# althonos/pyhmmer

Measured on AMD Instinct MI355X. Metric: GCUPS (DP cells/s) + seqs/s for hmmsearch, Pfam-A vs proteome, 1/2/4/8 GPUs, higher is better.
Workload: dtype u8/i16 filters (MSV, Viterbi), f32 Forward/Backward

## Files before the change

include/p7x.h:

```cpp
#ifndef P7X_H
#define P7X_H

#include <stddef.h>
#include <stdint.h>

#ifdef __cplusplus
extern "C" {
#endif

#define P7X_ABI_VERSION 8

enum {
  P7X_OK = 0, P7X_EMEM = 5, P7X_EFORMAT = 7, P7X_EINVAL = 11, P7X_ERANGE = 16, P7X_ENORESULT = 19,
  P7X_ENODEVICE = 100, P7X_EDEVICE = 101
};

enum { P7X_RNA = 1, P7X_DNA = 2, P7X_AMINO = 3 };
enum { P7X_SEARCH_SEQS = 0, P7X_SCAN_MODELS = 1 };
enum { P7X_ZSETBY_NTARGETS = 0, P7X_ZSETBY_OPTION = 1, P7X_ZSETBY_FILEINFO = 2 };
enum { P7X_MMU = 0, P7X_MLAMBDA, P7X_VMU, P7X_VLAMBDA, P7X_FTAU, P7X_FLAMBDA };
enum { P7X_GA1 = 0, P7X_GA2, P7X_TC1, P7X_TC2, P7X_NC1, P7X_NC2 };
#define P7X_CUTOFF_UNSET (-99999.0f)
#define P7X_EVPARAM_UNSET (-99999.0f)
enum { P7X_IS_INCLUDED = 1, P7X_IS_REPORTED = 2, P7X_IS_NEW = 4, P7X_IS_DROPPED = 8, P7X_IS_DUPLICATE = 16 };
// ... 78 lines not shown
  int32_t do_max, do_biasfilter, do_null2;
  uint32_t seed;
  int32_t mode;
  int32_t host_threads;
  int32_t host_envelopes;
  int32_t host_regions;
  int32_t long_targets;
  int32_t strands;
  int32_t B1, B2, B3;
  int32_t block_length;
  int32_t window_length;
  int32_t evalue_window_length;
  int32_t lt_part, lt_nparts;
  float   oa_guard;
  float   f3_guard;
  uint64_t lt_resident_key;
  int32_t host_ensembles;
  float   ens_guard;
} p7x_pipeline_cfg;
enum { P7X_STRAND_BOTH = 0, P7X_STRAND_TOPONLY = 1, P7X_STRAND_BOTTOMONLY = 2 };
void p7x_pipeline_cfg_default(p7x_pipeline_cfg *cfg);

typedef struct p7x_counters {
  uint64_t nmodels, nseqs, nres, nnodes;
  uint64_t n_past_msv, n_past_bias, n_past_vit, n_past_fwd;
  uint64_t n_output, pos_past_msv, pos_past_bias, pos_past_vit, pos_past_fwd, pos_output;
} p7x_counters;

typedef struct p7x_domain {
  int64_t ienv, jenv, iali, jali, iorf, jorf;
  float envsc, domcorrection, dombias, oasc, bitscore;
  double lnP;
  int32_t is_reported, is_included;
  int32_t N, hmmfrom, hmmto, M;
  int64_t sqfrom, sqto, L;
  const char *model, *mline, *aseq, *ppline, *rfline, *mmline, *csline;
  const char *hmmname, *hmmacc, *hmmdesc, *sqname, *sqacc, *sqdesc;
} p7x_domain;

typedef struct p7x_hit {
  const char *name, *acc, *desc;
  int64_t seqidx;
  int32_t window_length;
  double sortkey;
  float score, pre_score, sum_score;
  double lnP, pre_lnP, sum_lnP;
  float nexpected;
  int32_t nregions, nclustered, noverlaps, nenvelopes, ndom;
  uint32_t flags;
  int32_t nreported, nincluded, best_domain;
} p7x_hit;

typedef struct p7x_tophits p7x_tophits;

int p7x_search_block(const p7x_pipeline_cfg *cfg, const p7x_oprofile *om, const float *bg_f,
                     const p7x_seqdb *db, const char *const *names, const char *const *accs,
                     const char *const *descs, p7x_tophits **out);

typedef struct p7x_pending p7x_pending;
int  p7x_search_block_begin(const p7x_pipeline_cfg *cfg, const p7x_oprofile *om, const float *bg_f,
                            const p7x_seqdb *db, p7x_pending **out);
int  p7x_search_block_finish(p7x_pending *pending, const char *const *names, const char *const *accs,
                             const char *const *descs, p7x_tophits **out);
void p7x_pending_destroy(p7x_pending *pending);
int  p7x_search_block_enqueue(const p7x_pipeline_cfg *cfg, const p7x_oprofile *om, const float *bg_f,
                              const p7x_seqdb *db, p7x_pending **out);
int  p7x_search_block_wait(p7x_pending *pending);
int  p7x_search_batch_enqueue(const p7x_pipeline_cfg *cfg, const p7x_oprofile *const *oms, size_t nq, const float *bg_f,
                              const p7x_seqdb *db, p7x_pending **out);
int  p7x_search_batch_finish(p7x_pending *pending, const char *const *names, const char *const *accs,
                             const char *const *descs, p7x_tophits **outs);
size_t p7x_pending_nqueries(const p7x_pending *pending);
int  p7x_debug_log_of_float(int device, const float *in, float *out, size_t n);
int  p7x_debug_memory_stats(int device, int64_t out[4]);
int  p7x_debug_choice(const float *p, int n, uint32_t x, int *via_thresholds, int *via_fchoose);
int  p7x_debug_order_spread(const p7x_oprofile *om, const uint8_t *dsq1, int32_t L, int32_t i, int32_t j, int multihit, double *out12);
int  p7x_debug_parser_rows(const p7x_oprofile *om, const uint8_t *dsq1, int32_t L, float *fx, float *bx);
int64_t p7x_debug_ssv_tables(const p7x_oprofile *om, int pair, int32_t *R, int32_t *pair_slack, uint32_t *tab4q, size_t cap_words);
int  p7x_debug_set_option(const char *name, int value);
int  p7x_debug_ensemble(const p7x_oprofile *om, const p7x_seqdb *db, int64_t target, int32_t i, int32_t j, uint32_t seed,
                        int use_device, int32_t *ndom, int32_t *dom, int32_t dom_cap, float *n2, int32_t *status);
int  p7x_search_batch_raw(const p7x_pipeline_cfg *cfg, const p7x_oprofile *const *oms, size_t nq, const float *bg_f,
                          const p7x_seqdb *db, int32_t *xJ, int32_t *xC, uint8_t *stage);

int p7x_search_longtargets(const p7x_pipeline_cfg *cfg, const p7x_oprofile *om, int device,
                           const uint8_t *dsq, const int64_t *offsets, const int64_t *lengths, size_t n,
                           const char *const *names, const char *const *accs, const char *const *descs, p7x_tophits **out);
int p7x_longtargets_release_resident(int device, uint64_t key);
int64_t p7x_ssv_longtarget_seeds(const p7x_pipeline_cfg *cfg, const p7x_oprofile *om, int device, const uint8_t *dsq, int64_t L,
                                 int complement, int64_t *seeds, size_t cap);
int p7x_longtarget_from_seeds(const p7x_pipeline_cfg *cfg, const p7x_oprofile *om,
                              const uint8_t *dsq, const int64_t *offsets, const int64_t *lengths, size_t n,
                              const char *const *names, const char *const *accs, const char *const *descs,
                              const int64_t *seed_target, const int64_t *seed_block, const int32_t *seed_strand,
                              const int64_t *seeds, size_t nseeds, p7x_tophits **out);

int p7x_forward_parser_exact(const p7x_oprofile *om, const uint8_t *dsq, int32_t L, float *sc);

int p7x_scan_collect(p7x_tophits *const *per_model, size_t nmodels, const p7x_pipeline_cfg *cfg, size_t nseqs,
                     const char *const *seq_names, const char *const *seq_accs, const char *const *seq_descs,
                     const int32_t *seq_lengths, p7x_tophits **out);
typedef struct p7x_scan_accum p7x_scan_accum;
int  p7x_scan_accum_create(const p7x_pipeline_cfg *cfg, size_t nseqs, const char *const *seq_names, const char *const *seq_accs,
                           const char *const *seq_descs, const int32_t *seq_lengths, p7x_scan_accum **out);
int  p7x_scan_accum_add(p7x_scan_accum *acc, p7x_tophits *const *per_model, size_t nmodels);
int  p7x_scan_accum_add_indexed(p7x_scan_accum *acc, p7x_tophits *const *per_model, const int64_t *model_index, size_t nmodels);
int  p7x_debug_tophits_set_stages(p7x_tophits *th, const uint8_t *stage, size_t n);
int  p7x_scan_accum_finish(p7x_scan_accum *acc, p7x_tophits **out);
void p7x_scan_accum_destroy(p7x_scan_accum *acc);

int p7x_postprocess_targets(const p7x_pipeline_cfg *cfg, const p7x_oprofile *om, const uint8_t *dsq,
                            const int64_t *offsets, const int32_t *lengths, size_t n, const int32_t *surv,
                            size_t nsurv, const float *fwdsc, const float *fwd_xmx, const float *bck_xmx,
                            const int64_t *xmx_off, const uint64_t *stage_counts, const char *const *names,
                            const char *const *accs, const char *const *descs, p7x_tophits **out);

void     p7x_tophits_destroy(p7x_tophits *th);
void     p7x_tophits_destroy_many(p7x_tophits **th, size_t n);
p7x_tophits *p7x_tophits_clone(const p7x_tophits *th);
int64_t  p7x_tophits_nhits(const p7x_tophits *th);
int      p7x_tophits_abc_type(const p7x_tophits *th);
int      p7x_tophits_get_counters(const p7x_tophits *th, p7x_counters *c);
int      p7x_tophits_get_cfg(const p7x_tophits *th, p7x_pipeline_cfg *cfg);
int      p7x_tophits_get_hit(const p7x_tophits *th, int64_t i, p7x_hit *hit);
int      p7x_tophits_get_domain(const p7x_tophits *th, int64_t i, int32_t d, p7x_domain *dom);
int      p7x_tophits_merge(p7x_tophits *dst, const p7x_tophits *src);
int      p7x_tophits_merge_longtargets(p7x_tophits **parts, size_t nparts, p7x_tophits **out);
int      p7x_tophits_merge_many(const void *const *blobs, const size_t *sizes, size_t nq, size_t nparts, int threads, p7x_tophits **outs);
int64_t  p7x_tophits_serialize(const p7x_tophits *th, void *buf, size_t cap);
p7x_tophits *p7x_tophits_deserialize(const void *buf, size_t n);
int      p7x_tophits_sort_by_key(p7x_tophits *th);
int      p7x_tophits_threshold(p7x_tophits *th);
int      p7x_tophits_sort_by_seqidx(p7x_tophits *th);
int      p7x_tophits_is_sorted(const p7x_tophits *th, int by_seqidx);
int      p7x_tophits_set_hit_flags(p7x_tophits *th, int64_t i, uint32_t flags);
int      p7x_tophits_set_hit_text(p7x_tophits *th, int64_t i, int which, const char *value);
int      p7x_tophits_get_timings(const p7x_tophits *th, double *ms, int n);
int      p7x_tophits_get_guard_counts(const p7x_tophits *th, int64_t *f3_dropped, int64_t *oa_redone, int64_t oa_why[8]);
int      p7x_tophits_get_ensemble_counts(const p7x_tophits *th, int64_t *sampled_on_device, int64_t *redone_by_host, int64_t *region_scans_redone);

typedef struct p7x_traces p7x_traces;
enum { P7X_TRACE_HAS_PP = 1, P7X_TRACE_DEVICE = 2 };
int     p7x_tracealign_compute(const p7x_oprofile *om, int device, const uint8_t *dsq, const int64_t *offsets,
                               const int32_t *lengths, size_t n, int host_threads, p7x_traces **out);
int64_t p7x_traces_count(const p7x_traces *tr);
int64_t p7x_traces_nflagged(const p7x_traces *tr);
int     p7x_traces_stats(const p7x_traces *tr, int64_t out4[4]);
int     p7x_traces_get(const p7x_traces *tr, int64_t idx, int32_t *N, int32_t *M, int32_t *L, float *sc2, int32_t *status, uint8_t *origin);
int     p7x_traces_copy(const p7x_traces *tr, int64_t idx, int8_t *st, int32_t *k, int32_t *i, float *pp);
void    p7x_traces_destroy(p7x_traces *tr);

enum { P7X_MSA_TRIM = 1, P7X_MSA_ALL_CONSENSUS_COLS = 2, P7X_MSA_DIGITIZE = 4 };
typedef struct p7x_msa p7x_msa;
int     p7x_msa_from_traces(int32_t M, size_t n, const int8_t *st, const int32_t *k, const int32_t *i, const float *pp,
                            const int64_t *toff, const uint8_t *origin, const uint8_t *dsq, const int64_t *offsets,
                            const int32_t *lengths, int32_t abc_type, const char *cs, int flags, const p7x_oprofile *om,
                            p7x_msa **out);
int64_t p7x_msa_alen(const p7x_msa *msa);
int64_t p7x_msa_get(const p7x_msa *msa, int64_t idx, int which, char *buf, size_t cap);
void    p7x_msa_destroy(p7x_msa *msa);
int64_t p7x_msa_write_stockholm(size_t n, int64_t alen, const char *const *names, const char *const *accs,
                                const char *const *descs, const char *const *aseqs, const char *const *pps,
                                const char *ss_cons, const char *pp_cons, const char *rf, char *buf, size_t cap);

int     p7x_alidisplay_backconvert(int32_t abc_type, const char *model, const char *aseq, const char *ppline, int32_t hmmfrom,
                                   int32_t hmmto, int64_t sqfrom, int64_t sqto, int64_t L, int whole, int32_t *N, int32_t *subL,
// ... 33 lines not shown
```

pyhmmer_amd/_lib.py:

```python
from __future__ import annotations

import ctypes as C
import os
import shutil
import subprocess
from pathlib import Path

_PKG = Path(__file__).resolve().parent
_ROOT = _PKG.parent
CSRC = _PKG / "csrc"
LIB_PATH = _PKG / "libp7x.so"

SOURCES = ["p7x_profile.cpp", "p7x_device.hip", "p7x_devmem.hip", "p7x_devimage.hip", "p7x_msv.hip", "p7x_vitfwd.hip", "p7x_vitpk.hip", "p7x_fwdpk.hip", "p7x_envelope.hip", "p7x_ensemble.hip", "p7x_ssvlong.hip", "p7x_longtarget.hip",
           "p7x_envscore.hip", "p7x_pipeline.hip", "p7x_domaindef.cpp", "p7x_longtarget_host.cpp", "p7x_tophits.cpp", "p7x_align.hip", "p7x_tracealign.cpp", "p7x_builder.cpp", "p7x_calibrate.hip"]


def _hipcc() -> str:
    for cand in (os.environ.get("HIPCC"), shutil.which("hipcc"), "/opt/rocm/bin/hipcc"):
        if cand and os.path.exists(cand):
            return cand
    raise RuntimeError("hipcc not found (need ROCm; set HIPCC=/path/to/hipcc)")


ISA_CHECKED = ("p7x_msv.hip", "p7x_envelope.hip")
# ... 121 lines not shown
        ("hmmname", C.c_char_p), ("hmmacc", C.c_char_p), ("hmmdesc", C.c_char_p),
        ("sqname", C.c_char_p), ("sqacc", C.c_char_p), ("sqdesc", C.c_char_p),
    ]


class HitRec(C.Structure):
    _fields_ = [
        ("name", C.c_char_p), ("acc", C.c_char_p), ("desc", C.c_char_p),
        ("seqidx", C.c_int64), ("window_length", C.c_int32), ("sortkey", C.c_double),
        ("score", C.c_float), ("pre_score", C.c_float), ("sum_score", C.c_float),
        ("lnP", C.c_double), ("pre_lnP", C.c_double), ("sum_lnP", C.c_double),
        ("nexpected", C.c_float),
        ("nregions", C.c_int32), ("nclustered", C.c_int32), ("noverlaps", C.c_int32),
        ("nenvelopes", C.c_int32), ("ndom", C.c_int32),
        ("flags", C.c_uint32), ("nreported", C.c_int32), ("nincluded", C.c_int32), ("best_domain", C.c_int32),
    ]


_VP = C.c_void_p
_SIGNATURES = {
    "p7x_abi_version": (C.c_int, []),
    "p7x_tophits_merge_longtargets": (C.c_int, [C.POINTER(_VP), C.c_size_t, C.POINTER(_VP)]),
    "p7x_tophits_merge_many": (C.c_int, [C.POINTER(C.c_char_p), C.POINTER(C.c_size_t), C.c_size_t, C.c_size_t, C.c_int, C.POINTER(_VP)]),
    "p7x_tophits_get_guard_counts": (C.c_int, [_VP, C.POINTER(C.c_int64), C.POINTER(C.c_int64), C.POINTER(C.c_int64)]),
    "p7x_tophits_get_ensemble_counts": (C.c_int, [_VP, C.POINTER(C.c_int64), C.POINTER(C.c_int64), C.POINTER(C.c_int64)]),
    "p7x_hmm_max_length": (C.c_int, [C.POINTER(HmmView), C.c_double, C.POINTER(C.c_int32)]),
    "p7x_expf_neg": (None, [_VP, _VP, C.c_size_t]),
    "p7x_oprofile_create": (C.c_int, [C.POINTER(HmmView), _VP, C.c_int32, C.POINTER(_VP)]),
    "p7x_oprofile_destroy": (None, [_VP]),
    "p7x_oprofile_get_info": (C.c_int, [_VP, C.POINTER(OprofileInfo)]),
    "p7x_oprofile_striped": (C.c_int64, [_VP, C.c_int, _VP, C.c_size_t]),
    "p7x_device_count": (C.c_int, []),
    "p7x_device_name": (C.c_int, [C.c_int, C.c_char_p, C.c_size_t]),
    "p7x_seqdb_create": (C.c_int, [C.c_int, C.c_int32, _VP, _VP, _VP, C.c_size_t, C.POINTER(_VP)]),
    "p7x_seqdb_destroy": (None, [_VP]),
    "p7x_seqdb_ntargets": (C.c_int64, [_VP]),
    "p7x_seqdb_nresidues": (C.c_int64, [_VP]),
    "p7x_msv_filter": (C.c_int, [_VP, C.c_int, _VP, C.c_int32, C.POINTER(C.c_float)]),
    "p7x_vit_filter": (C.c_int, [_VP, C.c_int, _VP, C.c_int32, C.POINTER(C.c_float)]),
    "p7x_fwd_parser": (C.c_int, [_VP, C.c_int, _VP, C.c_int32, C.POINTER(C.c_float)]),
    "p7x_bck_parser": (C.c_int, [_VP, C.c_int, _VP, C.c_int32, C.POINTER(C.c_float)]),
    "p7x_filters_batch": (C.c_int, [_VP, _VP, _VP, _VP, _VP, _VP]),
    "p7x_pipeline_cfg_default": (None, [C.POINTER(PipelineCfg)]),
    "p7x_search_block": (C.c_int, [C.POINTER(PipelineCfg), _VP, _VP, _VP, _VP, _VP, _VP, C.POINTER(_VP)]),
    "p7x_postprocess_targets": (C.c_int, [C.POINTER(PipelineCfg), _VP, _VP, _VP, _VP, C.c_size_t, _VP, C.c_size_t, _VP, _VP, _VP,
                                          _VP, _VP, _VP, _VP, _VP, C.POINTER(_VP)]),
    "p7x_tophits_destroy": (None, [_VP]),
    "p7x_tophits_destroy_many": (None, [_VP, C.c_size_t]),
    "p7x_tophits_clone": (_VP, [_VP]),
    "p7x_tophits_nhits": (C.c_int64, [_VP]),
    "p7x_tophits_abc_type": (C.c_int, [_VP]),
    "p7x_tophits_get_counters": (C.c_int, [_VP, C.POINTER(Counters)]),
    "p7x_tophits_get_cfg": (C.c_int, [_VP, C.POINTER(PipelineCfg)]),
    "p7x_tophits_get_hit": (C.c_int, [_VP, C.c_int64, C.POINTER(HitRec)]),
    "p7x_tophits_get_domain": (C.c_int, [_VP, C.c_int64, C.c_int32, C.POINTER(DomainRec)]),
    "p7x_tophits_merge": (C.c_int, [_VP, _VP]),
    "p7x_tophits_serialize": (C.c_int64, [_VP, _VP, C.c_size_t]),
    "p7x_tophits_deserialize": (_VP, [_VP, C.c_size_t]),
    "p7x_tophits_sort_by_key": (C.c_int, [_VP]),
    "p7x_tophits_threshold": (C.c_int, [_VP]),
    "p7x_tophits_sort_by_seqidx": (C.c_int, [_VP]),
    "p7x_tophits_is_sorted": (C.c_int, [_VP, C.c_int]),
    "p7x_tophits_set_hit_flags": (C.c_int, [_VP, C.c_int64, C.c_uint32]),
    "p7x_tophits_set_hit_text": (C.c_int, [_VP, C.c_int64, C.c_int, C.c_char_p]),
    "p7x_tophits_get_timings": (C.c_int, [_VP, C.POINTER(C.c_double), C.c_int]),
    "p7x_search_block_begin": (C.c_int, [C.POINTER(PipelineCfg), _VP, _VP, _VP, C.POINTER(_VP)]),
    "p7x_search_block_enqueue": (C.c_int, [C.POINTER(PipelineCfg), _VP, _VP, _VP, C.POINTER(_VP)]),
    "p7x_search_block_wait": (C.c_int, [_VP]),
    "p7x_search_block_finish": (C.c_int, [_VP, _VP, _VP, _VP, C.POINTER(_VP)]),
    "p7x_pending_destroy": (None, [_VP]),
    "p7x_search_batch_enqueue": (C.c_int, [C.POINTER(PipelineCfg), C.POINTER(_VP), C.c_size_t, _VP, _VP, C.POINTER(_VP)]),
    "p7x_search_batch_finish": (C.c_int, [_VP, _VP, _VP, _VP, C.POINTER(_VP)]),
    "p7x_pending_nqueries": (C.c_size_t, [_VP]),
    "p7x_debug_log_of_float": (C.c_int, [C.c_int, _VP, _VP, C.c_size_t]),
    "p7x_debug_memory_stats": (C.c_int, [C.c_int, C.POINTER(C.c_int64)]),
    "p7x_debug_choice": (C.c_int, [_VP, C.c_int, C.c_uint32, _VP, _VP]),
    "p7x_debug_order_spread": (C.c_int, [_VP, _VP, C.c_int32, C.c_int32, C.c_int32, C.c_int, _VP]),
    "p7x_debug_parser_rows": (C.c_int, [_VP, _VP, C.c_int32, _VP, _VP]),
    "p7x_debug_ssv_tables": (C.c_int64, [_VP, C.c_int, _VP, _VP, _VP, C.c_size_t]),
    "p7x_debug_set_option": (C.c_int, [C.c_char_p, C.c_int]),
    "p7x_longtargets_release_resident": (C.c_int, [C.c_int, C.c_uint64]),
    "p7x_debug_ensemble": (C.c_int, [_VP, _VP, C.c_int64, C.c_int32, C.c_int32, C.c_uint32, C.c_int, _VP, _VP, C.c_int32, _VP, _VP]),
    "p7x_search_batch_raw": (C.c_int, [C.POINTER(PipelineCfg), C.POINTER(_VP), C.c_size_t, _VP, _VP, _VP, _VP, _VP]),
    "p7x_search_longtargets": (C.c_int, [C.POINTER(PipelineCfg), _VP, C.c_int, _VP, _VP, _VP, C.c_size_t, _VP, _VP, _VP, C.POINTER(_VP)]),
    "p7x_ssv_longtarget_seeds": (C.c_int64, [C.POINTER(PipelineCfg), _VP, C.c_int, _VP, C.c_int64, C.c_int, _VP, C.c_size_t]),
    "p7x_forward_parser_exact": (C.c_int, [_VP, _VP, C.c_int32, C.POINTER(C.c_float)]),
    "p7x_longtarget_from_seeds": (C.c_int, [C.POINTER(PipelineCfg), _VP, _VP, _VP, _VP, C.c_size_t, _VP, _VP, _VP, _VP, _VP, _VP, _VP,
                                            C.c_size_t, C.POINTER(_VP)]),
    "p7x_oprofile_write_pressed": (C.c_int, [_VP, C.POINTER(C.c_int64), _VP, C.c_size_t, C.POINTER(C.c_size_t), _VP, C.c_size_t,
                                             C.POINTER(C.c_size_t)]),
    "p7x_oprofile_read_pressed": (C.c_int, [_VP, C.c_size_t, _VP, C.c_size_t, _VP, C.POINTER(_VP), C.POINTER(C.c_size_t),
                                            C.POINTER(C.c_size_t), C.POINTER(C.c_int64)]),
    "p7x_oprofile_get_string": (C.c_int, [_VP, C.c_int, C.c_char_p, C.c_size_t]),
    "p7x_scan_collect": (C.c_int, [C.POINTER(_VP), C.c_size_t, C.POINTER(PipelineCfg), C.c_size_t, _VP, _VP, _VP, _VP, C.POINTER(_VP)]),
    "p7x_scan_accum_create": (C.c_int, [C.POINTER(PipelineCfg), C.c_size_t, _VP, _VP, _VP, _VP, C.POINTER(_VP)]),
    "p7x_scan_accum_add": (C.c_int, [_VP, C.POINTER(_VP), C.c_size_t]),
    "p7x_scan_accum_add_indexed": (C.c_int, [_VP, C.POINTER(_VP), C.POINTER(C.c_int64), C.c_size_t]),
    "p7x_debug_tophits_set_stages": (C.c_int, [_VP, _VP, C.c_size_t]),
    "p7x_scan_accum_finish": (C.c_int, [_VP, C.POINTER(_VP)]),
    "p7x_scan_accum_destroy": (None, [_VP]),
    "p7x_fasta_parse": (C.c_int, [_VP, C.c_size_t, _VP, C.POINTER(C.c_size_t), C.POINTER(C.c_size_t), C.POINTER(C.c_size_t),
                                  _VP, _VP, _VP, _VP, _VP, _VP, C.POINTER(C.c_size_t)]),
    "p7x_tracealign_compute": (C.c_int, [_VP, C.c_int, _VP, _VP, _VP, C.c_size_t, C.c_int, C.POINTER(_VP)]),
    "p7x_traces_count": (C.c_int64, [_VP]),
    "p7x_traces_nflagged": (C.c_int64, [_VP]),
    "p7x_traces_stats": (C.c_int, [_VP, _VP]),
    "p7x_traces_get": (C.c_int, [_VP, C.c_int64, C.POINTER(C.c_int32), C.POINTER(C.c_int32), C.POINTER(C.c_int32), _VP,
                                 C.POINTER(C.c_int32), C.POINTER(C.c_uint8)]),
    "p7x_traces_copy": (C.c_int, [_VP, C.c_int64, _VP, _VP, _VP, _VP]),
    "p7x_traces_destroy": (None, [_VP]),
    "p7x_msa_from_traces": (C.c_int, [C.c_int32, C.c_size_t, _VP, _VP, _VP, _VP, _VP, _VP, _VP, _VP, _VP, C.c_int32, C.c_char_p,
                                      C.c_int, _VP, C.POINTER(_VP)]),
    "p7x_msa_alen": (C.c_int64, [_VP]),
    "p7x_msa_get": (C.c_int64, [_VP, C.c_int64, C.c_int, C.c_char_p, C.c_size_t]),
    "p7x_msa_destroy": (None, [_VP]),
    "p7x_msa_write_stockholm": (C.c_int64, [C.c_size_t, C.c_int64, C.POINTER(C.c_char_p), C.POINTER(C.c_char_p),
                                            C.POINTER(C.c_char_p), C.POINTER(C.c_char_p), C.POINTER(C.c_char_p), C.c_char_p,
                                            C.c_char_p, C.c_char_p, C.c_char_p, C.c_size_t]),
    "p7x_alidisplay_backconvert": (C.c_int, [C.c_int32, C.c_char_p, C.c_char_p, C.c_char_p, C.c_int32, C.c_int32, C.c_int64, C.c_int64,
                                             C.c_int64, C.c_int, C.POINTER(C.c_int32), C.POINTER(C.c_int32), _VP, _VP, _VP, _VP, _VP,
                                             C.c_size_t]),
    "p7x_tophits_to_msa": (C.c_int, [_VP, C.c_int32, C.c_int32, C.c_size_t, _VP, _VP, _VP, _VP, _VP, _VP, _VP, _VP, _VP,
                                     C.POINTER(C.c_char_p), C.POINTER(C.c_char_p), C.POINTER(C.c_char_p), C.c_int, C.POINTER(_VP)]),
    "p7x_debug_tophits_from_displays": (C.c_int, [C.c_char_p, C.c_int32, C.c_int32, C.c_size_t, C.POINTER(C.c_char_p),
                                                  C.POINTER(C.c_char_p), C.POINTER(C.c_char_p), C.POINTER(C.c_uint32),
                                                  C.POINTER(C.c_int32), C.POINTER(DomainRec), C.POINTER(_VP)]),
    "p7x_debug_tophits_from_trace": (C.c_int, [_VP, _VP, C.c_int32, C.c_int32, _VP, _VP, _VP, _VP, C.c_char_p, C.POINTER(_VP)]),
    "p7x_builder_single": (C.c_int, [C.c_int32, _VP, C.c_int32, _VP, C.c_char_p, C.c_double, C.c_double, _VP, _VP, _VP]),
    "p7x_calibration_stream": (C.c_int, [C.c_int32, _VP, C.c_uint32, C.c_int, _VP]),
    "p7x_calibration_redraw": (C.c_int, [C.c_int32, _VP, C.c_uint32, C.c_int, _VP, C.c_int, _VP]),
    "p7x_calibration_draw_of": (C.c_int32, [C.c_int32, _VP, C.c_int]),
    "p7x_calibration_scores": (C.c_int, [_VP, _VP, _VP, _VP, _VP]),
    "p7x_calibration_fit": (C.c_int, [_VP, _VP, C.c_double, _VP]),
    "p7x_oprofile_match_relent": (C.c_double, [_VP]),
    "p7x_calibrate_batch": (C.c_int, [C.POINTER(_VP), C.c_size_t, C.c_int, C.c_uint32, _VP, _VP]),
    "p7x_last_error": (C.c_char_p, []),
}

_lib = None


def lib() -> C.CDLL:
    global _lib
    if _lib is None:
        if not LIB_PATH.exists():
            raise ImportError(
                f"{LIB_PATH} is missing: the HIP extension has not been built. "
                "Run `python -c 'import __graft_entry__ as g; g.build()'` (needs hipcc); there is no CPU fallback.")
        l = C.CDLL(str(LIB_PATH))
        for name, (res, args) in _SIGNATURES.items():
            fn = getattr(l, name)
            fn.restype = res
            fn.argtypes = args
        if l.p7x_abi_version() != 8:
            raise ImportError("libp7x ABI version mismatch; rebuild")
        _lib = l
    return _lib


def declared_symbols():
    return sorted(_SIGNATURES)


def last_error() -> str:
    e = lib().p7x_last_error()
    return e.decode() if e else ""
# ... 6 lines not shown
```

pyhmmer_amd/csrc/p7x_device.hpp:

```cpp
#pragma once
#include "p7x_internal.hpp"
#include "p7x_devmem.hpp"
#include <hip/hip_runtime.h>
#include <map>
#include <memory>
#include <mutex>

namespace p7x {

constexpr int kMaxL      = 100000;
constexpr int kTabRows   = 32;
constexpr int kNegPad    = -512;

#define P7X_HIP(call)                                                                          \
  do { hipError_t e_ = (call); if (e_ != hipSuccess) {                                         \
    p7x::set_error(std::string(#call) + ": " + hipGetErrorString(e_)); return e_ == hipErrorOutOfMemory ? P7X_EMEM : P7X_EDEVICE; } } while (0)

struct LengthTables {
  uint8_t *tjb = nullptr;
  int16_t *xwmove = nullptr;
  float   *null1 = nullptr;
  double  *logtab = nullptr;
};

struct DeviceCtx {
  int device = -1;
  hipStream_t stream = nullptr;
  hipStream_t stream2 = nullptr;
  LengthTables lt;
  int num_cu = 256;
  std::mutex mu;
  std::mutex msv_mu;
  std::mutex lt_scan_mu;
  static constexpr int kLtStreams = 4;
  hipStream_t lt_stream[kLtStreams]{};
  int lt_next = 0;
  hipEvent_t msv_done[2] = { nullptr, nullptr };
  int msv_last = -1;
  std::mutex slab_mu;
  std::multimap<size_t, void *> slab_free;
  size_t slab_free_bytes = 0;
  size_t slab_obtained_bytes = 0;
  static constexpr int kWsSets = 4, kWsSide = 7;
  hipStream_t ws_main[kWsSets]{};
  hipStream_t ws_side[kWsSets][kWsSide]{};
  std::vector<hipStream_t> ws_spacers;
  int ws_set_users[kWsSets]{};
};
int get_ctx(int device, DeviceCtx **out);
int create_tail_stream(DeviceCtx *ctx, bool high_priority, hipStream_t *out);

struct DevProfile {
  int device = -1;
  int M = 0, Kp = 0;
  int msvR = 0, msvK = 0, msvS = 0;
  uint32_t *msv_tab = nullptr;
  int16_t *msvw_emis = nullptr;
  uint32_t *msvw_pk = nullptr;
  int msvwC = 0, msvw_rows = kTabRows;
  int vitC = 0, Mpad = 0;
  int16_t *vit_trans = nullptr;
  int16_t *vit_emis = nullptr;
  int vitpkT = 0, vitpkP = 0;
  uint32_t *vitpk_trans = nullptr, *vitpk_emis = nullptr;
  float *fwd_trans = nullptr;
  float *fwd_emis = nullptr;
  int fwdgT = 0, fwdgC = 0;
  float *fwdg_trans = nullptr, *fwdg_emis = nullptr;
  float *bias_eo = nullptr;
  std::shared_ptr<DeviceBuf> shared;
};

int get_dev_profile(const p7x_oprofile *om, DeviceCtx *ctx, DevProfile **out);
int get_dev_profiles(const p7x_oprofile *const *oms, int n, DeviceCtx *ctx, DevProfile **out, int nthreads);
void free_dev_profile(DevProfile *d);

struct EnvelopeScorer;
struct EnsembleRunner;
}
struct p7x_seqdb;
#include <memory>
namespace p7x {
struct LongTargetWindowRegions;
int device_regions_of_all(const p7x_oprofile *om, const p7x_seqdb *db, std::vector<LongTargetWindowRegions> &out);
std::unique_ptr<EnvelopeScorer> make_device_envelope_scorer(DeviceCtx *ctx, const p7x_seqdb *db, float oa_guard);
std::unique_ptr<EnvelopeScorer> make_device_align_scorer(DeviceCtx *ctx, const p7x_seqdb *db, float oa_guard);
size_t align_budget_bytes();
std::unique_ptr<EnsembleRunner> make_device_ensemble_runner(DeviceCtx *ctx, const p7x_seqdb *db, float guard);

}

struct p7x_seqdb {
  int device = -1;
  int abc_type = 0, Kp = 0;
  int64_t n = 0;
  int64_t nres = 0;
  int64_t nslots = 0;
  int64_t ngroups = 0;
  std::vector<int32_t> h_len;
  std::vector<int32_t> h_order;
  std::vector<int64_t> h_off;
  std::vector<uint8_t> h_dsq;
  int64_t vit_long_slots = 0;
  std::vector<int32_t> h_grp_len;
  std::vector<int64_t> h_grp_suffix;
  uint8_t *d_dsq = nullptr;
  int64_t *d_slot_off = nullptr;
  int32_t *d_slot_len = nullptr;
  uint4   *d_tiles = nullptr;
  int64_t *d_grp_off = nullptr;
  int32_t *d_grp_nblk = nullptr;
  int64_t tile_u4 = 0;
  p7x::DeviceBuf slab;
};
```

pyhmmer_amd/csrc/p7x_devimage.hip:

```cpp
#include "p7x_device.hpp"
#include "p7x_kernels.hpp"
#include "p7x_host.hpp"
#include <cstring>
#include <memory>

namespace p7x {

static void chunk_transpose_fill(int M, int C, std::vector<int> &pos_of_node)
{
  pos_of_node.assign(M + 1, -1);
  for (int k = 1; k <= M; ++k) { const int z = (k - 1) / C, c = (k - 1) % C; pos_of_node[k] = c * 64 + z; }
}

void free_dev_profile(DevProfile *d)
{
  delete d;
}

struct DevCache { std::mutex mu; std::vector<DevProfile *> per_device; };

struct ImageStage { int device = -1; PinnedBuf pinned; hipStream_t stream = nullptr; };

struct HostImage {
  std::vector<char> bytes;
  std::vector<std::pair<void **, size_t>> fix;
  template <typename T, typename F>
  void add(F **field, const std::vector<T> &v)
  {
    const size_t off = bytes.size(), n = v.size() * sizeof(T);
    bytes.resize(((off + n + 255) / 256) * 256);
    std::memcpy(bytes.data() + off, v.data(), n);
    fix.emplace_back(reinterpret_cast<void **>(field), off);
  }
};

static void build_host_image(const Profile &p, DevProfile *d, HostImage &img)
{
  d->msvR = msv_pick(p.M, &d->msvK);
  if (d->msvR > 0) {
    d->msvS = msv_stride(d->msvR, d->msvK);
    std::vector<uint32_t> tab;
    msv_build_tables(p, d->msvR, d->msvK, tab);
    img.add(&d->msv_tab, tab);
  }
  d->vitC = vit_pick_C(p.M);
  if (d->vitC > 0) {
    const int C = d->vitC, Mpad = 64 * C, nrows = p.Kp + 1;
    d->Mpad = Mpad;
    std::vector<int> pos;
    chunk_transpose_fill(p.M, C, pos);
    std::vector<int16_t> vt((size_t) Mpad * 8, -32768), ve((size_t) nrows * Mpad, -32768);
    std::vector<float> ft((size_t) Mpad * 8, 0.0f), fe((size_t) nrows * Mpad, 0.0f);
    for (int k = 1; k <= p.M; ++k) {
      for (int t = 0; t < NTRANS; ++t) {
        vt[(size_t) pos[k] * 8 + t] = p.tw[(size_t) t * (p.M + 1) + k];
        ft[(size_t) pos[k] * 8 + t] = p.tf[(size_t) t * (p.M + 1) + k];
      }
      for (int x = 0; x < p.Kp; ++x) {
        ve[(size_t) x * Mpad + pos[k]] = p.rw[(size_t) x * (p.M + 1) + k];
        fe[(size_t) x * Mpad + pos[k]] = p.rf_[(size_t) x * (p.M + 1) + k];
      }
    }
    {
      std::vector<int16_t> me((size_t) kTabRows * Mpad, (int16_t) kNegPad);
      for (int k = 1; k <= p.M; ++k)
        for (int x = 0; x < p.Kp; ++x) me[(size_t) x * Mpad + pos[k]] = (int16_t) ((int) p.bias_b - (int) p.rb[(size_t) x * (p.M + 1) + k]);
      img.add(&d->msvw_emis, me);
      d->msvwC = C; d->msvw_rows = kTabRows;
      int Cp = 0;
      if ((d->msvR <= 0 || d->msvK >= 8) && C % 4 == 0 && C <= 32) Cp = C;
      else if (d->msvR <= 0 && C > 32 && p.M <= 2560 && p.Kp + 1 <= 30) { Cp = p.M <= 2304 ? 36 : 40; d->msvwC = Cp; d->msvw_rows = p.Kp + 1; }
      if (Cp > 0) {
        const int P2 = Cp / 4, rows = d->msvw_rows;
        std::vector<uint32_t> pk((size_t) rows * P2 * 64 * 2);
        auto em = [&](int x, int k) -> uint32_t { return (uint32_t) (uint16_t) (int16_t) ((x < p.Kp && k <= p.M) ? (int) p.bias_b - (int) p.rb[(size_t) x * (p.M + 1) + k] : kNegPad); };
        for (int x = 0; x < rows; ++x)
          for (int j2 = 0; j2 < P2; ++j2)
            for (int z = 0; z < 64; ++z)
              for (int h = 0; h < 2; ++h) {
                const int k = z * Cp + 2 * (2 * j2 + h) + 1;
                pk[(((size_t) x * P2 + j2) * 64 + z) * 2 + h] = em(x, k) | (em(x, k + 1) << 16);
              }
        img.add(&d->msvw_pk, pk);
      }
    }
    img.add(&d->vit_trans, vt);
    img.add(&d->vit_emis, ve);
    img.add(&d->fwd_trans, ft);
    img.add(&d->fwd_emis, fe);
    int gT = 0, gC = 0;
    if (fwdg_pick(p.M, d->vitC, &gT, &gC)) {
      std::vector<float> gt, ge;
      fwdg_build_tables(p, gT, gC, gt, ge);
      d->fwdgT = gT; d->fwdgC = gC;
      img.add(&d->fwdg_trans, gt);
      img.add(&d->fwdg_emis, ge);
    }
  }
  {
    int T = 0, P = 0;
    if (vitpk_pick(p.M, &T, &P)) {
      std::vector<uint32_t> tt, te;
      vitpk_build_tables(p, T, P, tt, te);
      d->vitpkT = T; d->vitpkP = P;
      img.add(&d->vitpk_trans, tt);
      img.add(&d->vitpk_emis, te);
    }
  }
  {
    const Alphabet &abc = Alphabet::get(p.abc_type);
    std::vector<float> eo((size_t) kTabRows * 2, 1.0f);
    for (int x = 0; x < p.K; ++x) { eo[x * 2 + 0] = p.bgf[x] / p.bgf[x]; eo[x * 2 + 1] = p.compo[x] / p.bgf[x]; }
    for (int x = p.K + 1; x <= p.Kp - 3; ++x)
      for (int s = 0; s < 2; ++s) {
        float e = 0.0f, den = 0.0f;
        for (int y = 0; y < p.K; ++y) if (abc.degen[x][y]) { e += (s == 0 ? p.bgf[y] : p.compo[y]); den += p.bgf[y]; }
        eo[x * 2 + s] = den > 0.0f ? e / den : 0.0f;
      }
    img.add(&d->bias_eo, eo);
  }
}

int get_dev_profiles(const p7x_oprofile *const *oms, int n, DeviceCtx *ctx, DevProfile **out, int nthreads)
{
  std::vector<int> missing;
  for (int i = 0; i < n; ++i) {
// ... 74 lines not shown
```

pyhmmer_amd/csrc/p7x_internal.hpp:

```cpp
#pragma once
#include "../../include/p7x.h"
#include <cstdint>
#include <string>
#include <vector>

namespace p7x {

constexpr int MAXK  = 20;
constexpr int MAXKP = 29;
constexpr double kLog2  = 0.69314718055994529;
constexpr double kLog2R = 1.44269504088896341;

enum { XE = 0, XN = 1, XJ = 2, XC = 3 };
enum { MOVE = 0, LOOP = 1 };
enum { tBM = 0, tMM, tIM, tDM, tMD, tMI, tII, tDD, NTRANS };
enum { gMM = 0, gIM, gDM, gBM, gMD, gDD, gMI, gII };

struct Alphabet {
  int type, K, Kp;
  const char *sym;
  unsigned char degen[MAXKP][MAXK];
  static const Alphabet &get(int type);
};

struct Profile {
  int M = 0, K = 0, Kp = 0, abc_type = 0, L = 0, max_length = -1, mode = 0;
  float nj = 1.0f;
  double relent_mh = 0.0;
  std::string name, acc, desc, consensus, rf, mm, cs;
  bool has_acc = false, has_desc = false;
  float evparam[6], cutoff[6], compo[MAXK], bgf[MAXK];
  std::vector<float> tsc;
  std::vector<float> msc;
  float xsc[4][2];
  std::vector<uint8_t> rb;
  uint8_t tbm_b, tec_b, tjb_b, base_b, bias_b;
  float scale_b;
  std::vector<int16_t> rw;
  std::vector<int16_t> tw;
  int16_t xw[4][2];
  float scale_w; int16_t base_w, ddbound_w; float ncj_roundoff;
  std::vector<float> rf_;
  std::vector<float> tf;
  float xf[4][2];

  int Q16() const { int q = (M - 1) / 16 + 1; return q < 2 ? 2 : q; }
  int Q8()  const { int q = (M - 1) / 8  + 1; return q < 2 ? 2 : q; }
  int Q4()  const { int q = (M - 1) / 4  + 1; return q < 2 ? 2 : q; }
};

float  sse_expf(float x);
uint8_t unbiased_byteify(float scale_b, float sc);
int16_t wordify(float scale_w, float sc);
double gumbel_surv(double x, double mu, double lambda);
double exp_surv(double x, double mu, double lambda);
double exp_logsurv(double x, double mu, double lambda);
float  null1_score(int L);
double match_relent_sum(const float *mat, const float *bg_f, int M, int K);
void   flogsum_init();
float  flogsum(float a, float b);

void set_error(const std::string &msg);

enum { OPT_SMALL_BLOCK = 0, OPT_VIT_WAVE, OPT_MSV_EXACT, OPT_MSV_LONG_GROUPS, OPT_MSV_BLOCKS_PER_CU, OPT_ENV_WORKSPACE_GB, OPT_DEVICE_CLUSTERED,
       OPT_TRACE_FINISH, OPT_TRACE_LONGTARGET, OPT_TRACE_ENVELOPE, OPT_HOST_PROFILE, OPT_SSV_KERNEL, OPT_MSV_F16, OPT_ENS_LDS_KB, OPT_ENS_FAIL, OPT_MSV_TIERS, OPT_STAGE_MERGE, OPT_EARLY_PACK, OPT_HOST_ORDER, OPT_VIT_LONG_CUT, OPT_FWD_GROUPED, OPT_REGION_GUARD_PPM, OPT_MSV_K8, OPT_MSV_LANE_BLOCKS, OPT_HOST_ALIGN, OPT_ALIGN_WORKSPACE_GB, OPT_COUNT };
int debug_opt(int which);

}
struct p7x_oprofile;
namespace p7x {
void attach_dev_cache(p7x_oprofile *om);

}

struct p7x_oprofile { p7x::Profile p; void *dev_cache = nullptr; };
```

pyhmmer_amd/csrc/p7x_kernels.hpp:

```cpp
#pragma once
#include <type_traits>
#include "p7x_device.hpp"

namespace p7x {

struct ArgRef { const void *base; uint32_t stride; };
#if defined(__HIPCC__)
template <class A> __device__ __forceinline__ A load_args(const ArgRef r)
{
#if defined(__HIP_DEVICE_COMPILE__)
  typedef const __attribute__((address_space(4))) A *cptr;
  return *(cptr) (unsigned long long) (static_cast<const char *>(r.base) + (size_t) blockIdx.y * r.stride);
#else
  return *reinterpret_cast<const A *>(static_cast<const char *>(r.base) + (size_t) blockIdx.y * r.stride);
#endif
}
#endif
template <class A> struct ArgRun {
  const A *host = nullptr; const void *dev = nullptr; uint32_t stride = 0; int n = 0;
  const A &at(int i) const { return *reinterpret_cast<const A *>(reinterpret_cast<const char *>(host) + (size_t) i * stride); }
  ArgRef ref() const { return ArgRef{ dev, stride }; }
};
inline unsigned lane_grid(long want, long resident, int nlanes)
{
  (void) nlanes;
  if (want > resident) want = resident;
  return (unsigned) (want < 1 ? 1 : want);
}

inline unsigned lane_grid_pull(long want, long resident, int nlanes, bool old_rule)
{
  if (old_rule || nlanes < 32) return lane_grid(want, resident, nlanes);
  long b = (2 * resident + nlanes - 1) / nlanes;
  if (b > resident) b = resident;
  if (b > want) b = want;
  return (unsigned) (b < 1 ? 1 : b);
}

struct MsvArgs {
  const uint32_t *tab;
  const uint4 *tiles;
  const int64_t *grp_off;
  const int32_t *grp_nblk;
  const int32_t *slot_len;
  const uint8_t *tjb_tab;
  int ngroups;
  int group_first;
  int base, bias, tec, tbm;
  int *counter;
  int16_t *out_xJ;
  int *amb_count; int *amb_groups; int *counter2;
  const int *group_list; const int *group_count;
  int R;
};
int  msv_pick(int M, int *K);
int  msv_stride(int R, int K);
void msv_build_tables(const Profile &p, int R, int K, std::vector<uint32_t> &out);
int  msv_launch(int R, int K, const ArgRun<MsvArgs> &main, const ArgRun<MsvArgs> *amb, int num_cu, hipStream_t st);
constexpr int kMsvTiers = 6;
int  msv_tier(int R, int K);
int  msv_tier_launch(int tier, const ArgRun<MsvArgs> &main, int num_cu, hipStream_t st);
int  msv_exact_launch(int R, int K, const ArgRun<MsvArgs> &amb, int num_cu, hipStream_t st);

#define P7X_NODE_TIERS(X) X(1) X(2) X(3) X(4) X(5) X(6) X(8) X(10) X(12) X(16) X(20) X(24) X(32) X(48) X(64) X(96) X(128)
template <class F> int node_tier_dispatch(int C, const char *too_long, F &&f)
{
  switch (C) {
#define P7X_TIER_CASE(CC) case CC: return f(std::integral_constant<int, CC>());
    P7X_NODE_TIERS(P7X_TIER_CASE)
#undef P7X_TIER_CASE
    default: set_error(too_long); return P7X_EINVAL;
  }
}
struct WaveSeqArgs {
  int M, C;
  const void *trans;
  const void *emis;
  const uint8_t *dsq;
  const int64_t *slot_off;
  const int32_t *slot_len;
  const int32_t *list;
  int nlist;
  const int *nlist_ptr;
  const int *abort_flag;
  int nrows;
  int *counter;
  const int16_t *xwmove_tab; int base_w, xw_e, ddbound;
  int32_t *out_xC;
  const int *lt_thresh;
  int *lt_nrec; int *lt_rec; int lt_cap;
  float xf_e_move, xf_e_loop;
  float *out_sc;
  float *xmx;
  const int64_t *xmx_off;
  const float *fwd_xmx;
};
int vit_pick_C(int M);
int vit_launch(const ArgRun<WaveSeqArgs> &a, int num_cu, hipStream_t st);
int fwd_launch(const ArgRun<WaveSeqArgs> &a, int num_cu, hipStream_t st);
bool fwdg_pick(int M, int vitC, int *T, int *C);
int fwdg_launch(const ArgRun<WaveSeqArgs> &a, int num_cu, hipStream_t st);
void fwdg_build_tables(const Profile &p, int T, int C, std::vector<float> &trans, std::vector<float> &emis);
int bck_launch(const ArgRun<WaveSeqArgs> &a, int num_cu, hipStream_t st);

struct MsvWaveArgs {
  int C, nrows;
  const void *emis;
  const void *emis_pk;
  const uint8_t *dsq; const int64_t *slot_off; const int32_t *slot_len; const uint8_t *tjb_tab;
  int nslots, base, bias, tec, tbm;
  int16_t *out_xJ;
};
int msv_wave_launch(const ArgRun<MsvWaveArgs> &a, int num_cu, hipStream_t st);

struct VitPkArgs {
  const void *trans, *emis;
  const uint8_t *dsq; const int64_t *slot_off; const int32_t *slot_len;
  const int32_t *list; int nlist; const int *nlist_ptr;
  const int *nskip_ptr;
  int nrows;
  const int16_t *xwmove_tab; int base_w, xw_e, ddbound;
  int32_t *out_xC;
};
bool vitpk_pick(int M, int *T, int *P);
void vitpk_build_tables(const Profile &p, int T, int P, std::vector<uint32_t> &trans, std::vector<uint32_t> &emis);
int  vitpk_launch(int T, int P, const ArgRun<VitPkArgs> &a, int num_cu, hipStream_t st);

struct EnvArgs {
  int M, C, K, nrows;
  const void *trans;
  const void *emis;
  const uint8_t *dsq;
  float nj, xf_e_move, xf_e_loop;
  int nenv;
  const int64_t *env_sq;
  const int32_t *env_len;
  const int32_t *env_L;
  const int32_t *order;
  int *cursor;
  float *work; int64_t work_stride; int Lmax;
  int nblocks, slab_base;
  float *out_sc;
  const float *env_emis;
  long long env_emis_stride;
  float *out_orig;
  float oa_guard;
  int32_t *out_status;
  float *out_null2;
  const int64_t *tr_off;
  uint32_t *tr_a; int32_t *tr_i; float *tr_pp;
  int32_t *tr_n;
};
constexpr int env_waves(int C) { return C >= 8 ? 4 : 8; }
enum class EnvMode { Envelope, LongTarget, Align };
inline size_t env_work_floats(int C, int Lmax)
{
  const size_t rows = (size_t) Lmax + 1, Mpad = (size_t) 64 * C;
  size_t f = 2 * rows * Mpad + rows * (6 + 6 + 5 + 3 + 1);
  f += (rows * Mpad + 1) / 2;
  return (f + 63) & ~(size_t) 63;
}
int env_max_blocks(EnvMode mode, int C, int nrows, int num_cu, int *nblocks);
int env_launch(EnvMode mode, const ArgRun<EnvArgs> &a, hipStream_t st);
__host__ __device__ inline float align_pp_guard(int M) { return 1.0e-5f + 2.5e-9f * (float) M; }
__host__ __device__ inline float align_pp_band(int M) { return 0.5f - 10.0f * align_pp_guard(M); }
int align_max_blocks(int C, int nrows, int num_cu, int *nblocks);
int align_launch(const ArgRun<EnvArgs> &a, hipStream_t st);

struct ChoiceCell; struct ChoiceRow;
struct EnsRegion {
  int64_t sq;
  int64_t cell0;
  int64_t row0;
  int64_t dom0;
  int32_t Lr, L;
  int32_t job, dom_cap;
};
struct EnsJob {
  int M, C, K, Kp, nrows, Q;
  const void *trans, *emis;
  const float *rft;
  const uint8_t *degen;
  int reg_first, nreg;
};
struct EnsArgs {
  const EnsJob *jobs; const EnsRegion *regions; int nregions;
  const uint8_t *dsq;
  ChoiceCell *cells; float2 *md; ChoiceRow *rows;
  uint32_t seed_x;
  int nsamples;
  float *n2acc;
  int32_t *dom;
  int32_t *out_ndom; int32_t *out_status;
  int lds_bytes;
// ... 26 lines not shown
```

pyhmmer_amd/csrc/p7x_msv.hip:

```cpp
#include <cstdlib>
#include <iterator>
#include <map>
#include <mutex>
#include "p7x_device.hpp"
#include "p7x_kernels.hpp"

namespace p7x {

typedef short s2 __attribute__((ext_vector_type(2)));

__device__ __forceinline__ s2 as_s2(uint32_t u) { return __builtin_bit_cast(s2, u); }
__device__ __forceinline__ uint32_t as_u32(s2 v) { return __builtin_bit_cast(uint32_t, v); }
__device__ __forceinline__ s2 pk_max(s2 a, s2 b) { return __builtin_elementwise_max(a, b); }
__device__ __forceinline__ s2 pk_adds(s2 a, s2 b) { return __builtin_elementwise_add_sat(a, b); }
__device__ __forceinline__ s2 pk_subs(s2 a, s2 b) { return __builtin_elementwise_sub_sat(a, b); }
__device__ __forceinline__ s2 splat(int v) { s2 r; r.x = (short) v; r.y = (short) v; return r; }
__device__ __forceinline__ s2 swap_halves(s2 v) { return as_s2(__builtin_amdgcn_alignbit(as_u32(v), as_u32(v), 16)); }

typedef _Float16 h2 __attribute__((ext_vector_type(2)));
__device__ __forceinline__ h2 as_h2(s2 v) { return __builtin_bit_cast(h2, v); }
__device__ __forceinline__ s2 as_s2(h2 v) { return __builtin_bit_cast(s2, v); }
__device__ __forceinline__ s2 h_adds(s2 a, s2 b)
{
  const h2 z = { (_Float16) 0.0f, (_Float16) 0.0f }, o = { (_Float16) 1.0f, (_Float16) 1.0f };
  return as_s2(__builtin_elementwise_min(__builtin_elementwise_max(as_h2(a) + as_h2(b), z), o));
}
__device__ __forceinline__ s2 h_subs(s2 a, s2 b)
{
  const h2 z = { (_Float16) 0.0f, (_Float16) 0.0f }, o = { (_Float16) 1.0f, (_Float16) 1.0f };
  return as_s2(__builtin_elementwise_min(__builtin_elementwise_max(as_h2(a) - as_h2(b), z), o));
}
__device__ __forceinline__ s2 h_max(s2 a, s2 b) { return as_s2(__builtin_elementwise_maximum(as_h2(a), as_h2(b))); }
__device__ __forceinline__ s2 h_max3(s2 a, s2 b, s2 c)
{ return as_s2(__builtin_elementwise_maximum(__builtin_elementwise_maximum(as_h2(a), as_h2(b)), as_h2(c))); }
__device__ __forceinline__ s2 h_splat(int units)
{ const _Float16 x = (_Float16) ((float) units * (1.0f / 256.0f)); h2 r; r.x = x; r.y = x; return as_s2(r); }
__device__ __forceinline__ uint32_t h_of_i16_pair(uint32_t w)
{
  const int lo = max((int) (short) (w & 0xffffu), -512), hi = max((int) (short) (w >> 16), -512);
  return __builtin_bit_cast(uint32_t, __builtin_amdgcn_cvt_pkrtz((float) lo * (1.0f / 256.0f), (float) hi * (1.0f / 256.0f)));
}


constexpr int msv_stride_c(int R)
{
  int S = R + (R & 1);
  if (((S / 2) & 1) == 0) S += 2;
  return S;
}
constexpr int msv_lane_stride_c(int R, int K)
{
  if (K == 1) return msv_stride_c(R);
  int s = R + (R & 1);
  while (s % 64 != 2) s += 2;
  return s;
}
constexpr int msv_row_stride_c(int R, int K) { return K * msv_lane_stride_c(R, K); }
constexpr bool msv_uniform_c(int K) { return K >= 8; }
constexpr int msv_parities_c(int K) { return msv_uniform_c(K) ? 1 : 2; }
constexpr int msv_even_imm_c(int R, int K) { return K == 1 ? kTabRows * msv_row_stride_c(R, K) * 4 : 0; }
constexpr int msv_even_add_c(int R, int K) { return (K == 1 || msv_uniform_c(K)) ? 0 : kTabRows * msv_row_stride_c(R, K) * 4; }
constexpr int msv_block_c(int K) { return K == 1 ? 256 : 512; }
template <int K, bool H = false> __device__ __forceinline__ s2 target_max(s2 m)
{
  auto mx = [](s2 a, s2 b) { if constexpr (H) return h_max(a, b); else return pk_max(a, b); };
  if constexpr (K >= 2) m = mx(m, as_s2((uint32_t) __builtin_amdgcn_update_dpp(0, (int) as_u32(m), 0xB1, 0xf, 0xf, false)));
  if constexpr (K >= 4) m = mx(m, as_s2((uint32_t) __builtin_amdgcn_update_dpp(0, (int) as_u32(m), 0x4E, 0xf, 0xf, false)));
  if constexpr (K >= 8) m = mx(m, as_s2((uint32_t) __builtin_amdgcn_update_dpp(0, (int) as_u32(m), 0x141, 0xf, 0xf, false)));
  return m;
}
template <int K> __device__ __forceinline__ s2 carry_in(s2 last, s2 edge, int h)
{
  if constexpr (K == 1) return edge;
  const s2 up = as_s2((uint32_t) __builtin_amdgcn_update_dpp(0, (int) as_u32(last), 0x111, 0xf, 0xf, false));
  return h == 0 ? edge : up;
}

struct Chunk { uint2 e0, e1, e2, e3; };

template <int OFF>
__device__ __forceinline__ void lds_issue4(uint32_t addr, Chunk &c)
{
  asm volatile("ds_read_b64 %0, %4 offset:%5\n\t"
               "ds_read_b64 %1, %4 offset:%6\n\t"
               "ds_read_b64 %2, %4 offset:%7\n\t"
               "ds_read_b64 %3, %4 offset:%8"
               : "=&v"(c.e0), "=&v"(c.e1), "=&v"(c.e2), "=&v"(c.e3)
               : "v"(addr), "i"(OFF), "i"(OFF + 8), "i"(OFF + 16), "i"(OFF + 24));
}
template <int OFF>
__device__ __forceinline__ void lds_issue2(uint32_t addr, Chunk &c)
{
  asm volatile("ds_read_b64 %0, %2 offset:%3\n\t"
               "ds_read_b64 %1, %2 offset:%4"
               : "=&v"(c.e0), "=&v"(c.e1)
               : "v"(addr), "i"(OFF), "i"(OFF + 8));
}
template <int PENDING>
__device__ __forceinline__ void lds_wait4(Chunk &c)
{
  asm volatile("s_waitcnt lgkmcnt(%4)" : "+v"(c.e0), "+v"(c.e1), "+v"(c.e2), "+v"(c.e3) : "i"(PENDING));
}
template <int PENDING>
__device__ __forceinline__ void lds_wait2(Chunk &c)
{
  asm volatile("s_waitcnt lgkmcnt(%2)" : "+v"(c.e0), "+v"(c.e1) : "i"(PENDING));
}

template <int R, int TB, bool ODD, int T, int FAST = 0, bool U = false>
struct RowChunks {
  static_assert(!U || ODD, "the uniform row reads the register below: it is walked from the top register down");
  static_assert(R % 4 == 0, "a row is walked in chunks of 8 registers and a last one of 4: the register count must be a multiple of 4");
  static constexpr int NT = (R + 7) / 8;
  static constexpr int TBASE = TB;
  static constexpr int pairs(int t) { return (t == NT - 1 && (R % 8) != 0) ? 2 : 4; }

  template <int TT>
  static __device__ __forceinline__ void issue(uint32_t addr, Chunk &c)
  {
    if constexpr (pairs(TT) == 4) lds_issue4<TBASE + TT * 32>(addr, c); else lds_issue2<TBASE + TT * 32>(addr, c);
  }

  template <int JJ>
// ... 45 lines not shown
      }
      accA = pk_max(accA, v[2 * JJ]);
      accB = pk_max(accB, v[2 * JJ + 1]);
      asm volatile("" : "+v"(accA), "+v"(accB));
    } else if constexpr (ODD) {
      const s2 t1 = pk_max(v[2 * JJ], xB);
      v[2 * JJ + 1] = t1 + as_s2(e.y);
      accA = pk_max(accA, v[2 * JJ + 1]);
      s2 t0 = pk_max(carry, xB);
      if constexpr (JJ > 0) t0 = pk_max(v[2 * JJ - 1], xB);
      v[2 * JJ] = t0 + as_s2(e.x);
      accB = pk_max(accB, v[2 * JJ]);
    } else {
      v[2 * JJ] = pk_max(v[2 * JJ], xB) + as_s2(e.x);
      accA = pk_max(accA, v[2 * JJ]);
      v[2 * JJ + 1] = pk_max(v[2 * JJ + 1], xB) + as_s2(e.y);
      accB = pk_max(accB, v[2 * JJ + 1]);
    }
  }

  static __device__ __forceinline__ void run(s2 (&v)[R], uint32_t addr, Chunk &cur, Chunk &nxt, const s2 xB, const s2 carry, s2 &accA, s2 &accB)
  {
    constexpr bool last = ODD ? (T == 0) : (T == NT - 1);
    constexpr int TN = ODD ? T - 1 : T + 1;
    constexpr int np = pairs(T);
    if constexpr (!last) {
      issue<TN>(addr, nxt);
      if constexpr (np == 4) lds_wait4<pairs(TN)>(cur); else lds_wait2<pairs(TN)>(cur);
    } else {
      if constexpr (np == 4) lds_wait4<0>(cur); else lds_wait2<0>(cur);
    }
    if constexpr (ODD) {
      if constexpr (np == 4) {
        pair<4 * T + 3>(v, cur.e3, xB, carry, accA, accB);
        pair<4 * T + 2>(v, cur.e2, xB, carry, accA, accB);
      }
      pair<4 * T + 1>(v, cur.e1, xB, carry, accA, accB);
      pair<4 * T + 0>(v, cur.e0, xB, carry, accA, accB);
    } else {
      pair<4 * T + 0>(v, cur.e0, xB, carry, accA, accB);
      pair<4 * T + 1>(v, cur.e1, xB, carry, accA, accB);
      if constexpr (np == 4) {
        pair<4 * T + 2>(v, cur.e2, xB, carry, accA, accB);
        pair<4 * T + 3>(v, cur.e3, xB, carry, accA, accB);
      }
    }
    if constexpr (!last) RowChunks<R, TB, ODD, TN, FAST, U>::run(v, addr, nxt, cur, xB, carry, accA, accB);
  }
};

template <int R, int K, bool ODD>
__device__ __forceinline__ void msv_row(s2 (&v)[R], uint32_t addr, int h, s2 &xB, s2 &xJ, s2 &xEmax,
                                        const s2 basev, const s2 tecv, const s2 tjbmv, const s2 zerov)
{
  constexpr int NT = (R + 7) / 8;
  constexpr bool U = msv_uniform_c(K), DOWN = ODD || U;
  constexpr int T0 = DOWN ? NT - 1 : 0;
  constexpr int TB = DOWN ? 0 : msv_even_imm_c(R, K);
  const s2 carry = DOWN ? carry_in<K>(v[R - 1], xB, h) : xB;
  Chunk ca, cb;
  RowChunks<R, TB, DOWN, T0, 0, U>::template issue<T0>(addr, ca);
  s2 accA = splat(kNegPad), accB = accA;
  RowChunks<R, TB, DOWN, T0, 0, U>::run(v, addr, ca, cb, xB, carry, accA, accB);
  s2 m = pk_max(accA, accB);
  m = pk_max(m, swap_halves(m));
  m = target_max<K>(m);
  xEmax = pk_max(xEmax, m);
  m = m - tecv;
  xJ = pk_max(xJ, m);
  xB = pk_max(pk_max(basev, xJ) - tjbmv, zerov);
}

template <int K> struct MsvItem {
  int g, t, h;
  __device__ __forceinline__ MsvItem(int group, int part, int lane) : g(group), t(part * (64 / K) + lane / K), h(lane % K) {}
};

template <int R, int K>
__global__ void __launch_bounds__(msv_block_c(K)) msv_kernel(const ArgRef ref)
{
  extern __shared__ __attribute__((aligned(16))) uint32_t lds[];
  constexpr int S = msv_row_stride_c(R, K), Rs = msv_lane_stride_c(R, K), BLK = msv_block_c(K);
  const MsvArgs a = load_args<MsvArgs>(ref);
  const int nitems = (a.group_list ? *a.group_count : a.ngroups - a.group_first) * K;
  if (nitems <= 0 || *a.counter >= nitems) return;
  {
    constexpr int n4 = (msv_parities_c(K) * kTabRows * S) / 4;
    const uint4 *src = reinterpret_cast<const uint4 *>(a.tab);
    uint4 *dst = reinterpret_cast<uint4 *>(lds);
    for (int i = threadIdx.x; i < n4; i += BLK) dst[i] = src[i];
  }
  __syncthreads();

  const int lane = threadIdx.x & 63;
  const s2 basev = splat(a.base), tecv = splat(a.tec), zerov = splat(0);

  for (;;) {
    int item = 0;
    if (lane == 0) item = atomicAdd(a.counter, 1);
    item = __builtin_amdgcn_readfirstlane(item);
    if (item >= nitems) break;
    const int gi = item / K;
    const MsvItem<K> it(a.group_list ? __builtin_amdgcn_readfirstlane(a.group_list[gi]) : gi + a.group_first, item % K, lane);

    const int slot = it.g * 64 + it.t;
    const int L = a.slot_len[slot];
    const int nblk = a.grp_nblk[it.g];
    const uint4 *tp = a.tiles + a.grp_off[it.g] + it.t;
    const s2 tjbmv = splat((int) a.tjb_tab[L] + a.tbm);
    const uint32_t lane_col = (uint32_t) it.h * (uint32_t) (Rs * 4);

    s2 v[R];
#pragma unroll
    for (int j = 0; j < R; ++j) v[j] = zerov;
    s2 xJ = zerov, xEmax = zerov;
    s2 xB = pk_max(basev - tjbmv, zerov);

    uint4 cur = tp[0];
    for (int b = 0; b < nblk; ++b) {
      const uint4 nxt = (b + 1 < nblk) ? tp[(size_t) (b + 1) * 64] : cur;
      uint32_t w0 = cur.x, w1 = cur.y, w2 = cur.z, w3 = cur.w;
#pragma unroll 1
      for (int c = 0; c < 8; ++c) {
        const uint32_t x0 = w0 & 0xffu, x1 = (w0 >> 8) & 0xffu;
        w0 = __builtin_amdgcn_alignbit(w1, w0, 16); w1 = __builtin_amdgcn_alignbit(w2, w1, 16);
        w2 = __builtin_amdgcn_alignbit(w3, w2, 16); w3 >>= 16;
        msv_row<R, K, true >(v, x0 * (uint32_t) (S * 4) + lane_col, it.h, xB, xJ, xEmax, basev, tecv, tjbmv, zerov);
        msv_row<R, K, false>(v, x1 * (uint32_t) (S * 4) + lane_col + (uint32_t) msv_even_add_c(R, K), it.h, xB, xJ, xEmax, basev, tecv, tjbmv, zerov);
      }
      cur = nxt;
    }
    if (L > 0 && it.h == 0) {
      const int xe = xEmax.x;
      a.out_xJ[slot] = (xe >= 255 - a.bias) ? (int16_t) -1 : (int16_t) xJ.x;
    }
  }
}

template <int R, int K, bool H>
__device__ __forceinline__ void msv_fast_body(const MsvArgs &a, uint32_t *lds)
{
  constexpr int S = msv_row_stride_c(R, K), Rs = msv_lane_stride_c(R, K), BLK = msv_block_c(K);
  constexpr int MODE = H ? 2 : 1;
  const int nitems = (a.ngroups - a.group_first) * K;
  if (*a.counter >= nitems) return;
  {
    constexpr int n4 = (msv_parities_c(K) * kTabRows * S) / 4;
    const uint4 *src = reinterpret_cast<const uint4 *>(a.tab);
    uint4 *dst = reinterpret_cast<uint4 *>(lds);
    for (int i = threadIdx.x; i < n4; i += BLK) {
      uint4 w = src[i];
      if constexpr (H) { w.x = h_of_i16_pair(w.x); w.y = h_of_i16_pair(w.y); w.z = h_of_i16_pair(w.z); w.w = h_of_i16_pair(w.w); }
      dst[i] = w;
    }
  }
  __syncthreads();

  const int lane = threadIdx.x & 63;
  const s2 floorv = H ? as_s2(0u) : splat(-32768);
  constexpr int NT = (R + 7) / 8;
  auto mx = [](s2 x, s2 y) { if constexpr (H) return h_max(x, y); else return pk_max(x, y); };

  for (;;) {
    int item = 0;
    if (lane == 0) item = atomicAdd(a.counter, 1);
    item = __builtin_amdgcn_readfirstlane(item);
    if (item >= nitems) break;
    const MsvItem<K> it(item / K + a.group_first, item % K, lane);

    const int slot = it.g * 64 + it.t;
    const int L = a.slot_len[slot];
    const int nblk = a.grp_nblk[it.g];
    const uint2 *tp = reinterpret_cast<const uint2 *>(a.tiles + a.grp_off[it.g] + it.t);
    const int tjbm = (int) a.tjb_tab[L] + a.tbm;
    const uint32_t lane_col = (uint32_t) it.h * (uint32_t) (Rs * 4);

    s2 v[R];
#pragma unroll
    for (int j = 0; j < R; ++j) v[j] = floorv;
    int xJ = 0, xEmax = 0;
    int xB = max(a.base - tjbm, 0);
    const int F0 = xB - a.tec;
    const s2 Tv = H ? h_splat(tjbm + a.tec) : splat(tjbm + a.tec - 32768);
    s2 accA = floorv, accB = floorv;
    auto fold = [&](const s2 m2) -> int {
      int rel;
      if constexpr (H) { const h2 m = as_h2(m2); rel = (int) (256.0f * fmaxf((float) m.x, (float) m.y)); }
      else rel = max((int) m2.x, (int) m2.y) + 32768;
      const int xE = rel + xB;
      xEmax = max(xEmax, xE);
      xJ = max(xJ, xE - a.tec);
      return max(max(a.base, xJ) - tjbm, 0);
    };

    uint2 cur = tp[0];
    for (int hb = 0; hb < 2 * nblk; ++hb) {
      const uint2 nxt = (hb + 1 < 2 * nblk) ? tp[(size_t) ((hb + 1) >> 1) * 128 + ((hb + 1) & 1)] : cur;
      uint32_t w0 = cur.x, w1 = cur.y;
#pragma unroll 1
      for (int c = 0; c < 4; ++c) {
        const uint32_t x0 = w0 & 0xffu, x1 = (w0 >> 8) & 0xffu;
        w0 = __builtin_amdgcn_alignbit(w1, w0, 16); w1 >>= 16;
#pragma unroll
        for (int half = 0; half < 2; ++half) {
          Chunk ca, cb;
          if constexpr (msv_uniform_c(K)) {
            const uint32_t addr = (half == 0 ? x0 : x1) * (uint32_t) (S * 4) + lane_col;
            const s2 carry = carry_in<K>(v[R - 1], floorv, it.h);
            RowChunks<R, 0, true, NT - 1, MODE, true>::template issue<NT - 1>(addr, ca);
            RowChunks<R, 0, true, NT - 1, MODE, true>::run(v, addr, ca, cb, floorv, carry, accA, accB);
          } else if (half == 0) {
            const uint32_t addr = x0 * (uint32_t) (S * 4) + lane_col;
            const s2 carry = carry_in<K>(v[R - 1], floorv, it.h);
            RowChunks<R, 0, true, NT - 1, MODE>::template issue<NT - 1>(addr, ca);
            RowChunks<R, 0, true, NT - 1, MODE>::run(v, addr, ca, cb, floorv, carry, accA, accB);
          } else {
            const uint32_t addr = x1 * (uint32_t) (S * 4) + lane_col + (uint32_t) msv_even_add_c(R, K);
            RowChunks<R, msv_even_imm_c(R, K), false, 0, MODE>::template issue<0>(addr, ca);
            RowChunks<R, msv_even_imm_c(R, K), false, 0, MODE>::run(v, addr, ca, cb, floorv, floorv, accA, accB);
          }
          const s2 m2 = target_max<K, H>(mx(accA, accB));
          if (__builtin_expect(__any(as_u32(mx(m2, Tv)) != as_u32(Tv)), 0)) {
            asm volatile("; re-bias: the begin score moved" ::: "memory");
            const int xBn = fold(m2);
            const s2 dv = H ? h_splat(xBn - xB) : splat(xBn - xB);
#pragma unroll
            for (int j = 0; j < R; ++j) v[j] = H ? h_subs(v[j], dv) : pk_subs(v[j], dv);
            xB = xBn;
            accA = floorv; accB = floorv;
          }
        }
      }
      cur = nxt;
    }
    fold(target_max<K, H>(mx(accA, accB)));
    const bool ambiguous = (L > 0) && (xJ == F0) && !(xEmax >= 255 - a.bias);
    if (L > 0 && it.h == 0) a.out_xJ[slot] = (xEmax >= 255 - a.bias) ? (int16_t) -1 : (int16_t) xJ;
    if (__any(ambiguous) && lane == 0) { const int idx = atomicAdd(a.amb_count, 1); a.amb_groups[idx] = it.g; }
  }
}

constexpr int msv_min_blocks_c(int R, int K) { return K > 1 ? 2 : (R <= 92 ? 4 : (R <= 136 ? 3 : 2)); }

template <int R, int K, bool H>
__global__ void __launch_bounds__(msv_block_c(K), msv_min_blocks_c(R, K)) msv_fast_kernel(const ArgRef ref)
{
  extern __shared__ __attribute__((aligned(16))) uint32_t lds[];
  const MsvArgs a = load_args<MsvArgs>(ref);
  msv_fast_body<R, K, H>(a, lds);
}

#define P7X_TILES_TIER0(X) X(8, 1) X(12, 1) X(16, 1) X(20, 1) X(24, 1) X(28, 1) X(32, 1) X(36, 1) X(40, 1) X(44, 1) X(48, 1) X(52, 1) \
                           X(56, 1) X(60, 1) X(64, 1) X(68, 1) X(72, 1) X(76, 1) X(80, 1) X(84, 1) X(88, 1) X(92, 1)
#define P7X_TILES_TIER1(X) X(96, 1) X(100, 1) X(104, 1) X(108, 1) X(112, 1) X(116, 1) X(120, 1) X(124, 1) X(128, 1) X(132, 1) X(136, 1)
#define P7X_TILES_TIER2(X) X(140, 1) X(144, 1) X(148, 1) X(152, 1) X(156, 1) X(160, 1) X(176, 1) X(192, 1) X(208, 1) X(224, 1)
#define P7X_TILES_TIER3(X) X(120, 2) X(128, 2) X(136, 2) X(144, 2) X(152, 2) X(160, 2) X(168, 2) X(176, 2) X(184, 2) X(192, 2) X(200, 2) \
                           X(208, 2) X(216, 2) X(224, 2)
#define P7X_TILES_TIER4(X) X(120, 4) X(128, 4)
#define P7X_TILES_TIER5(X) X(64, 8) X(72, 8) X(80, 8) X(88, 8) X(96, 8) X(104, 8) X(112, 8) X(120, 8) X(128, 8)
constexpr int msv_tier_block_c(int T) { return T <= 2 ? 256 : 512; }
constexpr int msv_tier_min_blocks_c(int T) { return T == 0 ? 4 : (T == 1 ? 3 : 2); }

template <int TIER>
__global__ void __launch_bounds__(msv_tier_block_c(TIER), msv_tier_min_blocks_c(TIER)) msv_tier_kernel(const ArgRef ref)
{
  extern __shared__ __attribute__((aligned(16))) uint32_t lds[];
  const MsvArgs a = load_args<MsvArgs>(ref);
  const int R = __builtin_amdgcn_readfirstlane(a.R);
#define P7X_TILE(r, k) case r: msv_fast_body<r, k, true>(a, lds); break;
  if constexpr (TIER == 0) { switch (R) { P7X_TILES_TIER0(P7X_TILE) default: break; } }
  else if constexpr (TIER == 1) { switch (R) { P7X_TILES_TIER1(P7X_TILE) default: break; } }
  else if constexpr (TIER == 2) { switch (R) { P7X_TILES_TIER2(P7X_TILE) default: break; } }
  else if constexpr (TIER == 3) { switch (R) { P7X_TILES_TIER3(P7X_TILE) default: break; } }
  else if constexpr (TIER == 4) { switch (R) { P7X_TILES_TIER4(P7X_TILE) default: break; } }
  else { switch (R) { P7X_TILES_TIER5(P7X_TILE) default: break; } }
#undef P7X_TILE
}


#define P7X_R_ONLY(r, k) r,
static const int kRList[] = { P7X_TILES_TIER0(P7X_R_ONLY) P7X_TILES_TIER1(P7X_R_ONLY) P7X_TILES_TIER2(P7X_R_ONLY) };
static const int kRList2[] = { P7X_TILES_TIER3(P7X_R_ONLY) };
static const int kRList4[] = { P7X_TILES_TIER4(P7X_R_ONLY) };
static const int kRList8[] = { P7X_TILES_TIER5(P7X_R_ONLY) };
#undef P7X_R_ONLY
static bool msv_tile_exists(int R, int K)
{
  auto in = [R](const int *b, const int *e) { for (; b != e; ++b) if (*b == R) return true; return false; };
  switch (K) {
    case 1: return in(std::begin(kRList), std::end(kRList));
    case 2: return in(std::begin(kRList2), std::end(kRList2));
    case 4: return in(std::begin(kRList4), std::end(kRList4));
    case 8: return in(std::begin(kRList8), std::end(kRList8));
    default: return false;
  }
}

int msv_pick(int M, int *K)
{
  const int need = (M + 1) / 2 + 1;
  *K = 1;
  for (int r : kRList) if (r >= need) return r;
  *K = 2;
  for (int r : kRList2) if (2 * r >= need) return r;
  *K = 4;
  for (int r : kRList4) if (4 * r >= need) return r;
  *K = 8;
  if (debug_opt(OPT_MSV_K8) != 0)
    for (int r : kRList8) if (8 * r >= (M + 1) / 2) return r;
  *K = 0;
  return -1;
}

static int row_stride(int R, int K)
{
  int rs = R + (R & 1);
  if (K == 1) { if (((rs / 2) & 1) == 0) rs += 2; return rs; }
  while (rs % 64 != 2) rs += 2;
  return K * rs;
}
int msv_stride(int R, int K) { return row_stride(R, K); }
// ... 170 lines not shown
```

pyhmmer_amd/csrc/p7x_pipeline.hip:

```cpp
#include "p7x_wave.hpp"
#include "p7x_host.hpp"
#include <atomic>
#include <chrono>
#include <cmath>
#include <cstdlib>
#include <cstring>
#include <memory>
#include <string>

namespace p7x {

struct StageBufs {
  int16_t *xJ;
  float *usc, *filtersc, *vfsc, *fwdsc;
  int32_t *xC;
  float *fwd_by_item;
  int32_t *list_bias, *list_vit, *list_fwd, *list_fin;
  uint8_t *stage;
  int *counters;
};

struct StageParams {
  double F1, F2, F3;
  double F3_near;
  float mmu, mlambda, vmu, vlambda, ftau, flambda;
  float msv_reject_below;
  int do_bias;
  int base_b, tjb_unused; float scale_b;
  int base_w; float scale_w;
  int M;
};

__device__ __forceinline__ double d_gumbel_surv(double x, double mu, double lambda)
{
  const double y = lambda * (x - mu), ey = -exp(-y);
  return (fabs(ey) < 5e-9) ? -ey : 1 - exp(ey);
}
__device__ __forceinline__ double d_exp_surv(double x, double mu, double lambda) { return x < mu ? 1.0 : exp(-lambda * (x - mu)); }

__device__ __forceinline__ void wave_append(int *counter, int32_t *list, bool take, int32_t value)
{
  const unsigned long long mask = __ballot(take);
  if (mask == 0) return;
  const int lane = (int) (threadIdx.x & 63);
  const int leader = __ffsll((long long) mask) - 1;
  int base = 0;
  if (lane == leader) base = atomicAdd(counter, __popcll(mask));
  base = __shfl(base, leader);
  if (take) list[base + __popcll(mask & ((1ull << lane) - 1ull))] = value;
}
__device__ __forceinline__ void wave_count(int *counter, bool take)
{
  const unsigned long long mask = __ballot(take);
  if (mask != 0 && (int) (threadIdx.x & 63) == __ffsll((long long) mask) - 1) atomicAdd(counter, __popcll(mask));
}

struct DecideArgs {
  StageBufs b; StageParams p;
  const int32_t *slot_len; const uint8_t *tjb_tab; const float *null1_tab; const int16_t *xwmove_tab; const double *logtab;
  const uint8_t *dsq; const int64_t *slot_off; const float *eo;
  int64_t nslots;
};

__global__ void decide_msv_kernel(const ArgRef ref)
{
  const DecideArgs a = load_args<DecideArgs>(ref);
  const StageBufs &b = a.b; const StageParams &p = a.p;
  const int64_t s = (int64_t) blockIdx.x * blockDim.x + threadIdx.x;
  bool take = false;
  if (s < a.nslots) {
    const int L = a.slot_len[s];
    const int xJ = b.xJ[s];
    float usc;
    if (xJ < 0) usc = __builtin_inff();
    else {
      usc = ((float) (xJ - (int) a.tjb_tab[L]) - (float) p.base_b);
      usc /= p.scale_b;
      usc -= 3.0f;
    }
    b.usc[s] = usc;
    const float seq_score = (float) ((double) (usc - a.null1_tab[L]) / kLog2);
    if (!(seq_score < p.msv_reject_below)) {
      const double P = d_gumbel_surv((double) seq_score, (double) p.mmu, (double) p.mlambda);
      take = !(P > p.F1);
    }
    b.stage[s] = take ? 1 : 0;
  }
  wave_append(&b.counters[1], b.list_bias, take, (int32_t) s);
}

__device__ __forceinline__ float log_of_float(float x, const double *tab)
{
  const uint32_t u = __float_as_uint(x);
  if (u - 0x00800000u >= 0x7f000000u) return (float) log((double) x);
  const int e = (int) (u >> 23) - 127;
  const uint32_t mant = u & 0x7fffffu;
  const int i = (int) (mant >> 16);
  const double m = (double) __uint_as_float(mant | 0x3f800000u);
  const double r = fma(m, tab[2 * i], -1.0);
  const double q = r * fma(r, fma(r, fma(r, fma(r, 0.2, -0.25), 1.0 / 3.0), -0.5), 1.0);
  const double y = fma((double) e, 0.693147180559945309417232121458, tab[2 * i + 1] + q);
  const float f = (float) y;
  const uint32_t fb = __float_as_uint(f) & 0x7f800000u;
  if (fb > (25u << 23)) {
    const double half_ulp = (double) __uint_as_float(fb - (24u << 23));
    if (fabs(fabs(y - (double) f) - half_ulp) < 4e-14 * fabs(y) + 1e-17) return (float) log((double) x);
  }
  return f;
}

__global__ void log_of_float_kernel(const float *in, float *out, size_t n, const double *tab)
{
  __shared__ double s_logtab[256];
  for (int z = (int) threadIdx.x; z < 256; z += (int) blockDim.x) s_logtab[z] = tab[z];
  __syncthreads();
  for (size_t i = (size_t) blockIdx.x * blockDim.x + threadIdx.x; i < n; i += (size_t) gridDim.x * blockDim.x) out[i] = log_of_float(in[i], s_logtab);
}

__global__ void bias_kernel(const ArgRef ref)
{
  const DecideArgs a = load_args<DecideArgs>(ref);
  const StageBufs &b = a.b; const StageParams &p = a.p;
  const uint8_t *dsq = a.dsq; const float *eo = a.eo;
  __shared__ double s_logtab[256];
  __shared__ float s_eo[kTabRows * 2];
  for (int z = (int) threadIdx.x; z < 256; z += (int) blockDim.x) s_logtab[z] = a.logtab[z];
  for (int z = (int) threadIdx.x; z < kTabRows * 2; z += (int) blockDim.x) s_eo[z] = eo[z];
  __syncthreads();
  const int n = b.counters[1];
  for (int it0 = blockIdx.x * blockDim.x; it0 < n; it0 += gridDim.x * blockDim.x) {
    const int it = it0 + (int) threadIdx.x;
    bool to_vit = false, to_fwd = false;
    int s = 0;
    if (it < n) {
    s = b.list_bias[it];
    const int L = a.slot_len[s];
    const float nullsc = a.null1_tab[L];
    float filtersc = nullsc;
    const float usc = b.usc[s];
    double P;
    bool pass = true;
    if (p.do_bias) {
      const uint8_t *sq = dsq + a.slot_off[s];
      const float p1 = (float) L / (float) (L + 1);
      const float L1 = (float) ((double) (float) p.M / 8.0);
      const float t00 = p1, t01 = 1.0f - p1, t10 = 1.0f / (L1 + 1.0f), t11 = L1 / (L1 + 1.0f);
      const float pi0 = (float) 0.999, pi1 = (float) 0.001;
      int x = sq[0];
      float dp0 = s_eo[x * 2] * pi0, dp1 = s_eo[x * 2 + 1] * pi1;
      float mx = 0.0f; mx = dp0 > mx ? dp0 : mx; mx = dp1 > mx ? dp1 : mx;
      dp0 /= mx; dp1 /= mx;
      float logsc = 0.0f;
      logsc += log_of_float(mx, s_logtab);
      int xcur[16];
#pragma unroll
      for (int j = 0; j < 16; ++j) xcur[j] = (1 + j < L) ? (int) sq[1 + j] : 0;
      for (int i0 = 1; i0 < L; i0 += 16) {
        const int nstep = min(16, L - i0);
        int xnext[16];
#pragma unroll
        for (int j = 0; j < 16; ++j) xnext[j] = (i0 + 16 + j < L) ? (int) sq[i0 + 16 + j] : 0;
        float e0[16], e1[16];
#pragma unroll
        for (int j = 0; j < 16; ++j) { e0[j] = s_eo[xcur[j] * 2]; e1[j] = s_eo[xcur[j] * 2 + 1]; }
        float mxs[16];
#pragma unroll
        for (int j = 0; j < 16; ++j) {
          mxs[j] = 1.0f;
          if (j < nstep) {
            float n0 = 0.0f; n0 += dp0 * t00; n0 += dp1 * t10; n0 *= e0[j];
            float n1 = 0.0f; n1 += dp0 * t01; n1 += dp1 * t11; n1 *= e1[j];
// ... 375 lines not shown
  return P7X_OK;
}

static int get_workspace(DeviceCtx *ctx, int64_t nslots, int nlanes, Lease<Workspace> &out)
{
  out = LeasePool<Workspace>::instance().lease(ctx->device, [&](const Workspace &w, const Workspace *b) {
    return w.cap_slots >= nslots && w.nlanes >= nlanes && (!b || w.cap_slots * w.nlanes < b->cap_slots * b->nlanes); });
  if (out->cap_slots == 0) {
    const int st = build_workspace(out.get(), ctx, nslots, nlanes);
    if (st != P7X_OK) { out.discard(); return st; }
  }
  out->take_stream_set();
  return P7X_OK;
}

static StageParams make_params(const Profile &p, const p7x_pipeline_cfg &cfg)
{
  StageParams s{};
  s.F1 = cfg.do_max ? 1.0 : cfg.F1; s.F2 = cfg.do_max ? 1.0 : cfg.F2; s.F3 = cfg.do_max ? 1.0 : cfg.F3;
  s.F3_near = 2.0;
  if (!cfg.do_max && !cfg.long_targets && cfg.f3_guard > 0.0f) { s.F3 = cfg.F3 * (1.0 + (double) cfg.f3_guard); s.F3_near = cfg.F3 * (1.0 - (double) cfg.f3_guard); }
  s.mmu = p.evparam[P7X_MMU]; s.mlambda = p.evparam[P7X_MLAMBDA]; s.vmu = p.evparam[P7X_VMU];
  s.vlambda = p.evparam[P7X_VLAMBDA]; s.ftau = p.evparam[P7X_FTAU]; s.flambda = p.evparam[P7X_FLAMBDA];
  s.do_bias = cfg.do_max ? 0 : cfg.do_biasfilter;
  s.msv_reject_below = -INFINITY;
  if (s.F1 > 0.0 && s.F1 < 1.0 && s.mlambda > 0.0f) {
    const double x1 = (double) s.mmu - std::log(-std::log1p(-s.F1)) / (double) s.mlambda;
    if (std::isfinite(x1)) s.msv_reject_below = (float) (x1 - 1e-3) - 1e-3f;
  }
  s.base_b = p.base_b; s.scale_b = p.scale_b; s.base_w = p.base_w; s.scale_w = p.scale_w; s.M = p.M;
  return s;
}

struct ListEstimates { int bias, vit, fwd, fin; };
static ListEstimates estimate_lists(const p7x_pipeline_cfg &cfg, int64_t nslots)
{
  auto est = [&](double f, double slack, int floor_) {
    const double v = cfg.do_max ? (double) nslots : std::min<double>((double) nslots, (double) nslots * f * slack + floor_);
    return (int) std::min<double>(v, (double) INT_MAX);
  };
  ListEstimates e;
  e.bias = est(cfg.F1, 2.0, 1024); e.vit = e.bias;
  e.fwd = est(cfg.F2, 8.0, 512);
  e.fin = est(cfg.F3, 50.0, 1024);
  return e;
}

static WaveSeqArgs ws_args(const Profile &p, const DevProfile *dp, const p7x_seqdb *db, DeviceCtx *ctx)
{
  WaveSeqArgs a{};
  a.M = p.M; a.C = dp->vitC; a.nrows = p.Kp + 1;
  a.dsq = db->d_dsq; a.slot_off = db->d_slot_off; a.slot_len = db->d_slot_len;
  a.xwmove_tab = ctx->lt.xwmove; a.base_w = p.base_w; a.xw_e = p.xw[XE][MOVE]; a.ddbound = p.ddbound_w;
  a.xf_e_move = p.xf[XE][MOVE]; a.xf_e_loop = p.xf[XE][LOOP];
  return a;
}

static bool msv_exact_only() { return debug_opt(OPT_MSV_EXACT) > 0; }
static bool vit_wave_only() { return debug_opt(OPT_VIT_WAVE) > 0; }
static bool device_clustered(int host_threads)
{
  const int forced = debug_opt(OPT_DEVICE_CLUSTERED);
  if (forced >= 0) return forced != 0;
  const int threads = host_threads > 0 ? std::min(host_threads, tophits_usable_cpus()) : tophits_usable_cpus();
  return threads < 12;
}

static bool small_block(const p7x_seqdb *db, const DeviceCtx *ctx, int nlanes)
{
  return debug_opt(OPT_SMALL_BLOCK) != 0 && db->ngroups * (int64_t) nlanes <= (int64_t) ctx->num_cu * 4;
}

static int long_groups(const p7x_seqdb *db, const DeviceCtx *ctx, int nlanes)
{
  if (debug_opt(OPT_MSV_LONG_GROUPS) == 0 || db->ngroups < 2) return 0;
  const int64_t resident = (int64_t) ctx->num_cu * 4 * 3;
  const int64_t G = db->ngroups;
  int64_t g = 0;
  while (g < G / 2 && (int64_t) db->h_grp_len[(size_t) g] * resident > (int64_t) nlanes * db->h_grp_suffix[(size_t) g]) ++g;
  return (int) g;
}

static void fill_msv_args(LaneArgs &la, const Profile &p, const DevProfile *dp, const p7x_seqdb *db, DeviceCtx *ctx, const StageBufs &b,
                          int nlong = 0)
{
  MsvWaveArgs w{};
  w.C = dp->msvwC; w.nrows = dp->msvw_rows; w.emis = dp->msvw_emis; w.emis_pk = dp->msvw_pk; w.dsq = db->d_dsq; w.slot_off = db->d_slot_off; w.slot_len = db->d_slot_len;
  w.tjb_tab = ctx->lt.tjb; w.nslots = (int) db->nslots; w.base = p.base_b; w.bias = p.bias_b; w.tec = p.tec_b; w.tbm = p.tbm_b;
  w.out_xJ = b.xJ;
  if (nlong > 0) w.nslots = (int) std::min<int64_t>((int64_t) nlong * 64, db->nslots);
  la.msvw = w;
  MsvArgs a{};
  a.group_first = nlong;
  a.tab = dp->msv_tab; a.tiles = db->d_tiles; a.grp_off = db->d_grp_off; a.grp_nblk = db->d_grp_nblk;
  a.slot_len = db->d_slot_len; a.tjb_tab = ctx->lt.tjb; a.ngroups = (int) db->ngroups;
  a.base = p.base_b; a.bias = p.bias_b; a.tec = p.tec_b; a.tbm = p.tbm_b;
  a.counter = &b.counters[0]; a.out_xJ = b.xJ;
  a.amb_count = &b.counters[10]; a.counter2 = &b.counters[11];
  a.amb_groups = msv_exact_only() ? nullptr : b.list_fin;
  a.R = dp->msvR;
  la.msv = a;
  MsvArgs x = a;
  x.group_list = a.amb_groups; x.group_count = a.amb_count; x.counter = a.counter2; x.amb_groups = nullptr;
  la.msv_amb = x;
}

static void fill_vit_args(LaneArgs &la, const Profile &p, const DevProfile *dp, const p7x_seqdb *db, DeviceCtx *ctx,
                          const int32_t *list, int nlist, const int *nlist_ptr, int32_t *out_xC,
                          const int *nlong_ptr = nullptr, int nlong_bound = 0)
{
  WaveSeqArgs w = ws_args(p, dp, db, ctx);
  w.trans = dp->vit_trans; w.emis = dp->vit_emis; w.list = list; w.nlist = nlist; w.nlist_ptr = nlist_ptr; w.out_xC = out_xC;
  if (nlong_ptr) { w.nlist_ptr = nlong_ptr; w.nlist = nlong_bound; }
  la.vit = w;
  VitPkArgs a{};
  a.trans = dp->vitpk_trans; a.emis = dp->vitpk_emis; a.dsq = db->d_dsq; a.slot_off = db->d_slot_off; a.slot_len = db->d_slot_len;
  a.list = list; a.nlist = nlist; a.nlist_ptr = nlist_ptr; a.nskip_ptr = nlong_ptr; a.nrows = p.Kp + 1;
  a.xwmove_tab = ctx->lt.xwmove; a.base_w = p.base_w; a.xw_e = p.xw[XE][MOVE]; a.ddbound = p.ddbound_w;
  a.out_xC = out_xC;
  la.vitpk = a;
}

template <class A> static ArgRun<A> lane_run(const Workspace *ws, A LaneArgs::*member, int first, int n)
{
  ArgRun<A> r;
  r.host = &(ws->h_args.as<LaneArgs>()[first].*member);
  r.dev = reinterpret_cast<const char *>(ws->d_args.as<LaneArgs>() + first) + (reinterpret_cast<const char *>(r.host) - reinterpret_cast<const char *>(ws->h_args.as<LaneArgs>() + first));
  r.stride = (uint32_t) sizeof(LaneArgs); r.n = n;
  return r;
}

struct LaneModel { const p7x_oprofile *om = nullptr; DevProfile *dp = nullptr; };

static int upload_args(Workspace *ws, int first, int n, hipStream_t s)
{
  P7X_HIP(hipMemcpyAsync(ws->d_args.as<LaneArgs>() + first, ws->h_args.as<LaneArgs>() + first, (size_t) n * sizeof(LaneArgs), hipMemcpyHostToDevice, s));
  return P7X_OK;
}

struct LaneClass { int first = 0, n = 0; long msv_key = 0, vit_key = 0; int C = 0; int nlong = 0; int64_t vit_long = 0; };

static long msv_key_of(const DevProfile *dp, bool small)
{
  return (dp->msvR <= 0 || small) ? -(long) dp->msvwC : (long) (dp->msvK * 1000 + dp->msvR);
}
static long vit_key_of(const DevProfile *dp, bool small)
{
  return (dp->vitpkT > 0 && !vit_wave_only() && !small) ? (long) (dp->vitpkT * 256 + dp->vitpkP) : -(long) dp->vitC;
}

static int lane_classes(const std::vector<LaneModel> &lm, const p7x_seqdb *db, const DeviceCtx *ctx, std::vector<LaneClass> &out)
{
  const int nl = (int) lm.size();
  const bool small = small_block(db, ctx, nl);
  const int nlong = small ? 0 : long_groups(db, ctx, nl);
  out.clear();
  for (int l = 0; l < nl; ++l) {
    const DevProfile *dp = lm[l].dp;
    if ((dp->msvR <= 0 || small) && !dp->msvw_emis) { set_error("model too long for the MSV kernels (M > 8192)"); return P7X_EINVAL; }
    LaneClass c; c.first = l; c.n = 1; c.msv_key = msv_key_of(dp, small); c.vit_key = vit_key_of(dp, small); c.C = dp->vitC;
    c.nlong = (c.msv_key >= 0 && dp->msvw_emis) ? nlong : 0;
    c.vit_long = c.vit_key >= 0 ? db->vit_long_slots : 0;
    if (!out.empty() && out.back().msv_key == c.msv_key && out.back().vit_key == c.vit_key && out.back().C == c.C) out.back().n++;
    else out.push_back(c);
  }
  return P7X_OK;
}

static int class_msv(const LaneClass &c, const std::vector<LaneModel> &lm, DeviceCtx *ctx, Workspace *ws, hipStream_t stream)
{
  if (c.msv_key < 0) return msv_wave_launch(lane_run(ws, &LaneArgs::msvw, c.first, c.n), ctx->num_cu, stream);
  if (c.nlong > 0) {
    const int st = msv_wave_launch(lane_run(ws, &LaneArgs::msvw, c.first, c.n), ctx->num_cu, stream);
    if (st != P7X_OK) return st;
  }
  const ArgRun<MsvArgs> amb = lane_run(ws, &LaneArgs::msv_amb, c.first, c.n);
  return msv_launch(lm[c.first].dp->msvR, lm[c.first].dp->msvK, lane_run(ws, &LaneArgs::msv, c.first, c.n), msv_exact_only() ? nullptr : &amb, ctx->num_cu, stream);
}

static int class_msv_rest(const LaneClass &c, const std::vector<LaneModel> &lm, DeviceCtx *ctx, Workspace *ws, hipStream_t stream)
{
  if (c.nlong > 0) {
    const int st = msv_wave_launch(lane_run(ws, &LaneArgs::msvw, c.first, c.n), ctx->num_cu, stream);
    if (st != P7X_OK) return st;
  }
  return msv_exact_launch(lm[c.first].dp->msvR, lm[c.first].dp->msvK, lane_run(ws, &LaneArgs::msv_amb, c.first, c.n), ctx->num_cu, stream);
}
static bool msv_tiers_enabled() { return !msv_exact_only() && debug_opt(OPT_MSV_F16) != 0 && debug_opt(OPT_MSV_TIERS) != 0; }

static int class_viterbi(const LaneClass &c, const std::vector<LaneModel> &lm, DeviceCtx *ctx, Workspace *ws, hipStream_t s)
{
  if (c.vit_key < 0) return vit_launch(lane_run(ws, &LaneArgs::vit, c.first, c.n), ctx->num_cu, s);
  if (c.vit_long > 0) {
    const int st = vit_launch(lane_run(ws, &LaneArgs::vit, c.first, c.n), ctx->num_cu, s);
    if (st != P7X_OK) return st;
  }
  return vitpk_launch(lm[c.first].dp->vitpkT, lm[c.first].dp->vitpkP, lane_run(ws, &LaneArgs::vitpk, c.first, c.n), ctx->num_cu, s);
}

static int class_wave(const LaneClass &c, Workspace *ws, WaveSeqArgs LaneArgs::*member, bool backward, DeviceCtx *ctx, hipStream_t s)
{
  return backward ? bck_launch(lane_run(ws, member, c.first, c.n), ctx->num_cu, s) : fwd_launch(lane_run(ws, member, c.first, c.n), ctx->num_cu, s);
}

struct CascadeOut {
  std::vector<int32_t> fin_slots;
  std::vector<float> fwdsc;
  std::vector<float> fwd_xmx, bck_xmx;
  std::vector<int64_t> xmx_off;
  std::vector<int32_t> reg_n, regs;
  std::vector<int32_t> reg_start;
  std::vector<float> nexpected;
  std::vector<char> near;
  bool have_xmx = false;
  std::vector<uint8_t> stage;
  int counts[16]{};
  double ms[12]{};
};

struct CascadeRun {
  p7x_pipeline_cfg cfg{};
  std::vector<const p7x_oprofile *> oms;
  std::vector<int> lane_of;
  std::vector<LaneModel> lm;
  std::vector<int> query_of;
  const p7x_seqdb *db = nullptr;
  DeviceCtx *ctx = nullptr;
  Lease<Workspace> ws;
  int est_bias = 0, est_vit = 0, est_fwd = 0, est_fin = 0;
  bool queued = false, collected = false;
  ~CascadeRun() { sync_and_return(ws); }
};

struct PackArgs {
  const int32_t *list_fin; const float *fwd_by_item; int64_t slot_pitch;
  const int64_t *xmx_off; const int32_t *reg_out; int64_t cap;
  const int *counters;
  const int32_t *lane_base;
  int32_t *fin; float *fwd; int64_t *off; int32_t *regn; float *nexp; int32_t *reg_start; int32_t *regs; int32_t regs_cap;
  int *cursor;
  int64_t tcap;
};
__global__ void pack_survivors_kernel(const PackArgs a)
{
  const int l = (int) blockIdx.y;
  const int nfin = a.counters[(size_t) l * kLaneCounters + 4];
  if (a.counters[(size_t) l * kLaneCounters + 12] != 0) return;
  const int32_t *reg_l = a.reg_out + (size_t) l * (size_t) a.cap * (kRegionCap * 3 + 2);
  for (int i = (int) (blockIdx.x * blockDim.x + threadIdx.x); i < nfin; i += (int) (gridDim.x * blockDim.x)) {
    const int64_t t = (int64_t) a.lane_base[l] + i;
    if (t >= a.tcap) return;
    a.fin[t] = a.list_fin[(size_t) l * a.slot_pitch + i];
    a.fwd[t] = a.fwd_by_item[(size_t) l * a.slot_pitch + i];
    a.off[t] = a.xmx_off[(size_t) l * a.cap + i];
    const int n = reg_l[(size_t) a.cap * kRegionCap * 3 + i];
    a.regn[t] = n;
    a.nexp[t] = reinterpret_cast<const float *>(reg_l)[(size_t) a.cap * (kRegionCap * 3 + 1) + i];
    int start = -1;
    if (n > 0) {
      const int r0 = atomicAdd(a.cursor, n);
      if (r0 + n <= a.regs_cap) {
        start = r0;
        const int32_t *src = reg_l + (size_t) i * kRegionCap * 3;
        for (int z = 0; z < n * 3; ++z) a.regs[(size_t) r0 * 3 + z] = src[z];
      }
    }
    a.reg_start[t] = start;
  }
}

__global__ void __launch_bounds__(1024) lane_base_kernel(const int *counters, int nq, int32_t *lane_base, int *cursor)
{
  __shared__ int part[1024];
  const int t = (int) threadIdx.x, per = (nq + 1023) / 1024;
  auto count_of = [&](int l) { return counters[(size_t) l * kLaneCounters + 12] != 0 ? 0 : counters[(size_t) l * kLaneCounters + 4]; };
  int sum = 0;
  for (int i = 0; i < per; ++i) { const int l = t * per + i; if (l < nq) sum += count_of(l); }
  part[t] = sum;
  __syncthreads();
  if (t == 0) {
    int run = 0;
    for (int i = 0; i < 1024; ++i) { const int v = part[i]; part[i] = run; run += v; }
    *cursor = 0;
  }
  __syncthreads();
  int run = part[t];
  for (int i = 0; i < per; ++i) { const int l = t * per + i; if (l < nq) { lane_base[l] = run; run += count_of(l); } }
}

struct PackLayout { size_t o_base, o_cursor, o_off, o_fin, o_fwd, o_regn, o_nexp, o_start, o_regs, o_stage, bytes; int64_t regs_cap; };
static PackLayout pack_layout(int nq, int64_t T, bool scan_mode, int64_t nslots)
{
  PackLayout p{};
  p.regs_cap = std::max<int64_t>(8 * T, 4096);
  p.o_base = 0; p.o_cursor = (size_t) nq * 4; p.o_off = (p.o_cursor + 4 + 7) & ~(size_t) 7;
  p.o_fin = p.o_off + (size_t) T * 8; p.o_fwd = p.o_fin + (size_t) T * 4; p.o_regn = p.o_fwd + (size_t) T * 4; p.o_nexp = p.o_regn + (size_t) T * 4;
  p.o_start = p.o_nexp + (size_t) T * 4; p.o_regs = p.o_start + (size_t) T * 4; p.o_stage = p.o_regs + (size_t) p.regs_cap * 12;
  p.bytes = p.o_stage + (scan_mode ? (size_t) nq * (size_t) nslots : 0);
  return p;
}

static int64_t longest_rows(const p7x_seqdb *db, int64_t count)
{
  int64_t rows = 0;
  count = std::min<int64_t>(count, db->nslots);
  for (int64_t sl = 0; sl < count; ++sl) rows += (int64_t) db->h_len[db->h_order[sl]] + 1;
  return rows;
}

static int fill_survivor_args(CascadeRun &r, int first, int n, bool retry, int nfin)
{
  const p7x_seqdb *db = r.db; Workspace *ws = r.ws.get(); DeviceCtx *ctx = r.ctx;
  int64_t want_cap = std::min<int64_t>(db->nslots, std::max<int64_t>(4096, db->nslots / 64));
// ... 14 lines not shown
    const size_t items = lanes * (size_t) want;
    if ((st = off.reserve(ctx, items * 8)) != P7X_OK || (st = reg.reserve(ctx, items * (kRegionCap * 3 + 2) * 4)) != P7X_OK ||
        (st = bck.reserve(ctx, items * 4)) != P7X_OK) return st;
    have = want;
    return (int) P7X_OK;
  };
  if (!retry) st = grow_survivors(ws->xmx_off, ws->reg_out, ws->bck_sc, ws->fin_cap, (size_t) ws->nlanes, want_cap);
  else st = grow_survivors(ws->rt_xmx_off, ws->rt_reg_out, ws->rt_bck_sc, ws->rt_cap, 1, want_cap);
  if (st != P7X_OK) return st;
  const int64_t cap = retry ? ws->rt_cap : ws->fin_cap;
  for (int l = first; l < first + n; ++l) {
    const Profile &p = r.lm[l].om->p; const DevProfile *dp = r.lm[l].dp;
    LaneArgs &la = ws->h_args.as<LaneArgs>()[l];
    const StageBufs b = ws->lane_bufs(l);
    int64_t *xmx_off = retry ? ws->rt_xmx_off.as<int64_t>() : ws->xmx_off.as<int64_t>() + (size_t) l * cap;
    int32_t *reg_out = retry ? ws->rt_reg_out.as<int32_t>() : ws->reg_out.as<int32_t>() + (size_t) l * cap * (kRegionCap * 3 + 2);
    float *bck_sc = retry ? ws->rt_bck_sc.as<float>() : ws->bck_sc.as<float>() + (size_t) l * cap;
    LayoutArgs lay{};
    lay.nfin_ptr = &b.counters[4]; lay.list_fin = b.list_fin; lay.slot_len = db->d_slot_len; lay.xmx_off = xmx_off;
    lay.cap_items = (int) std::min<int64_t>(cap, INT_MAX); lay.cap_floats = (long long) ws->xmx_cap; lay.cursor = ws->cursor();
    lay.flags = &b.counters[12];
    la.lay = lay;
    WaveSeqArgs a = ws_args(p, dp, db, ctx);
    a.trans = dp->fwd_trans; a.emis = dp->fwd_emis; a.list = b.list_fin; a.nlist_ptr = &b.counters[4];
    a.nlist = (int) std::min<int64_t>(cap, retry ? std::max(nfin, 1) : std::max(r.est_fin, 1));
    a.out_sc = b.fwd_by_item; a.xmx = ws->xmx_f.as<float>(); a.xmx_off = xmx_off;
    a.abort_flag = &b.counters[12];
    la.rows = a;
    a.out_sc = bck_sc; a.xmx = ws->xmx_b.as<float>(); a.fwd_xmx = ws->xmx_f.as<float>();
    la.bck = a;
    RegionArgs ra{};
    ra.nitems_ptr = &b.counters[4]; ra.abort_flag = &b.counters[12];
    ra.list = b.list_fin; ra.slot_len = db->d_slot_len; ra.fx = ws->xmx_f.as<float>(); ra.bx = ws->xmx_b.as<float>();
    ra.xmx_off = xmx_off; ra.scratch = ws->xmx_s.as<float>();
    ra.out_regs = reg_out; ra.out_n = reg_out + (size_t) cap * kRegionCap * 3;
    ra.out_nexpected = reinterpret_cast<float *>(ra.out_n + cap);
    ra.guard = (r.cfg.oa_guard > 0.0f && !r.cfg.long_targets && debug_opt(OPT_HOST_ORDER) <= 0) ? 2.0e-5f : 0.0f;
    if (debug_opt(OPT_REGION_GUARD_PPM) >= 0 && !r.cfg.long_targets) ra.guard = 1.0e-6f * (float) debug_opt(OPT_REGION_GUARD_PPM);
    la.reg = ra;
  }
  return P7X_OK;
}

static int launch_survivor_passes(CascadeRun &r, const LaneClass &c, hipStream_t s, bool retry, bool record_events)
{
  Workspace *ws = r.ws.get(); DeviceCtx *ctx = r.ctx;
  const int64_t cap = retry ? ws->rt_cap : ws->fin_cap;
  int st = P7X_OK;
  hipLaunchKernelGGL(layout_rows_kernel, dim3(1, (unsigned) c.n), dim3(256), 0, s, lane_run(ws, &LaneArgs::lay, c.first, c.n).ref());
  P7X_HIP(hipGetLastError());
  if ((st = class_wave(c, ws, &LaneArgs::rows, false, ctx, s)) != P7X_OK) return st;
  if (record_events) P7X_HIP(hipEventRecord(ws->ev[5], s));
  if ((st = class_wave(c, ws, &LaneArgs::bck, true, ctx, s)) != P7X_OK) return st;
  {
    const int64_t items = std::min<int64_t>(cap, retry ? cap : std::max(r.est_fin, 1));
    const unsigned gx = lane_grid((items + 3) / 4, ctx->num_cu * 4, c.n);
    hipLaunchKernelGGL(regions_kernel, dim3(gx, (unsigned) c.n), dim3(256), 0, s, lane_run(ws, &LaneArgs::reg, c.first, c.n).ref());
    P7X_HIP(hipGetLastError());
  }
  if (record_events) P7X_HIP(hipEventRecord(ws->ev[6], s));
  return P7X_OK;
}

static bool fwd_grouped(const p7x_seqdb *db) { return debug_opt(OPT_FWD_GROUPED) > 0 && db->ngroups > 256 && debug_opt(OPT_STAGE_MERGE) <= 0; }

static int class_cascade(CascadeRun &r, const LaneClass &c, hipStream_t s, bool record_events, bool chain_msv, bool msv_by_tier = false)
{
  const p7x_seqdb *db = r.db; Workspace *ws = r.ws.get(); DeviceCtx *ctx = r.ctx;
  int st = P7X_OK;
  if (chain_msv) {
    std::lock_guard<std::mutex> lk(ctx->msv_mu);
    if (ctx->msv_last >= 0) P7X_HIP(hipStreamWaitEvent(s, ctx->msv_done[ctx->msv_last], 0));
    if (record_events) P7X_HIP(hipEventRecord(ws->ev[0], s));
    if ((st = class_msv(c, r.lm, ctx, ws, s)) != P7X_OK) return st;
    if (record_events) P7X_HIP(hipEventRecord(ws->ev[7], s));
    ctx->msv_last = (ctx->msv_last + 1) & 1;
    P7X_HIP(hipEventRecord(ctx->msv_done[ctx->msv_last], s));
  } else {
    if (record_events) P7X_HIP(hipEventRecord(ws->ev[0], s));
    if ((st = msv_by_tier ? class_msv_rest(c, r.lm, ctx, ws, s) : class_msv(c, r.lm, ctx, ws, s)) != P7X_OK) return st;
    if (record_events) P7X_HIP(hipEventRecord(ws->ev[7], s));
  }
  const ArgRef dec = lane_run(ws, &LaneArgs::dec, c.first, c.n).ref();
  hipLaunchKernelGGL(decide_msv_kernel, dim3((unsigned) ((db->nslots + 255) / 256), (unsigned) c.n), dim3(256), 0, s, dec);
  if (record_events) P7X_HIP(hipEventRecord(ws->ev[1], s));
  hipLaunchKernelGGL(bias_kernel, dim3(lane_grid((r.est_bias + 63) / 64, ctx->num_cu * 4, c.n), (unsigned) c.n), dim3(64), 0, s, dec);
  {
    const unsigned nchunks = (unsigned) ((db->nslots + kCompactChunk - 1) / kCompactChunk);
    const ArgRef cmp = lane_run(ws, &LaneArgs::cmp, c.first, c.n).ref();
    hipLaunchKernelGGL(vit_compact_count_kernel, dim3(nchunks, (unsigned) c.n), dim3(256), 0, s, cmp);
    hipLaunchKernelGGL(vit_compact_write_kernel, dim3(nchunks, (unsigned) c.n), dim3(256), 0, s, cmp);
  }
  if (record_events) P7X_HIP(hipEventRecord(ws->ev[2], s));
  if ((st = class_viterbi(c, r.lm, ctx, ws, s)) != P7X_OK) return st;
  hipLaunchKernelGGL(decide_vit_kernel, dim3(lane_grid((r.est_vit + 255) / 256, ctx->num_cu, c.n), (unsigned) c.n), dim3(256), 0, s, dec);
  if (record_events) P7X_HIP(hipEventRecord(ws->ev[3], s));
  if (fwd_grouped(db) && r.lm[c.first].dp->fwdgT > 0) {
    if ((st = fwdg_launch(lane_run(ws, &LaneArgs::fwd, c.first, c.n), ctx->num_cu, s)) != P7X_OK) return st;
  } else if ((st = class_wave(c, ws, &LaneArgs::fwd, false, ctx, s)) != P7X_OK) return st;
  hipLaunchKernelGGL(decide_fwd_kernel, dim3(lane_grid((r.est_fwd + 255) / 256, ctx->num_cu, c.n), (unsigned) c.n), dim3(256), 0, s, dec);
  P7X_HIP(hipGetLastError());
  if (record_events) P7X_HIP(hipEventRecord(ws->ev[4], s));
  return launch_survivor_passes(r, c, s, false, record_events);
}

struct CascadeRun;
struct PackLayout;
static int queue_pack(CascadeRun &r, const PackLayout &lay, int64_t T, const int32_t *lane_base, int max_nfin);

static int staged_cascade(CascadeRun &r, const std::vector<LaneClass> &classes, hipStream_t s, int nside, const std::vector<int> &run_of)
{
  const p7x_seqdb *db = r.db; Workspace *ws = r.ws.get(); DeviceCtx *ctx = r.ctx;
  const int nq = (int) r.lm.size();
  constexpr int kStreams = Workspace::kSide + 1;
  int st = P7X_OK;
  auto stream_of = [&](size_t n) -> hipStream_t {
    int turn = (int) (n % (size_t) kStreams);
    if ((n / (size_t) kStreams) & 1) turn = kStreams - 1 - turn;
    turn = std::min(turn, nside);
    return turn == 0 ? s : ws->side[turn - 1];
  };
  auto fork = [&]() -> int {
    P7X_HIP(hipEventRecord(ws->ev_fork, s));
    for (int k = 0; k < nside; ++k) P7X_HIP(hipStreamWaitEvent(ws->side[k], ws->ev_fork, 0));
    return P7X_OK;
  };
  auto join = [&]() -> int {
    for (int k = 0; k < nside; ++k) {
      P7X_HIP(hipEventRecord(ws->ev_join[k], ws->side[k]));
      P7X_HIP(hipStreamWaitEvent(s, ws->ev_join[k], 0));
    }
    return P7X_OK;
  };
  auto runs_by = [&](auto same) {
    std::vector<LaneClass> out;
    for (const LaneClass &c : classes) {
      if (!out.empty() && same(out.back(), c)) out.back().n += c.n;
      else out.push_back(c);
    }
    std::reverse(out.begin(), out.end());
    return out;
  };
  P7X_HIP(hipEventRecord(ws->ev[0], s));
  for (size_t n = 0; n < classes.size(); ++n) {
    const size_t c = classes.size() - 1 - n;
    hipStream_t cs = stream_of(n);
    if (run_of[c] >= 0) P7X_HIP(hipStreamWaitEvent(cs, ws->ev_tier[run_of[c]], 0));
    if ((st = run_of[c] >= 0 ? class_msv_rest(classes[c], r.lm, ctx, ws, cs) : class_msv(classes[c], r.lm, ctx, ws, cs)) != P7X_OK) return st;
  }
  if ((st = join()) != P7X_OK) return st;
  P7X_HIP(hipEventRecord(ws->ev[7], s));
  const ArgRef dec = lane_run(ws, &LaneArgs::dec, 0, nq).ref();
  hipLaunchKernelGGL(decide_msv_kernel, dim3((unsigned) ((db->nslots + 255) / 256), (unsigned) nq), dim3(256), 0, s, dec);
  P7X_HIP(hipEventRecord(ws->ev[1], s));
  hipLaunchKernelGGL(bias_kernel, dim3(lane_grid((r.est_bias + 63) / 64, ctx->num_cu * 4, nq), (unsigned) nq), dim3(64), 0, s, dec);
  {
    const unsigned nchunks = (unsigned) ((db->nslots + kCompactChunk - 1) / kCompactChunk);
    const ArgRef cmp = lane_run(ws, &LaneArgs::cmp, 0, nq).ref();
    hipLaunchKernelGGL(vit_compact_count_kernel, dim3(nchunks, (unsigned) nq), dim3(256), 0, s, cmp);
    hipLaunchKernelGGL(vit_compact_write_kernel, dim3(nchunks, (unsigned) nq), dim3(256), 0, s, cmp);
  }
  P7X_HIP(hipGetLastError());
  P7X_HIP(hipEventRecord(ws->ev[2], s));
  if ((st = fork()) != P7X_OK) return st;
  {
    const std::vector<LaneClass> runs = runs_by([](const LaneClass &a, const LaneClass &b) { return a.vit_key == b.vit_key && a.C == b.C && a.vit_long == b.vit_long; });
    for (size_t n = 0; n < runs.size(); ++n)
      if ((st = class_viterbi(runs[n], r.lm, ctx, ws, stream_of(n))) != P7X_OK) return st;
  }
  if ((st = join()) != P7X_OK) return st;
  hipLaunchKernelGGL(decide_vit_kernel, dim3(lane_grid((r.est_vit + 255) / 256, ctx->num_cu, nq), (unsigned) nq), dim3(256), 0, s, dec);
  P7X_HIP(hipEventRecord(ws->ev[3], s));
  const std::vector<LaneClass> by_C = runs_by([](const LaneClass &a, const LaneClass &b) { return a.C == b.C; });
  if ((st = fork()) != P7X_OK) return st;
  for (size_t n = 0; n < by_C.size(); ++n)
    if ((st = class_wave(by_C[n], ws, &LaneArgs::fwd, false, ctx, stream_of(n))) != P7X_OK) return st;
  if ((st = join()) != P7X_OK) return st;
  hipLaunchKernelGGL(decide_fwd_kernel, dim3(lane_grid((r.est_fwd + 255) / 256, ctx->num_cu, nq), (unsigned) nq), dim3(256), 0, s, dec);
  P7X_HIP(hipEventRecord(ws->ev[4], s));
  hipLaunchKernelGGL(layout_rows_kernel, dim3(1, (unsigned) nq), dim3(256), 0, s, lane_run(ws, &LaneArgs::lay, 0, nq).ref());
  P7X_HIP(hipGetLastError());
  P7X_HIP(hipEventRecord(ws->ev[5], s));
  if ((st = fork()) != P7X_OK) return st;
  for (size_t n = 0; n < by_C.size(); ++n) {
    hipStream_t cs = stream_of(n);
    if ((st = class_wave(by_C[n], ws, &LaneArgs::rows, false, ctx, cs)) != P7X_OK) return st;
    if ((st = class_wave(by_C[n], ws, &LaneArgs::bck, true, ctx, cs)) != P7X_OK) return st;
  }
  if ((st = join()) != P7X_OK) return st;
  {
    const int64_t items = std::min<int64_t>(ws->fin_cap, std::max(r.est_fin, 1));
    const unsigned gx = lane_grid((items + 3) / 4, ctx->num_cu * 4, nq);
    hipLaunchKernelGGL(regions_kernel, dim3(gx, (unsigned) nq), dim3(256), 0, s, lane_run(ws, &LaneArgs::reg, 0, nq).ref());
    P7X_HIP(hipGetLastError());
  }
  P7X_HIP(hipEventRecord(ws->ev[6], s));
  return P7X_OK;
}

static int cascade_enqueue(CascadeRun &r)
{
  const p7x_pipeline_cfg &cfg = r.cfg; const p7x_seqdb *db = r.db;
  int st = get_ctx(db->device, &r.ctx);
  if (st != P7X_OK) return st;
  DeviceCtx *ctx = r.ctx;
  const int nq = (int) r.oms.size();
  r.query_of.resize(nq);
  for (int i = 0; i < nq; ++i) r.query_of[i] = i;
  std::stable_sort(r.query_of.begin(), r.query_of.end(), [&](int a, int b) { return r.oms[a]->p.M < r.oms[b]->p.M; });
  r.lane_of.resize(nq); r.lm.resize(nq);
  for (int l = 0; l < nq; ++l) { r.lane_of[r.query_of[l]] = l; r.lm[l].om = r.oms[r.query_of[l]]; }
  const bool debug = debug_opt(OPT_TRACE_FINISH) > 0;
  auto tlast = std::chrono::steady_clock::now();
  std::string dbg;
  auto tick = [&](const char *what) {
    if (!debug) return;
    const auto now = std::chrono::steady_clock::now();
    char buf[64]; std::snprintf(buf, sizeof buf, " %s %.2f", what, std::chrono::duration<double, std::milli>(now - tlast).count());
    dbg += buf; tlast = now;
  };
  {
    std::vector<const p7x_oprofile *> lane_oms((size_t) nq);
    std::vector<DevProfile *> dps((size_t) nq, nullptr);
    for (int l = 0; l < nq; ++l) lane_oms[(size_t) l] = r.lm[l].om;
    if ((st = get_dev_profiles(lane_oms.data(), nq, ctx, dps.data(), cfg.host_threads)) != P7X_OK) return st;
    for (int l = 0; l < nq; ++l) r.lm[l].dp = dps[(size_t) l];
  }
  tick("images");
  if (db->nslots == 0 || nq == 0) return P7X_OK;
  for (int l = 0; l < nq; ++l)
    if (r.lm[l].dp->vitC <= 0) { set_error("model too long for the device kernels: M > 8192 nodes (the reference has no limit, plan7.pyx:6156-6262; the lane-chunk layout of the wave-per-target kernels ends at 128 nodes per lane -- no Pfam-A model comes near it)"); return P7X_EINVAL; }
  std::vector<LaneClass> classes;
  if ((st = lane_classes(r.lm, db, ctx, classes)) != P7X_OK) return st;
  if ((st = get_workspace(ctx, db->nslots, nq, r.ws)) != P7X_OK) return st;
  tick("classes+workspace");
  Workspace *ws = r.ws.get();
  hipStream_t s = ws->stream;
  r.queued = true;
  const ListEstimates est = estimate_lists(cfg, db->nslots);
  r.est_bias = est.bias; r.est_vit = est.vit; r.est_fwd = est.fwd; r.est_fin = est.fin;
  std::vector<int> nlong_of((size_t) nq, 0);
  std::vector<int64_t> vit_long_of((size_t) nq, 0);
  for (const LaneClass &c : classes) for (int l = c.first; l < c.first + c.n; ++l) { nlong_of[(size_t) l] = c.nlong; vit_long_of[(size_t) l] = c.vit_long; }
  for (int l = 0; l < nq; ++l) {
    const Profile &p = r.lm[l].om->p; const DevProfile *dp = r.lm[l].dp;
    LaneArgs &la = ws->h_args.as<LaneArgs>()[l];
    const StageBufs b = ws->lane_bufs(l);
    DecideArgs d{};
    d.b = b; d.p = make_params(p, cfg);
    d.slot_len = db->d_slot_len; d.tjb_tab = ctx->lt.tjb; d.null1_tab = ctx->lt.null1; d.xwmove_tab = ctx->lt.xwmove; d.logtab = ctx->lt.logtab;
    d.dsq = db->d_dsq; d.slot_off = db->d_slot_off; d.eo = dp->bias_eo; d.nslots = db->nslots;
    la.dec = d;
    fill_msv_args(la, p, dp, db, ctx, b, nlong_of[(size_t) l]);
    const int64_t vit_long = vit_long_of[(size_t) l];
    fill_vit_args(la, p, dp, db, ctx, b.list_vit, est.vit, &b.counters[2], b.xC,
                  vit_long > 0 ? &b.counters[13] : nullptr, (int) std::min<int64_t>(vit_long, (int64_t) est.vit));
    CompactArgs ca{};
    ca.stage = b.stage; ca.list = b.list_vit; ca.chunk_cnt = ws->chunk_cnt.as<int>() + (size_t) l * (size_t) ws->chunks_per_lane; ca.counters = b.counters;
    ca.nslots = db->nslots; ca.long_slots = vit_long;
    la.cmp = ca;
    WaveSeqArgs a = ws_args(p, dp, db, ctx);
    a.trans = dp->fwd_trans; a.emis = dp->fwd_emis; a.list = b.list_fwd; a.nlist = est.fwd; a.nlist_ptr = &b.counters[3];
    a.out_sc = b.fwd_by_item;
    if (fwd_grouped(db) && dp->fwdgT > 0) { a.trans = dp->fwdg_trans; a.emis = dp->fwdg_emis; a.C = dp->fwdgT * 256 + dp->fwdgC; a.counter = &b.counters[5]; }
    la.fwd = a;
  }
  tick("args");
  if ((st = fill_survivor_args(r, 0, nq, false, 0)) != P7X_OK) return st;
  tick("survivor_args");
  if ((st = upload_args(ws, 0, nq, s)) != P7X_OK) return st;
  tick("upload");
  P7X_HIP(hipMemsetAsync(ws->counters.as<int>(), 0, ws->counters_bytes(), s));
  ws->ntier_runs = 0;
  if (classes.size() == 1) {
    const bool fills_device = (db->nslots / 64) * (int64_t) nq >= (int64_t) ctx->num_cu * 8;
    if ((st = class_cascade(r, classes[0], s, true, fills_device)) != P7X_OK) return st;
  } else {
    P7X_HIP(hipEventRecord(ws->ev_fork, s));
    const int nside = std::min<int>((int) classes.size() - 1, Workspace::kSide);
    for (int k = 0; k < nside; ++k) P7X_HIP(hipStreamWaitEvent(ws->side[k], ws->ev_fork, 0));
    constexpr int kStreamsAll = Workspace::kSide + 1;
    std::vector<int> run_of(classes.size(), -1);
    if (msv_tiers_enabled()) {
      int nruns = 0, last_tier = -1;
      for (size_t c = 0; c < classes.size(); ++c) {
        const LaneClass &k = classes[c];
        if (k.msv_key < 0) { last_tier = -1; continue; }
        const int tier = msv_tier(r.lm[k.first].dp->msvR, r.lm[k.first].dp->msvK);
        if (tier != last_tier) { if (nruns == Workspace::kTierRuns) break; ++nruns; last_tier = tier; }
        run_of[c] = nruns - 1;
      }
      for (int run = nruns - 1; run >= 0; --run) {
        size_t a = 0; while (run_of[a] != run) ++a;
        size_t b = a; while (b + 1 < classes.size() && run_of[b + 1] == run) ++b;
        const int first = classes[a].first, n = classes[b].first + classes[b].n - first;
        const int turn = (kStreamsAll - 1 - run) % kStreamsAll;
        hipStream_t ts = turn == 0 ? s : ws->side[std::min(turn, nside) - 1];
        const LaneClass &k = classes[a];
        P7X_HIP(hipEventRecord(ws->ev_tier0[run], ts));
        if ((st = msv_tier_launch(msv_tier(r.lm[k.first].dp->msvR, r.lm[k.first].dp->msvK), lane_run(ws, &LaneArgs::msv, first, n), ctx->num_cu, ts)) != P7X_OK) return st;
        P7X_HIP(hipEventRecord(ws->ev_tier[run], ts));
        ws->tier_lanes[run] = n; ws->tier_nodes[run] = 0;
        for (int l = first; l < first + n; ++l) ws->tier_nodes[run] += r.lm[l].om->p.M;
      }
      ws->ntier_runs = nruns;
    }
    const int sm = debug_opt(OPT_STAGE_MERGE);
    const bool staged = sm >= 0 ? sm != 0 : db->ngroups <= 256;
    if (staged) {
      if ((st = staged_cascade(r, classes, s, nside, run_of)) != P7X_OK) return st;
    } else
    for (size_t n = 0; n < classes.size(); ++n) {
      const size_t c = classes.size() - 1 - n;
      constexpr int kStreams = Workspace::kSide + 1;
      int turn = (int) (n % (size_t) kStreams);
      if ((n / (size_t) kStreams) & 1) turn = kStreams - 1 - turn;
      hipStream_t cs = turn == 0 ? s : ws->side[turn - 1];
      if (run_of[c] >= 0) P7X_HIP(hipStreamWaitEvent(cs, ws->ev_tier[run_of[c]], 0));
      if ((st = class_cascade(r, classes[c], cs, n == 0, false, run_of[c] >= 0)) != P7X_OK) return st;
    }
    for (int k = 0; k < nside; ++k) {
      P7X_HIP(hipEventRecord(ws->ev_join[k], ws->side[k]));
      P7X_HIP(hipStreamWaitEvent(s, ws->ev_join[k], 0));
    }
  }
  ws->early_T_cap = 0;
  if (debug_opt(OPT_EARLY_PACK) > 0 || (debug_opt(OPT_EARLY_PACK) < 0 && db->ngroups <= 256)) {
    int64_t room = 1024;
    while (room < 16384 && room < 2 * ws->last_T) room *= 2;
    const int64_t kEarlyPack = debug_opt(OPT_EARLY_PACK) > 0 ? debug_opt(OPT_EARLY_PACK) : room;
    const PackLayout lay = pack_layout(nq, kEarlyPack, cfg.mode == P7X_SCAN_MODELS, db->nslots);
    if ((st = queue_pack(r, lay, kEarlyPack, nullptr, 2048)) != P7X_OK) return st;
    ws->early_T_cap = kEarlyPack;
  }
  P7X_HIP(hipMemcpyAsync(ws->h_counts.as<int>(), ws->counters.as<int>(), ws->counters_bytes(), hipMemcpyDeviceToHost, s));
  P7X_HIP(hipEventRecord(ws->ev_sync, s));
// ... 318 lines not shown
    for (int64_t sl = 0; sl < ns; ++sl) bias_filtersc[db->h_order[sl]] = h[sl];
  }
  return P7X_OK;
}

static int run_cascade(const p7x_pipeline_cfg &cfg, const p7x_oprofile *om, const p7x_seqdb *db, CascadeOut &out)
{
  CascadeRun r;
  r.cfg = cfg; r.oms.assign(1, om); r.db = db;
  int st = cascade_enqueue(r);
  if (st != P7X_OK) return st;
  std::vector<CascadeOut> outs;
  if ((st = cascade_collect(r, outs)) != P7X_OK) return st;
  out = std::move(outs[0]);
  return P7X_OK;
}

static int one_seq(const p7x_oprofile *om, int device, const uint8_t *dsq, int32_t L, int which, float *sc)
{
  if (!om || !dsq || !sc || L < 1) { set_error("bad arguments"); return P7X_EINVAL; }
  const int64_t off = 0; const int32_t len = L;
  p7x_seqdb *db = nullptr;
  int st = p7x_seqdb_create(device, om->p.abc_type, dsq, &off, &len, 1, &db);
  if (st != P7X_OK) return st;
  int32_t xJ = 0, xC = 0; float f = 0;
  const Profile &p = om->p;
  DeviceCtx *ctx = nullptr;
  get_ctx(device, &ctx);
  if (which == 0) {
    st = p7x_filters_batch(om, db, &xJ, nullptr, nullptr, nullptr);
    if (st == P7X_OK) {
      if (xJ < 0) { *sc = INFINITY; st = P7X_ERANGE; }
      else {
        const uint8_t tjb = unbiased_byteify(p.scale_b, logf(3.0f / (float) (L + 3)));
        float v = ((float) (xJ - tjb) - (float) p.base_b); v /= p.scale_b; v -= 3.0; *sc = v;
      }
    }
  } else if (which == 1) {
    st = p7x_filters_batch(om, db, nullptr, &xC, nullptr, nullptr);
    if (st == P7X_OK) {
      if (xC >= 32767) { *sc = INFINITY; st = P7X_ERANGE; }
      else if (xC > -32768) {
        const float pmove = 3.0f / ((float) L + 3.0f);
        float v = (float) xC + (float) wordify(p.scale_w, logf(pmove)) - (float) p.base_w; v /= p.scale_w; v -= 3.0; *sc = v;
      } else *sc = -INFINITY;
    }
  } else if (which == 2) {
    st = p7x_filters_batch(om, db, nullptr, nullptr, &f, nullptr);
    *sc = f;
    if (st == P7X_OK && (std::isnan(f) || std::isinf(f))) st = P7X_ERANGE;
  } else {
    p7x_pipeline_cfg cfg; p7x_pipeline_cfg_default(&cfg);
    cfg.do_max = 1;
    cfg.host_regions = 1;
    CascadeOut out;
    st = run_cascade(cfg, om, db, out);
    if (st == P7X_OK) {
      if (out.fin_slots.size() != 1) { set_error("backward: sequence did not reach the Backward stage"); st = P7X_EINVAL; }
      else {
        double tot = 0.0;
        for (int i = 1; i <= L; ++i) { const float s = out.bck_xmx[(size_t) i * 6 + 5]; if (s > 1.0f) tot += std::log((double) s); }
        *sc = (float) (tot + std::log((double) out.bck_xmx[1]));
      }
    }
  }
  p7x_seqdb_destroy(db);
  return st;
}

int p7x_msv_filter(const p7x_oprofile *om, int device, const uint8_t *dsq, int32_t L, float *sc) { return one_seq(om, device, dsq, L, 0, sc); }
int p7x_vit_filter(const p7x_oprofile *om, int device, const uint8_t *dsq, int32_t L, float *sc) { return one_seq(om, device, dsq, L, 1, sc); }
int p7x_fwd_parser(const p7x_oprofile *om, int device, const uint8_t *dsq, int32_t L, float *sc) { return one_seq(om, device, dsq, L, 2, sc); }
int p7x_bck_parser(const p7x_oprofile *om, int device, const uint8_t *dsq, int32_t L, float *sc) { return one_seq(om, device, dsq, L, 3, sc); }

struct p7x_pending {
  p7x_pipeline_cfg cfg{};
  const p7x_seqdb *db = nullptr;
  CascadeRun run;
  std::vector<CascadeOut> co;
  bool waited = false;
  std::chrono::steady_clock::time_point t0;
};

int p7x_search_batch_enqueue(const p7x_pipeline_cfg *cfg, const p7x_oprofile *const *oms, size_t nq, const float *bg_f,
                             const p7x_seqdb *db, p7x_pending **out)
{
  if (!cfg || !oms || !db || !out || nq == 0 || nq > 4096) { set_error("p7x_search_batch_enqueue: bad arguments"); return P7X_EINVAL; }
  *out = nullptr;
  auto pd = std::make_unique<p7x_pending>();
  pd->t0 = std::chrono::steady_clock::now();
  for (size_t q = 0; q < nq; ++q) {
    if (!oms[q]) { set_error("p7x_search_batch_enqueue: null profile"); return P7X_EINVAL; }
    const Profile &p = oms[q]->p;
    if (p.abc_type != db->abc_type) { set_error("profile and target block have different alphabets"); return P7X_EINVAL; }
    if (bg_f) for (int x = 0; x < p.K; ++x) if (bg_f[x] != p.bgf[x]) {
      set_error("the pipeline's background differs from the one the optimized profile was configured with"); return P7X_EINVAL; }
    if (cfg->use_bit_cutoffs) {
      const int i = cfg->use_bit_cutoffs == P7X_BITCUT_GA ? P7X_GA1 : (cfg->use_bit_cutoffs == P7X_BITCUT_TC ? P7X_TC1 : P7X_NC1);
      if (p.cutoff[i] == P7X_CUTOFF_UNSET || p.cutoff[i + 1] == P7X_CUTOFF_UNSET) { set_error("model is missing the requested bit score cutoffs"); return P7X_EINVAL; }
    }
  }
  pd->cfg = *cfg; pd->db = db;
  pd->run.cfg = *cfg; pd->run.oms.assign(oms, oms + nq); pd->run.db = db;
  const int st = cascade_enqueue(pd->run);
  if (st != P7X_OK) return st;
  *out = pd.release();
  return P7X_OK;
}

int p7x_debug_log_of_float(int device, const float *in, float *out, size_t n)
{
  if (!in || !out) { set_error("p7x_debug_log_of_float: bad arguments"); return P7X_EINVAL; }
  if (n == 0) return P7X_OK;
  DeviceCtx *ctx = nullptr;
  int st = get_ctx(device, &ctx);
  if (st != P7X_OK) return st;
  DeviceBuf b_in, b_out;
  if ((st = b_in.reserve(ctx, n * 4)) != P7X_OK || (st = b_out.reserve(ctx, n * 4)) != P7X_OK) return st;
  float *d_in = b_in.as<float>(), *d_out = b_out.as<float>();
  P7X_HIP(hipMemcpy(d_in, in, n * 4, hipMemcpyHostToDevice));
  hipLaunchKernelGGL(log_of_float_kernel, dim3(1024), dim3(256), 0, ctx->stream, d_in, d_out, n, ctx->lt.logtab);
  P7X_HIP(hipGetLastError());
  P7X_HIP(hipStreamSynchronize(ctx->stream));
  P7X_HIP(hipMemcpy(out, d_out, n * 4, hipMemcpyDeviceToHost));
  return P7X_OK;
}

int p7x_search_batch_raw(const p7x_pipeline_cfg *cfg, const p7x_oprofile *const *oms, size_t nq, const float *bg_f,
                         const p7x_seqdb *db, int32_t *xJ, int32_t *xC, uint8_t *stage)
{
  p7x_pending *pd = nullptr;
  int st = p7x_search_batch_enqueue(cfg, oms, nq, bg_f, db, &pd);
  if (st != P7X_OK) return st;
  std::unique_ptr<p7x_pending> owner(pd);
  CascadeRun &r = pd->run;
  const int64_t n = db->n, ns = db->nslots;
  if (xJ) std::fill(xJ, xJ + nq * (size_t) n, 0);
  if (xC) std::fill(xC, xC + nq * (size_t) n, INT32_MIN);
  if (stage) std::fill(stage, stage + nq * (size_t) n, (uint8_t) 0);
  if (!r.queued || ns == 0) return P7X_OK;
  Workspace *ws = r.ws.get();
  P7X_HIP(hipStreamSynchronize(ws->stream));
  std::vector<int16_t> hj((size_t) ns); std::vector<int32_t> hl((size_t) ns), hc((size_t) ns); std::vector<uint8_t> hs((size_t) ns);
  for (size_t q = 0; q < nq; ++q) {
    const int l = r.lane_of[q];
    const StageBufs b = ws->lane_bufs(l);
    int counters[kLaneCounters];
    P7X_HIP(hipMemcpy(counters, b.counters, sizeof(counters), hipMemcpyDeviceToHost));
    if (xJ) {
      P7X_HIP(hipMemcpy(hj.data(), b.xJ, (size_t) ns * 2, hipMemcpyDeviceToHost));
      for (int64_t sl = 0; sl < ns; ++sl) xJ[q * (size_t) n + (size_t) db->h_order[sl]] = hj[(size_t) sl];
    }
    if (xC) {
      const int nv = counters[2];
      P7X_HIP(hipMemcpy(hl.data(), b.list_vit, (size_t) nv * 4, hipMemcpyDeviceToHost));
      P7X_HIP(hipMemcpy(hc.data(), b.xC, (size_t) nv * 4, hipMemcpyDeviceToHost));
      for (int it = 0; it < nv; ++it) xC[q * (size_t) n + (size_t) db->h_order[hl[(size_t) it]]] = hc[(size_t) it];
    }
    if (stage) {
      P7X_HIP(hipMemcpy(hs.data(), b.stage, (size_t) ns, hipMemcpyDeviceToHost));
      for (int64_t sl = 0; sl < ns; ++sl) stage[q * (size_t) n + (size_t) db->h_order[sl]] = hs[(size_t) sl];
    }
  }
  return p7x_search_block_wait(pd);
}

int p7x_search_block_enqueue(const p7x_pipeline_cfg *cfg, const p7x_oprofile *om, const float *bg_f, const p7x_seqdb *db,
                             p7x_pending **out)
{
  if (!cfg || !om || !db || !out) { set_error("p7x_search_block_enqueue: bad arguments"); return P7X_EINVAL; }
  return p7x_search_batch_enqueue(cfg, &om, 1, bg_f, db, out);
}

int p7x_search_block_wait(p7x_pending *pd)
{
  if (!pd) { set_error("p7x_search_block_wait: bad arguments"); return P7X_EINVAL; }
  if (pd->waited) return P7X_OK;
  const int st = cascade_collect(pd->run, pd->co);
  if (st != P7X_OK) return st;
  pd->waited = true;
  const double wall = std::chrono::duration<double, std::milli>(std::chrono::steady_clock::now() - pd->t0).count();
  for (auto &c : pd->co) c.ms[6] = wall;
  return P7X_OK;
}

size_t p7x_pending_nqueries(const p7x_pending *pd) { return pd ? pd->run.oms.size() : 0; }

int p7x_search_block_begin(const p7x_pipeline_cfg *cfg, const p7x_oprofile *om, const float *bg_f, const p7x_seqdb *db,
                           p7x_pending **out)
{
  if (!out) { set_error("p7x_search_block_begin: bad arguments"); return P7X_EINVAL; }
  p7x_pending *pd = nullptr;
  int st = p7x_search_block_enqueue(cfg, om, bg_f, db, &pd);
  if (st != P7X_OK) return st;
  if ((st = p7x_search_block_wait(pd)) != P7X_OK) { delete pd; *out = nullptr; return st; }
  *out = pd;
  return P7X_OK;
}

int p7x_search_batch_finish(p7x_pending *pd, const char *const *names, const char *const *accs, const char *const *descs,
                            p7x_tophits **outs)
{
  if (!pd || !outs) { set_error("p7x_search_batch_finish: bad arguments"); return P7X_EINVAL; }
  std::unique_ptr<p7x_pending> owner(pd);
  const size_t nq = pd->run.oms.size();
  for (size_t q = 0; q < nq; ++q) outs[q] = nullptr;
  if (!pd->waited) { const int wst = p7x_search_block_wait(pd); if (wst != P7X_OK) return wst; }
  const p7x_seqdb *db = pd->db;
  HostTargets tg;
  tg.n = db->n; tg.nres = db->nres; tg.len = db->h_len.data(); tg.off = db->h_off.data(); tg.dsq = db->h_dsq.data();
  const auto t1 = std::chrono::steady_clock::now();
  std::vector<std::vector<int32_t>> targets(nq);
  std::vector<DeviceRegions> dr(nq);
  std::vector<FinishItem> items(nq);
  bool any_device = false;
  for (size_t q = 0; q < nq; ++q) {
    const p7x_oprofile *om = pd->run.oms[q]; CascadeOut &co = pd->co[q];
    targets[q].resize(co.fin_slots.size());
    for (size_t i = 0; i < targets[q].size(); ++i) targets[q][i] = db->h_order[co.fin_slots[i]];
    FinishItem &it = items[q];
    it.om = om; it.targets = &targets[q]; it.fwdsc = co.fwdsc.data();
    it.near = &co.near;
    it.fwd_xmx = co.fwd_xmx.data(); it.bck_xmx = co.bck_xmx.data(); it.xmx_off = co.xmx_off.data();
    it.counts[0] = (uint64_t) co.counts[1]; it.counts[1] = (uint64_t) co.counts[8]; it.counts[2] = (uint64_t) co.counts[3]; it.counts[3] = (uint64_t) co.counts[4];
    it.ms = co.ms; it.nms = 12;
    if (!co.have_xmx && !targets[q].empty()) { dr[q].n = co.reg_n.data(); dr[q].regs = co.regs.data(); dr[q].nexpected = co.nexpected.data(); dr[q].cap = kRegionCap;
      dr[q].start = co.reg_start.empty() ? nullptr : co.reg_start.data(); it.regions = &dr[q]; }
    it.device_envelopes = !pd->cfg.host_envelopes && !targets[q].empty();
    any_device = any_device || it.device_envelopes;
  }
  int st = P7X_OK;
  std::unique_ptr<EnvelopeScorer> scorer, scorer2;
  std::unique_ptr<EnsembleRunner> ensembles;
  if (any_device) {
    DeviceCtx *ctx = nullptr;
    if ((st = get_ctx(db->device, &ctx)) != P7X_OK) return st;
    scorer = make_device_envelope_scorer(ctx, db, pd->cfg.oa_guard);
    if (!pd->cfg.host_ensembles) {
      ensembles = make_device_ensemble_runner(ctx, db, pd->cfg.ens_guard);
      scorer2 = make_device_envelope_scorer(ctx, db, pd->cfg.oa_guard);
    } else if (device_clustered(pd->cfg.host_threads)) scorer2 = make_device_envelope_scorer(ctx, db, pd->cfg.oa_guard);
  }
  const auto t2 = std::chrono::steady_clock::now();
  if ((st = host_finish_batch(pd->cfg, items, tg, names, accs, descs, outs, scorer.get(), scorer2.get(), ensembles.get())) != P7X_OK) return st;
  const auto t3 = std::chrono::steady_clock::now();
  const double stage2 = std::chrono::duration<double, std::milli>(t3 - t1).count();
  for (size_t q = 0; q < nq; ++q) {
// ... 64 lines not shown
```

pyhmmer_amd/csrc/p7x_profile.cpp:

```cpp
#include "p7x_internal.hpp"
#include <atomic>
#include <algorithm>
#include <cmath>
#include <cstdio>
#include <cstring>
#include <memory>
#include <mutex>

namespace p7x {
std::atomic<int> g_debug_opt[OPT_COUNT];
static const bool g_debug_opt_ready = [] { for (auto &o : g_debug_opt) o.store(-1); return true; }();
int debug_opt(int which) { return (which >= 0 && which < OPT_COUNT) ? g_debug_opt[which].load(std::memory_order_relaxed) : -1; }


static thread_local std::string g_err;
void set_error(const std::string &msg) { g_err = msg; }

static Alphabet make_alphabet(int type)
{
  Alphabet a{};
  a.type = type;
  std::memset(a.degen, 0, sizeof(a.degen));
  if (type == P7X_AMINO) {
    a.K = 20; a.Kp = 29; a.sym = "ACDEFGHIKLMNPQRSTVWY-BJZOUX*~";
// ... 147 lines not shown
  p.scale_b = 3.0 / kLog2;
  p.base_b = 190;
  p.bias_b = unbiased_byteify(p.scale_b, -1.0 * mx);
  p.rb.assign((size_t) p.Kp * (M + 1), 255);
  for (int x = 0; x < p.Kp; ++x)
    for (int k = 1; k <= M; ++k)
      p.rb[(size_t) x * (M + 1) + k] = biased_byteify(p.scale_b, p.bias_b, p.msc[(size_t) x * (M + 1) + k]);
  p.tbm_b = unbiased_byteify(p.scale_b, logf(2.0f / ((float) M * (float) (M + 1))));
  p.tec_b = unbiased_byteify(p.scale_b, logf(0.5f));
  p.tjb_b = unbiased_byteify(p.scale_b, logf(3.0f / (float) (p.L + 3)));
}

static void convert_viterbi(Profile &p)
{
  const int M = p.M;
  p.scale_w = 500.0 / kLog2;
  p.base_w = 12000;
  p.rw.assign((size_t) p.Kp * (M + 1), -32768);
  for (int x = 0; x < p.Kp; ++x)
    for (int k = 1; k <= M; ++k) p.rw[(size_t) x * (M + 1) + k] = wordify(p.scale_w, p.msc[(size_t) x * (M + 1) + k]);
  p.tw.assign((size_t) NTRANS * (M + 1), -32768);
  auto W = [&](int t, int k) -> int16_t & { return p.tw[(size_t) t * (M + 1) + k]; };
  auto cap = [](int16_t v, int16_t maxval) { return v <= maxval ? v : maxval; };
  for (int k = 1; k <= M; ++k) {
    W(tBM, k) = cap(wordify(p.scale_w, p.tsc[(size_t) (k - 1) * 8 + gBM]), 0);
    W(tMM, k) = cap(wordify(p.scale_w, p.tsc[(size_t) (k - 1) * 8 + gMM]), 0);
    W(tIM, k) = cap(wordify(p.scale_w, p.tsc[(size_t) (k - 1) * 8 + gIM]), 0);
    W(tDM, k) = cap(wordify(p.scale_w, p.tsc[(size_t) (k - 1) * 8 + gDM]), 0);
    if (k < M) {
      W(tMD, k) = cap(wordify(p.scale_w, p.tsc[(size_t) k * 8 + gMD]), 0);
      W(tMI, k) = cap(wordify(p.scale_w, p.tsc[(size_t) k * 8 + gMI]), 0);
      W(tII, k) = cap(wordify(p.scale_w, p.tsc[(size_t) k * 8 + gII]), -1);
      W(tDD, k) = wordify(p.scale_w, p.tsc[(size_t) k * 8 + gDD]);
    }
  }
  p.xw[XE][LOOP] = wordify(p.scale_w, p.xsc[XE][LOOP]);
  p.xw[XE][MOVE] = wordify(p.scale_w, p.xsc[XE][MOVE]);
  for (int s : {XN, XC, XJ}) { p.xw[s][MOVE] = wordify(p.scale_w, p.xsc[s][MOVE]); p.xw[s][LOOP] = 0; }
  p.ncj_roundoff = 0.0f;
  int bound = -32768;
  for (int k = 2; k < M - 1; ++k) {
    int dd = (int) wordify(p.scale_w, p.tsc[(size_t) k * 8 + gDD]);
    dd += (int) wordify(p.scale_w, p.tsc[(size_t) (k + 1) * 8 + gDM]);
    dd -= (int) wordify(p.scale_w, p.tsc[(size_t) (k + 1) * 8 + gBM]);
    if (dd > bound) bound = dd;
  }
  p.ddbound_w = (int16_t) bound;
}

static void convert_forward(Profile &p)
{
  const int M = p.M;
  p.rf_.assign((size_t) p.Kp * (M + 1), 0.0f);
  for (int x = 0; x < p.Kp; ++x)
    for (int k = 1; k <= M; ++k) p.rf_[(size_t) x * (M + 1) + k] = sse_expf(p.msc[(size_t) x * (M + 1) + k]);
  p.tf.assign((size_t) NTRANS * (M + 1), 0.0f);
  auto F = [&](int t, int k) -> float & { return p.tf[(size_t) t * (M + 1) + k]; };
  for (int k = 1; k <= M; ++k) {
    F(tBM, k) = sse_expf(p.tsc[(size_t) (k - 1) * 8 + gBM]);
    F(tMM, k) = sse_expf(p.tsc[(size_t) (k - 1) * 8 + gMM]);
    F(tIM, k) = sse_expf(p.tsc[(size_t) (k - 1) * 8 + gIM]);
    F(tDM, k) = sse_expf(p.tsc[(size_t) (k - 1) * 8 + gDM]);
    if (k < M) {
      F(tMD, k) = sse_expf(p.tsc[(size_t) k * 8 + gMD]);
      F(tMI, k) = sse_expf(p.tsc[(size_t) k * 8 + gMI]);
      F(tII, k) = sse_expf(p.tsc[(size_t) k * 8 + gII]);
      F(tDD, k) = sse_expf(p.tsc[(size_t) k * 8 + gDD]);
    }
  }
  for (int s = 0; s < 4; ++s) for (int m = 0; m < 2; ++m) p.xf[s][m] = expf(p.xsc[s][m]);
}

}

using namespace p7x;

extern "C" {

int p7x_abi_version(void) { return P7X_ABI_VERSION; }

int p7x_debug_set_option(const char *name, int value)
{
  static const char *const names[p7x::OPT_COUNT] = { "small_block", "vit_wave", "msv_exact", "msv_long_groups", "msv_blocks_per_cu", "env_workspace_gb",
                                                     "device_clustered", "trace_finish", "trace_longtarget", "trace_envelope", "host_profile", "ssv_kernel", "msv_f16", "ens_lds_kb", "ens_fail", "msv_tiers", "stage_merge", "early_pack", "host_order", "vit_long_cut", "fwd_grouped", "region_guard_ppm", "msv_k8", "msv_lane_blocks", "host_align", "align_workspace_gb" };
  if (!name) { p7x::set_error("p7x_debug_set_option: no name"); return P7X_EINVAL; }
  for (int i = 0; i < p7x::OPT_COUNT; ++i)
    if (std::strcmp(name, names[i]) == 0) { p7x::g_debug_opt[i].store(value); return P7X_OK; }
  p7x::set_error(std::string("p7x_debug_set_option: unknown option ") + name);
  return P7X_EINVAL;
}

const char *p7x_last_error(void) { return g_err.c_str(); }

void p7x_expf_neg(const double *in, float *out, size_t n)
{
  for (size_t i = 0; i < n; ++i) out[i] = std::isinf(in[i]) ? 0.0f : expf((float) (-1.0 * in[i]));
}

int p7x_hmm_max_length(const p7x_hmm_view *h, double beta, int32_t *out)
{
  if (!h || !out || h->M < 1 || !h->t || !(beta > 0.0)) { set_error("p7x_hmm_max_length: bad arguments"); return P7X_EINVAL; }
  const int M = h->M;
  if (M == 1) { *out = 1; return P7X_OK; }
  const float *t = h->t;
  auto T = [&](int k, int x) -> double { return (double) t[(size_t) k * 7 + x]; };
  std::vector<double> Mm(2 * (size_t) (M + 1), 0.0), I(2 * (size_t) (M + 1), 0.0), D(2 * (size_t) (M + 1), 0.0);
  auto at = [&](std::vector<double> &v, int k, int c) -> double & { return v[(size_t) c * (M + 1) + k]; };
  at(Mm, 1, 0) = 1.0;
  for (int k = 2; k <= M; ++k) at(D, k, 0) = T(k - 1, 2) * at(Mm, k - 1, 0) + T(k - 1, 6) * at(D, k - 1, 0);
  const int length_bound = 200000;
  for (int L = 2; L <= length_bound; ++L) {
    const int c = (L - 1) & 1, pc = L & 1;
    at(Mm, 1, c) = 0.0; at(D, 1, c) = 0.0;
    at(I, 1, c) = T(1, 1) * at(Mm, 1, pc) + T(1, 4) * at(I, 1, pc);
    double alive = at(I, 1, c);
    for (int k = 2; k <= M; ++k) {
      const double m = T(k - 1, 0) * at(Mm, k - 1, pc) + T(k - 1, 3) * at(I, k - 1, pc) + T(k - 1, 5) * at(D, k - 1, pc);
      const double i = k < M ? T(k, 1) * at(Mm, k, pc) + T(k, 4) * at(I, k, pc) : 0.0;
      at(Mm, k, c) = m; at(I, k, c) = i;
      at(D, k, c) = T(k - 1, 2) * at(Mm, k - 1, c) + T(k - 1, 6) * at(D, k - 1, c);
      alive += m + i;
    }
    if (alive < beta) { *out = L; return P7X_OK; }
  }
  set_error("p7x_hmm_max_length: no bound below 200000 residues");
  return P7X_ERANGE;
}

int p7x_oprofile_create(const p7x_hmm_view *h, const float *bg_f, int32_t L, p7x_oprofile **out)
{
  if (!h || !bg_f || !out || h->M < 1 || !h->t || !h->mat || !h->name) { set_error("p7x_oprofile_create: bad arguments"); return P7X_EINVAL; }
  if (h->abc_type != P7X_AMINO && h->abc_type != P7X_DNA && h->abc_type != P7X_RNA) { set_error("unknown alphabet"); return P7X_EINVAL; }
  flogsum_init();
  auto *om = new p7x_oprofile();
  Profile &p = om->p;
  const Alphabet &abc = Alphabet::get(h->abc_type);
  p.M = h->M; p.K = abc.K; p.Kp = abc.Kp; p.abc_type = h->abc_type; p.L = L; p.max_length = h->max_length;
  p.mode = 1;
  p.name = h->name;
  if (h->acc)  { p.acc = h->acc;   p.has_acc = true; }
  if (h->desc) { p.desc = h->desc; p.has_desc = true; }
  if (h->consensus) p.consensus = h->consensus;
  if (h->rf) p.rf = h->rf;
  if (h->mm) p.mm = h->mm;
  if (h->cs) p.cs = h->cs;
  std::memcpy(p.evparam, h->evparam, sizeof(p.evparam));
  std::memcpy(p.cutoff, h->cutoff, sizeof(p.cutoff));
  std::memset(p.compo, 0, sizeof(p.compo));
  if (h->compo) std::memcpy(p.compo, h->compo, sizeof(float) * p.K);
  std::memset(p.bgf, 0, sizeof(p.bgf));
  std::memcpy(p.bgf, bg_f, sizeof(float) * p.K);
  p.relent_mh = match_relent_sum(h->mat, bg_f, p.M, p.K);
  configure_generic(p, *h);
  convert_msv(p);
  convert_viterbi(p);
  convert_forward(p);
  attach_dev_cache(om);
  *out = om;
  return P7X_OK;
}

int p7x_oprofile_get_info(const p7x_oprofile *om, p7x_oprofile_info *o)
{
  if (!om || !o) return P7X_EINVAL;
  const Profile &p = om->p;
  std::memset(o, 0, sizeof(*o));
  o->M = p.M; o->K = p.K; o->Kp = p.Kp; o->abc_type = p.abc_type; o->L = p.L; o->max_length = p.max_length; o->mode = p.mode;
// ... 330 lines not shown
```

pyhmmer_amd/csrc/p7x_vitfwd.hip:

```cpp
#include "p7x_wave.hpp"

namespace p7x {

template <int C>
__global__ void __launch_bounds__(kWsBlock) vit_kernel(const ArgRef ref)
{
  extern __shared__ __attribute__((aligned(16))) unsigned char smem[];
  constexpr int Mpad = 64 * C;
  const WaveSeqArgs a = load_args<WaveSeqArgs>(ref);
  const int nlist = (a.abort_flag && *a.abort_flag) ? 0 : (a.nlist_ptr ? *a.nlist_ptr : a.nlist);
  if ((int) (blockIdx.x * (kWsBlock / 64)) >= nlist) return;
  constexpr bool EG = C > 32;
  uint4 *tr = reinterpret_cast<uint4 *>(smem);
  const short *em = EG ? reinterpret_cast<const short *>(a.emis) : reinterpret_cast<const short *>(smem + (size_t) Mpad * 16);
  {
    const uint4 *gt = reinterpret_cast<const uint4 *>(a.trans);
    for (int i = threadIdx.x; i < Mpad; i += kWsBlock) tr[i] = gt[i];
    if constexpr (!EG) {
      const uint4 *ge = reinterpret_cast<const uint4 *>(a.emis);
      uint4 *le = reinterpret_cast<uint4 *>(smem + (size_t) Mpad * 16);
      for (int i = threadIdx.x; i < a.nrows * Mpad / 8; i += kWsBlock) le[i] = ge[i];
    }
  }
  __syncthreads();
// ... 107 lines not shown
    const int tjbm = rfl((int) a.tjb_tab[L]) + a.tbm;
    int mm[C];
#pragma unroll unroll_c(C)
    for (int c = 0; c < C; ++c) mm[c] = 0;
    int xJ = 0, xEmax = 0;
    int xB = max(a.base - tjbm, 0);
    constexpr int kBlk = C <= 8 ? 16 : 1;
    for (int i0 = 0; i0 < L; i0 += 64) {
      const int nrow = min(64, L - i0);
      const uint32_t resid = (lane < nrow) ? sq[i0 + lane] : 0;
      for (int r0 = 0; r0 < nrow; r0 += kBlk) {
        if (kBlk == 1) {
          const int x = __builtin_amdgcn_readlane((int) resid, r0);
          const short *er = em + x * Mpad + lane;
          int mp = dpp_shr1(mm[C - 1], 0);
          int rowmax = kNegPad;
#pragma unroll unroll_c(C)
          for (int c = 0; c < C; ++c) {
            const int sv = max(mp, xB) + (int) er[c * 64];
            mp = mm[c];
            mm[c] = sv;
            rowmax = max(rowmax, sv);
          }
          const int xE = wave_max_i32(rowmax);
          xEmax = max(xEmax, xE);
          xJ = max(xJ, xE - a.tec);
          xB = max(max(a.base, xJ) - tjbm, 0);
          continue;
        }
        const int nb = min(kBlk, nrow - r0);
        int saved[C];
#pragma unroll unroll_c(C)
        for (int c = 0; c < C; ++c) saved[c] = mm[c];
        int blkmax = kNegPad;
        auto row_held = [&](int r) {
          const int x = __builtin_amdgcn_readlane((int) resid, r);
          const short *er = em + x * Mpad + lane;
          int mp = dpp_shr1(mm[C - 1], 0);
#pragma unroll unroll_c(C)
          for (int c = 0; c < C; ++c) {
            const int sv = max(mp, xB) + (int) er[c * 64];
            mp = mm[c];
            mm[c] = sv;
            blkmax = max(blkmax, sv);
          }
        };
        if (C <= 4 && nb == kBlk) {
#pragma unroll
          for (int rr = 0; rr < kBlk; ++rr) row_held(r0 + rr);
        } else if (C <= 12) {
#pragma unroll 4
          for (int rr = 0; rr < nb; ++rr) row_held(r0 + rr);
        } else {
#pragma unroll 2
          for (int rr = 0; rr < nb; ++rr) row_held(r0 + rr);
        }
        const int xEb = wave_max_i32(blkmax);
        if (xEb - a.tec <= max(a.base, xJ)) {
          xEmax = max(xEmax, xEb);
          xJ = max(xJ, xEb - a.tec);
          continue;
        }
#pragma unroll unroll_c(C)
        for (int c = 0; c < C; ++c) mm[c] = saved[c];
        for (int r = r0; r < r0 + nb; ++r) {
          const int x = __builtin_amdgcn_readlane((int) resid, r);
          const short *er = em + x * Mpad + lane;
          int mp = dpp_shr1(mm[C - 1], 0);
          int rowmax = kNegPad;
#pragma unroll unroll_c(C)
          for (int c = 0; c < C; ++c) {
            const int sv = max(mp, xB) + (int) er[c * 64];
            mp = mm[c];
            mm[c] = sv;
            rowmax = max(rowmax, sv);
          }
          const int xE = wave_max_i32(rowmax);
          xEmax = max(xEmax, xE);
          xJ = max(xJ, xE - a.tec);
          xB = max(max(a.base, xJ) - tjbm, 0);
        }
      }
    }
    if (lane == 0 && L > 0) a.out_xJ[slot] = (xEmax >= 255 - a.bias) ? (int16_t) -1 : (int16_t) xJ;
  }
}

typedef short s2v __attribute__((ext_vector_type(2)));
__device__ __forceinline__ s2v u2s(uint32_t u) { return __builtin_bit_cast(s2v, u); }
__device__ __forceinline__ uint32_t s2u(s2v v) { return __builtin_bit_cast(uint32_t, v); }
constexpr int kPkWaves = 16;
template <int C>
__global__ void __launch_bounds__(kPkWaves * 64) msv_wavepk_kernel(const ArgRef ref)
{
  extern __shared__ __attribute__((aligned(16))) unsigned char smem[];
  static_assert(C % 4 == 0, "pairs of pairs");
  constexpr int P = C / 2, P2 = C / 4;
  constexpr uint32_t kFloor = 0x80008000u;
  const MsvWaveArgs a = load_args<MsvWaveArgs>(ref);
  const int nlist = a.nslots;
  if ((int) (blockIdx.x * kPkWaves) >= nlist) return;
  {
    const uint4 *g = reinterpret_cast<const uint4 *>(a.emis_pk);
    uint4 *l = reinterpret_cast<uint4 *>(smem);
    for (int i = threadIdx.x; i < a.nrows * P * 64 / 4; i += kPkWaves * 64) l[i] = g[i];
  }
  __syncthreads();
  const int lane = threadIdx.x & 63;
  const uint2 *tab = reinterpret_cast<const uint2 *>(smem) + lane;
  const int wave0 = rfl((int) (blockIdx.x * kPkWaves + (threadIdx.x >> 6)));
  const int nwaves = (int) (gridDim.x * kPkWaves);
  for (int it = wave0; it < nlist; it += nwaves) {
    const int slot = it;
    const int L = rfl(a.slot_len[slot]);
    const unsigned long long off = (unsigned long long) a.slot_off[slot];
    const unsigned lo = (unsigned) rfl((int) (unsigned) off), hi = (unsigned) rfl((int) (unsigned) (off >> 32));
    const uint8_t *sq = a.dsq + (((unsigned long long) hi << 32) | lo);
    const int tjbm = rfl((int) a.tjb_tab[L]) + a.tbm;
    uint32_t mm[P];
#pragma unroll
    for (int j = 0; j < P; ++j) mm[j] = kFloor;
    int xJ = 0, xEmax = 0;
    int xB = max(a.base - tjbm, 0);
    auto row = [&](const uint2 (&ee)[P2], const s2v xBs, s2v &acc) {
      uint32_t left = (uint32_t) dpp_shr1((int) mm[P - 1], (int) kFloor);
#pragma unroll
      for (int j2 = 0; j2 < P2; ++j2) {
#pragma unroll
        for (int h = 0; h < 2; ++h) {
          const int j = 2 * j2 + h;
          const uint32_t cur = mm[j];
          const uint32_t mp = __builtin_amdgcn_alignbit(cur, left, 16);
          const s2v sv = __builtin_elementwise_add_sat(__builtin_elementwise_max(u2s(mp), xBs), u2s(h == 0 ? ee[j2].x : ee[j2].y));
          mm[j] = s2u(sv);
          acc = __builtin_elementwise_max(acc, sv);
          left = cur;
        }
      }
    };
    constexpr int kBlk = 8;
    for (int i0 = 0; i0 < L; i0 += 64) {
      const int nrow = min(64, L - i0);
      const uint32_t resid = (lane < nrow) ? sq[i0 + lane] : 0;
      auto load_e = [&](uint2 (&dst)[P2], int r) {
        const int x = __builtin_amdgcn_readlane((int) resid, r);
#pragma unroll
        for (int j2 = 0; j2 < P2; ++j2) dst[j2] = tab[(x * P2 + j2) * 64];
      };
      for (int r0 = 0; r0 < nrow; r0 += kBlk) {
        const int nb = min(kBlk, nrow - r0);
        const s2v xBs = u2s((uint32_t) ((xB - 32768) & 0xffff) * 0x00010001u);
        if (nb == kBlk) {
          uint32_t saved[P];
#pragma unroll
          for (int j = 0; j < P; ++j) saved[j] = mm[j];
          s2v acc = u2s(kFloor);
          uint2 ea[P2], eb[P2];
          load_e(ea, r0);
#pragma unroll
          for (int rr = 0; rr < kBlk; rr += 2) {
            load_e(eb, r0 + rr + 1);
            row(ea, xBs, acc);
            if (rr + 2 < kBlk) load_e(ea, r0 + rr + 2);
            row(eb, xBs, acc);
          }
          const int xEb = wave_max_i32(max((int) acc.x, (int) acc.y)) + 32768;
          if (xEb - a.tec <= max(a.base, xJ)) {
            xEmax = max(xEmax, xEb);
            xJ = max(xJ, xEb - a.tec);
            continue;
          }
#pragma unroll
          for (int j = 0; j < P; ++j) mm[j] = saved[j];
        }
        for (int r = r0; r < r0 + nb; ++r) {
          uint2 e1[P2];
          load_e(e1, r);
          s2v rowmax = u2s(kFloor);
          row(e1, u2s((uint32_t) ((xB - 32768) & 0xffff) * 0x00010001u), rowmax);
          const int xE = wave_max_i32(max((int) rowmax.x, (int) rowmax.y)) + 32768;
          xEmax = max(xEmax, xE);
          xJ = max(xJ, xE - a.tec);
          xB = max(max(a.base, xJ) - tjbm, 0);
        }
      }
    }
    if (lane == 0 && L > 0) a.out_xJ[slot] = (xEmax >= 255 - a.bias) ? (int16_t) -1 : (int16_t) xJ;
  }
}

template <int C, bool EG = false>
__global__ void __launch_bounds__(kWsBlock) fwd_kernel(const ArgRef ref)
{
  extern __shared__ __attribute__((aligned(16))) unsigned char smem[];
  constexpr int Mpad = 64 * C;
  const WaveSeqArgs a = load_args<WaveSeqArgs>(ref);
  const int nlist = (a.abort_flag && *a.abort_flag) ? 0 : (a.nlist_ptr ? *a.nlist_ptr : a.nlist);
  if ((int) (blockIdx.x * (kWsBlock / 64)) >= nlist) return;
  constexpr bool TG = C > 64;
  const float4 *tr = TG ? reinterpret_cast<const float4 *>(a.trans) : reinterpret_cast<const float4 *>(smem);
  const float *em = EG ? reinterpret_cast<const float *>(a.emis) : reinterpret_cast<const float *>(smem + (size_t) Mpad * 32);
  {
    if constexpr (!TG) {
      const float4 *gt = reinterpret_cast<const float4 *>(a.trans);
      float4 *lt = reinterpret_cast<float4 *>(smem);
      for (int i = threadIdx.x; i < 2 * Mpad; i += kWsBlock) lt[i] = gt[i];
    }
    if constexpr (!EG) {
      const float4 *ge = reinterpret_cast<const float4 *>(a.emis);
      float4 *le = reinterpret_cast<float4 *>(smem + (size_t) Mpad * 32);
      for (int i = threadIdx.x; i < a.nrows * Mpad / 4; i += kWsBlock) le[i] = ge[i];
    }
  }
  __syncthreads();
  const int lane = threadIdx.x & 63;

  P7X_WAVE_ITEMS(it) {
    const Item item = load_item(a, it);
    const int L = item.L;
    const uint8_t *sq = item.sq;
    float *xo = a.xmx ? a.xmx + a.xmx_off[it] : nullptr;
    const float pmove = (2.0f + 1.0f) / ((float) L + 2.0f + 1.0f), ploop = 1.0f - pmove;

    float mm[C], im[C], dm[C];
#pragma unroll unroll_c(C)
    for (int c = 0; c < C; ++c) mm[c] = im[c] = dm[c] = 0.0f;
    float ddprod = 1.0f;
#pragma unroll unroll_c(C)
    for (int c = 0; c < C; ++c) ddprod *= tr[2 * (c * 64 + lane) + 1].w;

    float xN = 1.0f, xB = pmove, xJ = 0.0f, xC = 0.0f, xE = 0.0f, totscale = 0.0f;
    if (xo && lane == 0) { xo[0] = 0.0f; xo[1] = 1.0f; xo[2] = 0.0f; xo[3] = xB; xo[4] = 0.0f; xo[5] = 1.0f; }
    for (int i0 = 0; i0 < L; i0 += 64) {
     const int nrow = min(64, L - i0);
     const uint32_t resid = (lane < nrow) ? sq[i0 + lane] : 0;
     for (int r = 0; r < nrow; ++r) {
      const int i = i0 + r;
      const int x = __builtin_amdgcn_readlane((int) resid, r);
      const float *er = em + x * Mpad + lane;
      float mp = dpp_shr1f(mm[C - 1], 0.0f), ip = dpp_shr1f(im[C - 1], 0.0f), dp = dpp_shr1f(dm[C - 1], 0.0f);
      float esum = 0.0f, dcarry = 0.0f;
      float tdd[C], tmd[C];
#pragma unroll unroll_c(C)
      for (int c = 0; c < C; ++c) {
        const F8 t = load_f8(tr, c * 64 + lane);
        float sv = xB * t.bm;
        sv = sv + mp * t.mm;
        sv = sv + ip * t.im;
        sv = sv + dp * t.dm;
        sv = sv * er[c * 64];
        esum = esum + sv;
        mp = mm[c]; ip = im[c]; dp = dm[c];
        im[c] = mp * t.mi + ip * t.ii;
        mm[c] = sv;
        tdd[c] = t.dd; tmd[c] = t.md;
      }
      float A = 0.0f;
#pragma unroll unroll_c(C)
      for (int c = 0; c < C; ++c) { dm[c] = A; A = mm[c] * tmd[c] + A * tdd[c]; }
      float sa = A, sp = ddprod;
      affine_scan_up(sa, sp);
      dcarry = dpp_shr1f(sa, 0.0f);
      {
        float w = dcarry;
#pragma unroll unroll_c(C)
        for (int c = 0; c < C; ++c) { dm[c] = dm[c] + w; esum = esum + dm[c]; w = w * tdd[c]; }
      }
      xE = wave_sum_f32(esum);
      xN = xN * ploop;
      xC = (xC * ploop) + (xE * a.xf_e_move);
// ... 303 lines not shown
```

Before: 23880.

## Fuse MSV pass decision into MSV kernels via precomputed per-length thresholds

```diff
diff --git a/include/p7x.h b/include/p7x.h
--- a/include/p7x.h
+++ b/include/p7x.h
@@ -184,6 +184,12 @@
                         int use_device, int32_t *ndom, int32_t *dom, int32_t dom_cap, float *n2, int32_t *status);
 int  p7x_search_batch_raw(const p7x_pipeline_cfg *cfg, const p7x_oprofile *const *oms, size_t nq, const float *bg_f,
                           const p7x_seqdb *db, int32_t *xJ, int32_t *xC, uint8_t *stage);
+int  p7x_debug_msv_decide(const p7x_pipeline_cfg *cfg, const p7x_oprofile *const *oms, size_t nq, const float *bg_f, const p7x_seqdb *db,
+                          int exact_all, int32_t *xJ, uint8_t *stage, int32_t *counters, int32_t *list_bias, float *usc);
+int  p7x_debug_msv_thresholds(const p7x_pipeline_cfg *cfg, const p7x_oprofile *om, int device, int16_t *thr, size_t n);
+int  p7x_debug_decide_msv(const p7x_pipeline_cfg *cfg, const p7x_oprofile *om, int device, const int32_t *L, const int32_t *xJ, size_t n,
+                          uint8_t *take, float *usc);
+int64_t p7x_debug_msv_tables(const p7x_oprofile *om, int device, uint32_t *tab_i16, uint32_t *tab_f16, size_t cap_words);
 
 int p7x_search_longtargets(const p7x_pipeline_cfg *cfg, const p7x_oprofile *om, int device,
                            const uint8_t *dsq, const int64_t *offsets, const int64_t *lengths, size_t n,
diff --git a/pyhmmer_amd/_lib.py b/pyhmmer_amd/_lib.py
--- a/pyhmmer_amd/_lib.py
+++ b/pyhmmer_amd/_lib.py
@@ -227,6 +227,10 @@
     "p7x_longtargets_release_resident": (C.c_int, [C.c_int, C.c_uint64]),
     "p7x_debug_ensemble": (C.c_int, [_VP, _VP, C.c_int64, C.c_int32, C.c_int32, C.c_uint32, C.c_int, _VP, _VP, C.c_int32, _VP, _VP]),
     "p7x_search_batch_raw": (C.c_int, [C.POINTER(PipelineCfg), C.POINTER(_VP), C.c_size_t, _VP, _VP, _VP, _VP, _VP]),
+    "p7x_debug_msv_decide": (C.c_int, [C.POINTER(PipelineCfg), C.POINTER(_VP), C.c_size_t, _VP, _VP, C.c_int, _VP, _VP, _VP, _VP, _VP]),
+    "p7x_debug_msv_thresholds": (C.c_int, [C.POINTER(PipelineCfg), _VP, C.c_int, _VP, C.c_size_t]),
+    "p7x_debug_decide_msv": (C.c_int, [C.POINTER(PipelineCfg), _VP, C.c_int, _VP, _VP, C.c_size_t, _VP, _VP]),
+    "p7x_debug_msv_tables": (C.c_int64, [_VP, C.c_int, _VP, _VP, C.c_size_t]),
     "p7x_search_longtargets": (C.c_int, [C.POINTER(PipelineCfg), _VP, C.c_int, _VP, _VP, _VP, C.c_size_t, _VP, _VP, _VP, C.POINTER(_VP)]),
     "p7x_ssv_longtarget_seeds": (C.c_int64, [C.POINTER(PipelineCfg), _VP, C.c_int, _VP, C.c_int64, C.c_int, _VP, C.c_size_t]),
     "p7x_forward_parser_exact": (C.c_int, [_VP, _VP, C.c_int32, C.POINTER(C.c_float)]),
diff --git a/pyhmmer_amd/csrc/p7x_device.hpp b/pyhmmer_amd/csrc/p7x_device.hpp
--- a/pyhmmer_amd/csrc/p7x_device.hpp
+++ b/pyhmmer_amd/csrc/p7x_device.hpp
@@ -55,6 +55,7 @@
   int M = 0, Kp = 0;
   int msvR = 0, msvK = 0, msvS = 0;
   uint32_t *msv_tab = nullptr;
+  uint32_t *msv_tab_h = nullptr;
   int16_t *msvw_emis = nullptr;
   uint32_t *msvw_pk = nullptr;
   int msvwC = 0, msvw_rows = kTabRows;
@@ -69,6 +70,9 @@
   float *fwdg_trans = nullptr, *fwdg_emis = nullptr;
   float *bias_eo = nullptr;
   std::shared_ptr<DeviceBuf> shared;
+  struct MsvThr { double F1; float mmu, mlambda, scale_b; int base_b; const int16_t *thr; std::shared_ptr<DeviceBuf> slab; };
+  std::mutex thr_mu;
+  std::vector<MsvThr> msv_thr;
 };
 
 int get_dev_profile(const p7x_oprofile *om, DeviceCtx *ctx, DevProfile **out);
diff --git a/pyhmmer_amd/csrc/p7x_devimage.hip b/pyhmmer_amd/csrc/p7x_devimage.hip
--- a/pyhmmer_amd/csrc/p7x_devimage.hip
+++ b/pyhmmer_amd/csrc/p7x_devimage.hip
@@ -42,6 +42,9 @@
     std::vector<uint32_t> tab;
     msv_build_tables(p, d->msvR, d->msvK, tab);
     img.add(&d->msv_tab, tab);
+    std::vector<uint32_t> tab_h;
+    msv_half_tables(tab, tab_h);
+    img.add(&d->msv_tab_h, tab_h);
   }
   d->vitC = vit_pick_C(p.M);
   if (d->vitC > 0) {
diff --git a/pyhmmer_amd/csrc/p7x_internal.hpp b/pyhmmer_amd/csrc/p7x_internal.hpp
--- a/pyhmmer_amd/csrc/p7x_internal.hpp
+++ b/pyhmmer_amd/csrc/p7x_internal.hpp
@@ -63,7 +63,7 @@
 void set_error(const std::string &msg);
 
 enum { OPT_SMALL_BLOCK = 0, OPT_VIT_WAVE, OPT_MSV_EXACT, OPT_MSV_LONG_GROUPS, OPT_MSV_BLOCKS_PER_CU, OPT_ENV_WORKSPACE_GB, OPT_DEVICE_CLUSTERED,
-       OPT_TRACE_FINISH, OPT_TRACE_LONGTARGET, OPT_TRACE_ENVELOPE, OPT_HOST_PROFILE, OPT_SSV_KERNEL, OPT_MSV_F16, OPT_ENS_LDS_KB, OPT_ENS_FAIL, OPT_MSV_TIERS, OPT_STAGE_MERGE, OPT_EARLY_PACK, OPT_HOST_ORDER, OPT_VIT_LONG_CUT, OPT_FWD_GROUPED, OPT_REGION_GUARD_PPM, OPT_MSV_K8, OPT_MSV_LANE_BLOCKS, OPT_HOST_ALIGN, OPT_ALIGN_WORKSPACE_GB, OPT_COUNT };
+       OPT_TRACE_FINISH, OPT_TRACE_LONGTARGET, OPT_TRACE_ENVELOPE, OPT_HOST_PROFILE, OPT_SSV_KERNEL, OPT_MSV_F16, OPT_ENS_LDS_KB, OPT_ENS_FAIL, OPT_MSV_TIERS, OPT_STAGE_MERGE, OPT_EARLY_PACK, OPT_HOST_ORDER, OPT_VIT_LONG_CUT, OPT_FWD_GROUPED, OPT_REGION_GUARD_PPM, OPT_MSV_K8, OPT_MSV_LANE_BLOCKS, OPT_HOST_ALIGN, OPT_ALIGN_WORKSPACE_GB, OPT_MSV_FUSED_DECIDE, OPT_COUNT };
 int debug_opt(int which);
 
 }
diff --git a/pyhmmer_amd/csrc/p7x_kernels.hpp b/pyhmmer_amd/csrc/p7x_kernels.hpp
--- a/pyhmmer_amd/csrc/p7x_kernels.hpp
+++ b/pyhmmer_amd/csrc/p7x_kernels.hpp
@@ -36,6 +36,59 @@
   if (b > want) b = want;
   return (unsigned) (b < 1 ? 1 : b);
 }
+
+struct MsvDecide {
+  const int16_t *thr;
+  uint8_t *stage;
+  float *usc;
+  int32_t *list_bias; int *counter_bias;
+  float scale_b;
+};
+struct MsvPassParams { double F1; float mmu, mlambda, reject_below, scale_b; int base_b; };
+#if defined(__HIPCC__)
+__device__ __forceinline__ double d_gumbel_surv(double x, double mu, double lambda)
+{
+  const double y = lambda * (x - mu), ey = -exp(-y);
+  return (fabs(ey) < 5e-9) ? -ey : 1 - exp(ey);
+}
+__device__ __forceinline__ float msv_usc(int xJ, int tjb, int base_b, float scale_b)
+{
+  if (xJ < 0) return __builtin_inff();
+  float usc = ((float) (xJ - tjb) - (float) base_b);
+  usc /= scale_b;
+  usc -= 3.0f;
+  return usc;
+}
+__device__ __forceinline__ bool msv_pass(float usc, float null1, const MsvPassParams &p)
+{
+  const float seq_score = (float) ((double) (usc - null1) / kLog2);
+  if (seq_score < p.reject_below) return false;
+  const double P = d_gumbel_surv((double) seq_score, (double) p.mmu, (double) p.mlambda);
+  return !(P > p.F1);
+}
+__device__ __forceinline__ void wave_append(int *counter, int32_t *list, bool take, int32_t value)
+{
+  const unsigned long long mask = __ballot(take);
+  if (mask == 0) return;
+  const int lane = (int) (threadIdx.x & 63);
+  const int leader = __ffsll((long long) mask) - 1;
+  int base = 0;
+  if (lane == leader) base = atomicAdd(counter, __popcll(mask));
+  base = __shfl(base, leader);
+  if (take) list[base + __popcll(mask & ((1ull << lane) - 1ull))] = value;
+}
+__device__ __forceinline__ void msv_decide(const MsvDecide &d, bool mine, int slot, int L, int xJ, int tjb, int base_b)
+{
+  bool take = false;
+  if (mine) {
+    take = xJ < 0 || xJ >= (int) d.thr[L];
+    d.stage[slot] = take ? 1 : 0;
+    if (take) d.usc[slot] = msv_usc(xJ, tjb, base_b, d.scale_b);
+  }
+  wave_append(d.counter_bias, d.list_bias, take, (int32_t) slot);
+}
+#endif
+int msv_thr_launch(const MsvPassParams *d_params, int n, const uint8_t *tjb_tab, const float *null1_tab, int16_t *thr, hipStream_t st);
 
 struct MsvArgs {
   const uint32_t *tab;
@@ -52,7 +105,11 @@
   int *amb_count; int *amb_groups; int *counter2;
   const int *group_list; const int *group_count;
   int R;
-};
+  const uint32_t *tab_h;
+  MsvDecide dec;
+  int exact_all;
+};
+void msv_half_tables(const std::vector<uint32_t> &tab, std::vector<uint32_t> &out);
 int  msv_pick(int M, int *K);
 int  msv_stride(int R, int K);
 void msv_build_tables(const Profile &p, int R, int K, std::vector<uint32_t> &out);
@@ -110,6 +167,7 @@
   const uint8_t *dsq; const int64_t *slot_off; const int32_t *slot_len; const uint8_t *tjb_tab;
   int nslots, base, bias, tec, tbm;
   int16_t *out_xJ;
+  MsvDecide dec;
 };
 int msv_wave_launch(const ArgRun<MsvWaveArgs> &a, int num_cu, hipStream_t st);
 
diff --git a/pyhmmer_amd/csrc/p7x_msv.hip b/pyhmmer_amd/csrc/p7x_msv.hip
--- a/pyhmmer_amd/csrc/p7x_msv.hip
+++ b/pyhmmer_amd/csrc/p7x_msv.hip
@@ -1,3 +1,4 @@
+#include <algorithm>
 #include <cstdlib>
 #include <iterator>
 #include <map>
@@ -35,10 +36,16 @@
 { return as_s2(__builtin_elementwise_maximum(__builtin_elementwise_maximum(as_h2(a), as_h2(b)), as_h2(c))); }
 __device__ __forceinline__ s2 h_splat(int units)
 { const _Float16 x = (_Float16) ((float) units * (1.0f / 256.0f)); h2 r; r.x = x; r.y = x; return as_s2(r); }
-__device__ __forceinline__ uint32_t h_of_i16_pair(uint32_t w)
-{
-  const int lo = max((int) (short) (w & 0xffffu), -512), hi = max((int) (short) (w >> 16), -512);
-  return __builtin_bit_cast(uint32_t, __builtin_amdgcn_cvt_pkrtz((float) lo * (1.0f / 256.0f), (float) hi * (1.0f / 256.0f)));
+static uint32_t h_of_i16_pair(uint32_t w)
+{
+  const int lo = std::max((int) (short) (w & 0xffffu), -512), hi = std::max((int) (short) (w >> 16), -512);
+  const _Float16 l = (_Float16) ((float) lo * (1.0f / 256.0f)), h = (_Float16) ((float) hi * (1.0f / 256.0f));
+  return (uint32_t) __builtin_bit_cast(uint16_t, l) | ((uint32_t) __builtin_bit_cast(uint16_t, h) << 16);
+}
+void msv_half_tables(const std::vector<uint32_t> &tab, std::vector<uint32_t> &out)
+{
+  out.resize(tab.size());
+  for (size_t i = 0; i < tab.size(); ++i) out[i] = h_of_i16_pair(tab[i]);
 }
 
 
@@ -250,7 +257,7 @@
   extern __shared__ __attribute__((aligned(16))) uint32_t lds[];
   constexpr int S = msv_row_stride_c(R, K), Rs = msv_lane_stride_c(R, K), BLK = msv_block_c(K);
   const MsvArgs a = load_args<MsvArgs>(ref);
-  const int nitems = (a.group_list ? *a.group_count : a.ngroups - a.group_first) * K;
+  const int nitems = a.group_list ? *a.group_count : (a.ngroups - a.group_first) * K;
   if (nitems <= 0 || *a.counter >= nitems) return;
   {
     constexpr int n4 = (msv_parities_c(K) * kTabRows * S) / 4;
@@ -268,8 +275,8 @@
     if (lane == 0) item = atomicAdd(a.counter, 1);
     item = __builtin_amdgcn_readfirstlane(item);
     if (item >= nitems) break;
-    const int gi = item / K;
-    const MsvItem<K> it(a.group_list ? __builtin_amdgcn_readfirstlane(a.group_list[gi]) : gi + a.group_first, item % K, lane);
+    const int id = a.group_list ? __builtin_amdgcn_readfirstlane(a.group_list[item]) : item + a.group_first * K;
+    const MsvItem<K> it(id / K, id % K, lane);
 
     const int slot = it.g * 64 + it.t;
     const int L = a.slot_len[slot];
@@ -298,9 +305,11 @@
       }
       cur = nxt;
     }
-    if (L > 0 && it.h == 0) {
-      const int xe = xEmax.x;
-      a.out_xJ[slot] = (xe >= 255 - a.bias) ? (int16_t) -1 : (int16_t) xJ.x;
+    const int xres = ((int) xEmax.x >= 255 - a.bias) ? -1 : (int) xJ.x;
+    if (L > 0 && it.h == 0) a.out_xJ[slot] = (int16_t) xres;
+    if (a.dec.thr) {
+      const bool mine = L > 0 && it.h == 0 && (a.group_list == nullptr || a.dec.stage[slot] == 255);
+      msv_decide(a.dec, mine, slot, L, xres, (int) a.tjb_tab[L], a.base);
     }
   }
 }
@@ -314,13 +323,9 @@
   if (*a.counter >= nitems) return;
   {
     constexpr int n4 = (msv_parities_c(K) * kTabRows * S) / 4;
-    const uint4 *src = reinterpret_cast<const uint4 *>(a.tab);
+    const uint4 *src = reinterpret_cast<const uint4 *>(H ? a.tab_h : a.tab);
     uint4 *dst = reinterpret_cast<uint4 *>(lds);
-    for (int i = threadIdx.x; i < n4; i += BLK) {
-      uint4 w = src[i];
-      if constexpr (H) { w.x = h_of_i16_pair(w.x); w.y = h_of_i16_pair(w.y); w.z = h_of_i16_pair(w.z); w.w = h_of_i16_pair(w.w); }
-      dst[i] = w;
-    }
+    for (int i = threadIdx.x; i < n4; i += BLK) dst[i] = src[i];
   }
   __syncthreads();
 
@@ -402,9 +407,21 @@
       cur = nxt;
     }
     fold(target_max<K, H>(mx(accA, accB)));
-    const bool ambiguous = (L > 0) && (xJ == F0) && !(xEmax >= 255 - a.bias);
-    if (L > 0 && it.h == 0) a.out_xJ[slot] = (xEmax >= 255 - a.bias) ? (int16_t) -1 : (int16_t) xJ;
-    if (__any(ambiguous) && lane == 0) { const int idx = atomicAdd(a.amb_count, 1); a.amb_groups[idx] = it.g; }
+    const bool over = xEmax >= 255 - a.bias;
+    const bool ambiguous = (L > 0) && (xJ == F0) && !over;
+    if (L > 0 && it.h == 0) a.out_xJ[slot] = over ? (int16_t) -1 : (int16_t) xJ;
+    bool redo = ambiguous;
+    if (a.dec.thr) {
+      int slot_e = slot, L_e = L;
+      asm volatile("" : "+v"(slot_e), "+v"(L_e));
+      const int thr = L_e > 0 ? (int) a.dec.thr[L_e] : 32767;
+      const bool open = ambiguous && F0 >= thr;
+      redo = open || (ambiguous && a.exact_all != 0);
+      const bool mine = L_e > 0 && it.h == 0 && !open;
+      msv_decide(a.dec, mine, slot_e, L_e, over ? -1 : xJ, tjbm - a.tbm, a.base);
+      if (open && it.h == 0) a.dec.stage[slot_e] = 255;
+    }
+    if (__any(redo) && lane == 0) { const int idx = atomicAdd(a.amb_count, 1); a.amb_groups[idx] = it.g * K + item % K; }
   }
 }
 
diff --git a/pyhmmer_amd/csrc/p7x_pipeline.hip b/pyhmmer_amd/csrc/p7x_pipeline.hip
--- a/pyhmmer_amd/csrc/p7x_pipeline.hip
+++ b/pyhmmer_amd/csrc/p7x_pipeline.hip
@@ -31,24 +31,8 @@
   int M;
 };
 
-__device__ __forceinline__ double d_gumbel_surv(double x, double mu, double lambda)
-{
-  const double y = lambda * (x - mu), ey = -exp(-y);
-  return (fabs(ey) < 5e-9) ? -ey : 1 - exp(ey);
-}
 __device__ __forceinline__ double d_exp_surv(double x, double mu, double lambda) { return x < mu ? 1.0 : exp(-lambda * (x - mu)); }
 
-__device__ __forceinline__ void wave_append(int *counter, int32_t *list, bool take, int32_t value)
-{
-  const unsigned long long mask = __ballot(take);
-  if (mask == 0) return;
-  const int lane = (int) (threadIdx.x & 63);
-  const int leader = __ffsll((long long) mask) - 1;
-  int base = 0;
-  if (lane == leader) base = atomicAdd(counter, __popcll(mask));
-  base = __shfl(base, leader);
-  if (take) list[base + __popcll(mask & ((1ull << lane) - 1ull))] = value;
-}
 __device__ __forceinline__ void wave_count(int *counter, bool take)
 {
   const unsigned long long mask = __ballot(take);
@@ -62,31 +46,50 @@
   int64_t nslots;
 };
 
+__device__ __forceinline__ MsvPassParams pass_params(const StageParams &p)
+{ return MsvPassParams{ p.F1, p.mmu, p.mlambda, p.msv_reject_below, p.scale_b, p.base_b }; }
+
 __global__ void decide_msv_kernel(const ArgRef ref)
 {
   const DecideArgs a = load_args<DecideArgs>(ref);
-  const StageBufs &b = a.b; const StageParams &p = a.p;
+  const StageBufs &b = a.b;
+  const MsvPassParams pp = pass_params(a.p);
   const int64_t s = (int64_t) blockIdx.x * blockDim.x + threadIdx.x;
   bool take = false;
   if (s < a.nslots) {
     const int L = a.slot_len[s];
-    const int xJ = b.xJ[s];
-    float usc;
-    if (xJ < 0) usc = __builtin_inff();
-    else {
-      usc = ((float) (xJ - (int) a.tjb_tab[L]) - (float) p.base_b);
-      usc /= p.scale_b;
-      usc -= 3.0f;
-    }
+    const float usc = msv_usc(b.xJ[s], (int) a.tjb_tab[L], pp.base_b, pp.scale_b);
     b.usc[s] = usc;
-    const float seq_score = (float) ((double) (usc - a.null1_tab[L]) / kLog2);
-    if (!(seq_score < p.msv_reject_below)) {
-      const double P = d_gumbel_surv((double) seq_score, (double) p.mmu, (double) p.mlambda);
-      take = !(P > p.F1);
-    }
+    take = msv_pass(usc, a.null1_tab[L], pp);
     b.stage[s] = take ? 1 : 0;
   }
   wave_append(&b.counters[1], b.list_bias, take, (int32_t) s);
+}
+
+__global__ void __launch_bounds__(256) msv_thr_kernel(const MsvPassParams *params, const uint8_t *tjb_tab, const float *null1_tab, int16_t *thr)
+{
+  const int L = (int) (blockIdx.x * blockDim.x + threadIdx.x);
+  if (L > kMaxL) return;
+  const MsvPassParams pp = params[blockIdx.y];
+  const int tjb = (int) tjb_tab[L];
+  const float null1 = null1_tab[L];
+  auto pass = [&](int xJ) { return msv_pass(msv_usc(xJ, tjb, pp.base_b, pp.scale_b), null1, pp); };
+  int lo = 0, hi = 256;
+  while (lo < hi) {
+    const int mid = (lo + hi) >> 1;
+    if (pass(mid)) hi = mid; else lo = mid + 1;
+  }
+  const bool ok = (lo >= 256 || pass(lo)) && (lo == 0 || !pass(lo - 1)) && (lo >= 255 || pass(lo + 1));
+  if (!ok) { lo = 0; while (lo < 256 && !pass(lo)) ++lo; }
+  thr[(size_t) blockIdx.y * (kMaxL + 1) + L] = lo >= 256 ? (int16_t) 32767 : (int16_t) lo;
+}
+
+int msv_thr_launch(const MsvPassParams *d_params, int n, const uint8_t *tjb_tab, const float *null1_tab, int16_t *thr, hipStream_t st)
+{
+  if (n <= 0) return P7X_OK;
+  hipLaunchKernelGGL(msv_thr_kernel, dim3((unsigned) ((kMaxL + 1 + 255) / 256), (unsigned) n), dim3(256), 0, st, d_params, tjb_tab, null1_tab, thr);
+  P7X_HIP(hipGetLastError());
+  return P7X_OK;
 }
 
 __device__ __forceinline__ float log_of_float(float x, const double *tab)
@@ -628,12 +631,14 @@
 }
 
 static void fill_msv_args(LaneArgs &la, const Profile &p, const DevProfile *dp, const p7x_seqdb *db, DeviceCtx *ctx, const StageBufs &b,
-                          int nlong = 0)
-{
+                          int nlong = 0, const int16_t *thr = nullptr, bool exact_all = false)
+{
+  MsvDecide dec{};
+  if (thr) { dec.thr = thr; dec.stage = b.stage; dec.usc = b.usc; dec.list_bias = b.list_bias; dec.counter_bias = &b.counters[1]; dec.scale_b = p.scale_b; }
   MsvWaveArgs w{};
   w.C = dp->msvwC; w.nrows = dp->msvw_rows; w.emis = dp->msvw_emis; w.emis_pk = dp->msvw_pk; w.dsq = db->d_dsq; w.slot_off = db->d_slot_off; w.slot_len = db->d_slot_len;
   w.tjb_tab = ctx->lt.tjb; w.nslots = (int) db->nslots; w.base = p.base_b; w.bias = p.bias_b; w.tec = p.tec_b; w.tbm = p.tbm_b;
-  w.out_xJ = b.xJ;
+  w.out_xJ = b.xJ; w.dec = dec;
   if (nlong > 0) w.nslots = (int) std::min<int64_t>((int64_t) nlong * 64, db->nslots);
   la.msvw = w;
   MsvArgs a{};
@@ -645,6 +650,7 @@
   a.amb_count = &b.counters[10]; a.counter2 = &b.counters[11];
   a.amb_groups = msv_exact_only() ? nullptr : b.list_fin;
   a.R = dp->msvR;
+  a.tab_h = dp->msv_tab_h; a.dec = dec; a.exact_all = exact_all ? 1 : 0;
   la.msv = a;
   MsvArgs x = a;
   x.group_list = a.amb_groups; x.group_count = a.amb_count; x.counter = a.counter2; x.amb_groups = nullptr;
@@ -677,6 +683,55 @@
 }
 
 struct LaneModel { const p7x_oprofile *om = nullptr; DevProfile *dp = nullptr; };
+
+static int get_msv_thresholds(const std::vector<LaneModel> &lm, const std::vector<MsvPassParams> &pp, DeviceCtx *ctx,
+                              std::vector<const int16_t *> &thr, std::vector<std::shared_ptr<DeviceBuf>> &keep)
+{
+  constexpr size_t kKept = 4;
+  const int nl = (int) lm.size();
+  thr.assign((size_t) nl, nullptr);
+  auto find = [&](DevProfile *dp, const MsvPassParams &q) -> const DevProfile::MsvThr * {
+    for (const auto &t : dp->msv_thr)
+      if (t.F1 == q.F1 && t.mmu == q.mmu && t.mlambda == q.mlambda && t.scale_b == q.scale_b && t.base_b == q.base_b) return &t;
+    return nullptr;
+  };
+  std::vector<int> missing;
+  for (int l = 0; l < nl; ++l) {
+    DevProfile *dp = lm[l].dp;
+    std::lock_guard<std::mutex> lk(dp->thr_mu);
+    if (const DevProfile::MsvThr *t = find(dp, pp[(size_t) l])) { thr[(size_t) l] = t->thr; keep.push_back(t->slab); }
+    else missing.push_back(l);
+  }
+  if (missing.empty()) return P7X_OK;
+  const size_t nm = missing.size(), params_bytes = ((nm * sizeof(MsvPassParams) + 255) / 256) * 256, tab = (size_t) kMaxL + 1;
+  auto slab = std::make_shared<DeviceBuf>();
+  int st = slab->reserve(ctx, params_bytes + nm * tab * 2);
+  if (st != P7X_OK) return st;
+  std::vector<MsvPassParams> h(nm);
+  for (size_t z = 0; z < nm; ++z) h[z] = pp[(size_t) missing[z]];
+  MsvPassParams *d_params = slab->as<MsvPassParams>();
+  int16_t *d_thr = reinterpret_cast<int16_t *>(slab->as<char>() + params_bytes);
+  P7X_HIP(hipMemcpy(d_params, h.data(), nm * sizeof(MsvPassParams), hipMemcpyHostToDevice));
+  if ((st = msv_thr_launch(d_params, (int) nm, ctx->lt.tjb, ctx->lt.null1, d_thr, ctx->stream)) != P7X_OK) return st;
+  P7X_HIP(hipStreamSynchronize(ctx->stream));
+  keep.push_back(slab);
+  for (size_t z = 0; z < nm; ++z) {
+    const int l = missing[z];
+    DevProfile *dp = lm[l].dp;
+    std::lock_guard<std::mutex> lk(dp->thr_mu);
+    const DevProfile::MsvThr *t = find(dp, pp[(size_t) l]);
+    if (!t) {
+      if (dp->msv_thr.size() >= kKept) dp->msv_thr.erase(dp->msv_thr.begin());
+      const MsvPassParams &q = pp[(size_t) l];
+      dp->msv_thr.push_back(DevProfile::MsvThr{ q.F1, q.mmu, q.mlambda, q.scale_b, q.base_b, d_thr + z * tab, slab });
+      t = &dp->msv_thr.back();
+    } else keep.push_back(t->slab);
+    thr[(size_t) l] = t->thr;
+  }
+  return P7X_OK;
+}
+static bool msv_fused_decide() { return debug_opt(OPT_MSV_FUSED_DECIDE) != 0; }
+
 
 static int upload_args(Workspace *ws, int first, int n, hipStream_t s)
 {
@@ -775,6 +830,9 @@
   Lease<Workspace> ws;
   int est_bias = 0, est_vit = 0, est_fwd = 0, est_fin = 0;
   bool queued = false, collected = false;
+  bool fused = true;
+  bool msv_exact_all = false;
+  std::vector<std::shared_ptr<DeviceBuf>> thr_keep;
   ~CascadeRun() { sync_and_return(ws); }
 };
 
@@ -955,7 +1013,7 @@
     if (record_events) P7X_HIP(hipEventRecord(ws->ev[7], s));
   }
   const ArgRef dec = lane_run(ws, &LaneArgs::dec, c.first, c.n).ref();
-  hipLaunchKernelGGL(decide_msv_kernel, dim3((unsigned) ((db->nslots + 255) / 256), (unsigned) c.n), dim3(256), 0, s, dec);
+  if (!r.fused) hipLaunchKernelGGL(decide_msv_kernel, dim3((unsigned) ((db->nslots + 255) / 256), (unsigned) c.n), dim3(256), 0, s, dec);
   if (record_events) P7X_HIP(hipEventRecord(ws->ev[1], s));
   hipLaunchKernelGGL(bias_kernel, dim3(lane_grid((r.est_bias + 63) / 64, ctx->num_cu * 4, c.n), (unsigned) c.n), dim3(64), 0, s, dec);
   {
@@ -1024,7 +1082,7 @@
   if ((st = join()) != P7X_OK) return st;
   P7X_HIP(hipEventRecord(ws->ev[7], s));
   const ArgRef dec = lane_run(ws, &LaneArgs::dec, 0, nq).ref();
-  hipLaunchKernelGGL(decide_msv_kernel, dim3((unsigned) ((db->nslots + 255) / 256), (unsigned) nq), dim3(256), 0, s, dec);
+  if (!r.fused) hipLaunchKernelGGL(decide_msv_kernel, dim3((unsigned) ((db->nslots + 255) / 256), (unsigned) nq), dim3(256), 0, s, dec);
   P7X_HIP(hipEventRecord(ws->ev[1], s));
   hipLaunchKernelGGL(bias_kernel, dim3(lane_grid((r.est_bias + 63) / 64, ctx->num_cu * 4, nq), (unsigned) nq), dim3(64), 0, s, dec);
   {
@@ -1112,6 +1170,17 @@
   r.queued = true;
   const ListEstimates est = estimate_lists(cfg, db->nslots);
   r.est_bias = est.bias; r.est_vit = est.vit; r.est_fwd = est.fwd; r.est_fin = est.fin;
+  r.fused = msv_fused_decide();
+  std::vector<const int16_t *> thr_of((size_t) nq, nullptr);
+  if (r.fused) {
+    std::vector<MsvPassParams> pp((size_t) nq);
+    for (int l = 0; l < nq; ++l) {
+      const StageParams sp = make_params(r.lm[l].om->p, cfg);
+      pp[(size_t) l] = MsvPassParams{ sp.F1, sp.mmu, sp.mlambda, sp.msv_reject_below, sp.scale_b, sp.base_b };
+    }
+    if ((st = get_msv_thresholds(r.lm, pp, ctx, thr_of, r.thr_keep)) != P7X_OK) return st;
+    tick("thresholds");
+  }
   std::vector<int> nlong_of((size_t) nq, 0);
   std::vector<int64_t> vit_long_of((size_t) nq, 0);
   for (const LaneClass &c : classes) for (int l = c.first; l < c.first + c.n; ++l) { nlong_of[(size_t) l] = c.nlong; vit_long_of[(size_t) l] = c.vit_long; }
@@ -1124,7 +1193,7 @@
     d.slot_len = db->d_slot_len; d.tjb_tab = ctx->lt.tjb; d.null1_tab = ctx->lt.null1; d.xwmove_tab = ctx->lt.xwmove; d.logtab = ctx->lt.logtab;
     d.dsq = db->d_dsq; d.slot_off = db->d_slot_off; d.eo = dp->bias_eo; d.nslots = db->nslots;
     la.dec = d;
-    fill_msv_args(la, p, dp, db, ctx, b, nlong_of[(size_t) l]);
+    fill_msv_args(la, p, dp, db, ctx, b, nlong_of[(size_t) l], thr_of[(size_t) l], r.msv_exact_all);
     const int64_t vit_long = vit_long_of[(size_t) l];
     fill_vit_args(la, p, dp, db, ctx, b.list_vit, est.vit, &b.counters[2], b.xC,
                   vit_long > 0 ? &b.counters[13] : nullptr, (int) std::min<int64_t>(vit_long, (int64_t) est.vit));
@@ -1609,8 +1678,8 @@
   std::chrono::steady_clock::time_point t0;
 };
 
-int p7x_search_batch_enqueue(const p7x_pipeline_cfg *cfg, const p7x_oprofile *const *oms, size_t nq, const float *bg_f,
-                             const p7x_seqdb *db, p7x_pending **out)
+static int batch_enqueue(const p7x_pipeline_cfg *cfg, const p7x_oprofile *const *oms, size_t nq, const float *bg_f,
+                         const p7x_seqdb *db, p7x_pending **out, bool exact_all)
 {
   if (!cfg || !oms || !db || !out || nq == 0 || nq > 4096) { set_error("p7x_search_batch_enqueue: bad arguments"); return P7X_EINVAL; }
   *out = nullptr;
@@ -1628,12 +1697,16 @@
     }
   }
   pd->cfg = *cfg; pd->db = db;
-  pd->run.cfg = *cfg; pd->run.oms.assign(oms, oms + nq); pd->run.db = db;
+  pd->run.cfg = *cfg; pd->run.oms.assign(oms, oms + nq); pd->run.db = db; pd->run.msv_exact_all = exact_all;
   const int st = cascade_enqueue(pd->run);
   if (st != P7X_OK) return st;
   *out = pd.release();
   return P7X_OK;
 }
+
+int p7x_search_batch_enqueue(const p7x_pipeline_cfg *cfg, const p7x_oprofile *const *oms, size_t nq, const float *bg_f,
+                             const p7x_seqdb *db, p7x_pending **out)
+{ return batch_enqueue(cfg, oms, nq, bg_f, db, out, false); }
 
 int p7x_debug_log_of_float(int device, const float *in, float *out, size_t n)
 {
@@ -1653,11 +1726,13 @@
   return P7X_OK;
 }
 
-int p7x_search_batch_raw(const p7x_pipeline_cfg *cfg, const p7x_oprofile *const *oms, size_t nq, const float *bg_f,
-                         const p7x_seqdb *db, int32_t *xJ, int32_t *xC, uint8_t *stage)
+struct RawDecide { int32_t *counters; int32_t *list_bias; float *usc; };
+
+static int batch_raw(const p7x_pipeline_cfg *cfg, const p7x_oprofile *const *oms, size_t nq, const float *bg_f,
+                     const p7x_seqdb *db, int32_t *xJ, int32_t *xC, uint8_t *stage, bool exact_all, const RawDecide *rd)
 {
   p7x_pending *pd = nullptr;
-  int st = p7x_search_batch_enqueue(cfg, oms, nq, bg_f, db, &pd);
+  int st = batch_enqueue(cfg, oms, nq, bg_f, db, &pd, exact_all);
   if (st != P7X_OK) return st;
   std::unique_ptr<p7x_pending> owner(pd);
   CascadeRun &r = pd->run;
@@ -1665,6 +1740,11 @@
   if (xJ) std::fill(xJ, xJ + nq * (size_t) n, 0);
   if (xC) std::fill(xC, xC + nq * (size_t) n, INT32_MIN);
   if (stage) std::fill(stage, stage + nq * (size_t) n, (uint8_t) 0);
+  if (rd) {
+    std::fill(rd->counters, rd->counters + nq * (size_t) kLaneCounters, 0);
+    std::fill(rd->list_bias, rd->list_bias + nq * (size_t) n, -1);
+    std::fill(rd->usc, rd->usc + nq * (size_t) n, 0.0f);
+  }
   if (!r.queued || ns == 0) return P7X_OK;
   Workspace *ws = r.ws.get();
   P7X_HIP(hipStreamSynchronize(ws->stream));
@@ -1688,8 +1768,100 @@
       P7X_HIP(hipMemcpy(hs.data(), b.stage, (size_t) ns, hipMemcpyDeviceToHost));
       for (int64_t sl = 0; sl < ns; ++sl) stage[q * (size_t) n + (size_t) db->h_order[sl]] = hs[(size_t) sl];
     }
+    if (rd) {
+      std::memcpy(rd->counters + q * (size_t) kLaneCounters, counters, sizeof(counters));
+      const int nb = (int) std::min<int64_t>(std::max(counters[1], 0), ns);
+      std::vector<float> hu((size_t) ns);
+      P7X_HIP(hipMemcpy(hl.data(), b.list_bias, (size_t) nb * 4, hipMemcpyDeviceToHost));
+      P7X_HIP(hipMemcpy(hu.data(), b.usc, (size_t) ns * 4, hipMemcpyDeviceToHost));
+      for (int it = 0; it < nb; ++it) {
+        const int32_t sl = hl[(size_t) it];
+        rd->list_bias[q * (size_t) n + (size_t) it] = (sl >= 0 && sl < ns) ? db->h_order[(size_t) sl] : -2;
+        if (sl >= 0 && sl < ns) rd->usc[q * (size_t) n + (size_t) db->h_order[(size_t) sl]] = hu[(size_t) sl];
+      }
+    }
   }
   return p7x_search_block_wait(pd);
+}
+
+int p7x_search_batch_raw(const p7x_pipeline_cfg *cfg, const p7x_oprofile *const *oms, size_t nq, const float *bg_f,
+                         const p7x_seqdb *db, int32_t *xJ, int32_t *xC, uint8_t *stage)
+{ return batch_raw(cfg, oms, nq, bg_f, db, xJ, xC, stage, true, nullptr); }
+
+int p7x_debug_msv_decide(const p7x_pipeline_cfg *cfg, const p7x_oprofile *const *oms, size_t nq, const float *bg_f, const p7x_seqdb *db,
+                         int exact_all, int32_t *xJ, uint8_t *stage, int32_t *counters, int32_t *list_bias, float *usc)
+{
+  if (!counters || !list_bias || !usc) { set_error("p7x_debug_msv_decide: bad arguments"); return P7X_EINVAL; }
+  const RawDecide rd{ counters, list_bias, usc };
+  return batch_raw(cfg, oms, nq, bg_f, db, xJ, nullptr, stage, exact_all != 0, &rd);
+}
+
+int p7x_debug_msv_thresholds(const p7x_pipeline_cfg *cfg, const p7x_oprofile *om, int device, int16_t *thr, size_t n)
+{
+  if (!cfg || !om || !thr || n > (size_t) kMaxL + 1) { set_error("p7x_debug_msv_thresholds: bad arguments"); return P7X_EINVAL; }
+  DeviceCtx *ctx = nullptr;
+  int st = get_ctx(device, &ctx);
+  if (st != P7X_OK) return st;
+  std::vector<LaneModel> lm(1);
+  lm[0].om = om;
+  if ((st = get_dev_profile(om, ctx, &lm[0].dp)) != P7X_OK) return st;
+  const StageParams sp = make_params(om->p, *cfg);
+  const std::vector<MsvPassParams> pp(1, MsvPassParams{ sp.F1, sp.mmu, sp.mlambda, sp.msv_reject_below, sp.scale_b, sp.base_b });
+  std::vector<const int16_t *> tab;
+  std::vector<std::shared_ptr<DeviceBuf>> keep;
+  if ((st = get_msv_thresholds(lm, pp, ctx, tab, keep)) != P7X_OK) return st;
+  P7X_HIP(hipMemcpy(thr, tab[0], n * 2, hipMemcpyDeviceToHost));
+  return P7X_OK;
+}
+
+int p7x_debug_decide_msv(const p7x_pipeline_cfg *cfg, const p7x_oprofile *om, int device, const int32_t *L, const int32_t *xJ, size_t n,
+                         uint8_t *take, float *usc)
+{
+  if (!cfg || !om || !L || !xJ || !take || !usc || n == 0 || n > ((size_t) 1 << 24)) { set_error("p7x_debug_decide_msv: bad arguments"); return P7X_EINVAL; }
+  for (size_t i = 0; i < n; ++i) if (L[i] < 0 || L[i] > kMaxL) { set_error("p7x_debug_decide_msv: target length out of range"); return P7X_EINVAL; }
+  DeviceCtx *ctx = nullptr;
+  int st = get_ctx(device, &ctx);
+  if (st != P7X_OK) return st;
+  Lease<Workspace> lease;
+  if ((st = get_workspace(ctx, (int64_t) n, 1, lease)) != P7X_OK) return st;
+  Workspace *ws = lease.get();
+  hipStream_t s = ctx->stream;
+  const StageBufs b = ws->lane_bufs(0);
+  DeviceBuf d_len;
+  if ((st = d_len.reserve(ctx, n * 4)) != P7X_OK) return st;
+  std::vector<int16_t> hj(n);
+  for (size_t i = 0; i < n; ++i) hj[i] = (int16_t) xJ[i];
+  DecideArgs d{};
+  d.b = b; d.p = make_params(om->p, *cfg);
+  d.slot_len = d_len.as<int32_t>(); d.tjb_tab = ctx->lt.tjb; d.null1_tab = ctx->lt.null1; d.nslots = (int64_t) n;
+  ws->h_args.as<LaneArgs>()[0].dec = d;
+  if ((st = upload_args(ws, 0, 1, s)) != P7X_OK) return st;
+  P7X_HIP(hipMemsetAsync(ws->counters.as<int>(), 0, ws->counters_bytes(), s));
+  P7X_HIP(hipMemcpyAsync(d_len.as<int32_t>(), L, n * 4, hipMemcpyHostToDevice, s));
+  P7X_HIP(hipMemcpyAsync(b.xJ, hj.data(), n * 2, hipMemcpyHostToDevice, s));
+  hipLaunchKernelGGL(decide_msv_kernel, dim3((unsigned) ((n + 255) / 256), 1), dim3(256), 0, s, lane_run(ws, &LaneArgs::dec, 0, 1).ref());
+  P7X_HIP(hipGetLastError());
+  P7X_HIP(hipMemcpyAsync(take, b.stage, n, hipMemcpyDeviceToHost, s));
+  P7X_HIP(hipMemcpyAsync(usc, b.usc, n * 4, hipMemcpyDeviceToHost, s));
+  P7X_HIP(hipStreamSynchronize(s));
+  return P7X_OK;
+}
+
+int64_t p7x_debug_msv_tables(const p7x_oprofile *om, int device, uint32_t *tab_i16, uint32_t *tab_f16, size_t cap_words)
+{
+  if (!om) { set_error("p7x_debug_msv_tables: bad arguments"); return -P7X_EINVAL; }
+  DeviceCtx *ctx = nullptr;
+  int st = get_ctx(device, &ctx);
+  if (st != P7X_OK) return -st;
+  DevProfile *dp = nullptr;
+  if ((st = get_dev_profile(om, ctx, &dp)) != P7X_OK) return -st;
+  if (dp->msvR <= 0) return 0;
+  const size_t words = (size_t) kTabRows * (size_t) dp->msvS * (dp->msvK >= 8 ? 1 : 2);
+  if (tab_i16 && tab_f16 && cap_words >= words) {
+    if (hipMemcpy(tab_i16, dp->msv_tab, words * 4, hipMemcpyDeviceToHost) != hipSuccess ||
+        hipMemcpy(tab_f16, dp->msv_tab_h, words * 4, hipMemcpyDeviceToHost) != hipSuccess) { set_error("p7x_debug_msv_tables: copy failed"); return -P7X_EDEVICE; }
+  }
+  return (int64_t) words;
 }
 
 int p7x_search_block_enqueue(const p7x_pipeline_cfg *cfg, const p7x_oprofile *om, const float *bg_f, const p7x_seqdb *db,
diff --git a/pyhmmer_amd/csrc/p7x_profile.cpp b/pyhmmer_amd/csrc/p7x_profile.cpp
--- a/pyhmmer_amd/csrc/p7x_profile.cpp
+++ b/pyhmmer_amd/csrc/p7x_profile.cpp
@@ -253,7 +253,7 @@
 int p7x_debug_set_option(const char *name, int value)
 {
   static const char *const names[p7x::OPT_COUNT] = { "small_block", "vit_wave", "msv_exact", "msv_long_groups", "msv_blocks_per_cu", "env_workspace_gb",
-                                                     "device_clustered", "trace_finish", "trace_longtarget", "trace_envelope", "host_profile", "ssv_kernel", "msv_f16", "ens_lds_kb", "ens_fail", "msv_tiers", "stage_merge", "early_pack", "host_order", "vit_long_cut", "fwd_grouped", "region_guard_ppm", "msv_k8", "msv_lane_blocks", "host_align", "align_workspace_gb" };
+                                                     "device_clustered", "trace_finish", "trace_longtarget", "trace_envelope", "host_profile", "ssv_kernel", "msv_f16", "ens_lds_kb", "ens_fail", "msv_tiers", "stage_merge", "early_pack", "host_order", "vit_long_cut", "fwd_grouped", "region_guard_ppm", "msv_k8", "msv_lane_blocks", "host_align", "align_workspace_gb", "msv_fused_decide" };
   if (!name) { p7x::set_error("p7x_debug_set_option: no name"); return P7X_EINVAL; }
   for (int i = 0; i < p7x::OPT_COUNT; ++i)
     if (std::strcmp(name, names[i]) == 0) { p7x::g_debug_opt[i].store(value); return P7X_OK; }
diff --git a/pyhmmer_amd/csrc/p7x_vitfwd.hip b/pyhmmer_amd/csrc/p7x_vitfwd.hip
--- a/pyhmmer_amd/csrc/p7x_vitfwd.hip
+++ b/pyhmmer_amd/csrc/p7x_vitfwd.hip
@@ -213,7 +213,9 @@
         }
       }
     }
-    if (lane == 0 && L > 0) a.out_xJ[slot] = (xEmax >= 255 - a.bias) ? (int16_t) -1 : (int16_t) xJ;
+    const int xres = (xEmax >= 255 - a.bias) ? -1 : xJ;
+    if (lane == 0 && L > 0) a.out_xJ[slot] = (int16_t) xres;
+    if (a.dec.thr) msv_decide(a.dec, lane == 0 && L > 0, slot, L, xres, tjbm - a.tbm, a.base);
   }
 }
 
@@ -316,7 +318,9 @@
         }
       }
     }
-    if (lane == 0 && L > 0) a.out_xJ[slot] = (xEmax >= 255 - a.bias) ? (int16_t) -1 : (int16_t) xJ;
+    const int xres = (xEmax >= 255 - a.bias) ? -1 : xJ;
+    if (lane == 0 && L > 0) a.out_xJ[slot] = (int16_t) xres;
+    if (a.dec.thr) msv_decide(a.dec, lane == 0 && L > 0, slot, L, xres, tjbm - a.tbm, a.base);
   }
 }
 
```

Result: faster. 24290, median of 5 (+1.7%).
